# lukashermann/hulc

Hardware: AMD Instinct MI355X
Metric: trajectory-windows/sec (seq_len=32, bs=64/GPU) (higher is better)
Workload: dtype bf16; 1 GPU; HULC training step, vision goal only (use_clip_auxiliary_loss=false), B=64 windows/GPU, seq_len=32, 200x200 static + 84x84 gripper fp32 NCHW frames, fwd+loss+bwd+Adam, dropout 0.1; global_batch=64, seq_len=32, parallelism=dp1

## Files before the change

### hulc_amd/csrc/capi.hip

```cpp
#include <cstdarg>
#include <cstdio>
#include <cstring>
#include <cstdlib>
#include <cmath>
#include <algorithm>
#include <stdexcept>

#include "engine.h"
#include "sbert.h"
#include "store_gather.h"
#include "store_stage.h"

using namespace hulc_bf16;

static thread_local char g_err[1024] = "";
void hulc_set_error(const char* fmt, ...) {
    va_list ap;
    va_start(ap, fmt);
    vsnprintf(g_err, sizeof(g_err), fmt, ap);
    va_end(ap);
}

struct hulc_ctx {
    IEngine* e = nullptr;
// ... 316 lines not shown
int hulc_set_dropout(hulc_ctx* ctx, float p) {
    if (!(p >= 0.f && p < 1.f)) { hulc_set_error("hulc_set_dropout: p must be in [0,1)"); return 1; }
    ctx->e->set_dropout(p);
    return 0;
}
int hulc_set_option(hulc_ctx* ctx, const char* name, int64_t value) {
    if (!ctx) { hulc_set_error("hulc_set_option: null context"); return 1; }
    return ctx->e->set_option(name, (long long)value);
}
int hulc_get_option(hulc_ctx* ctx, const char* name, int64_t* value) {
    if (!ctx || !value) { hulc_set_error("hulc_get_option: null argument"); return 1; }
    if (name && !strcmp(name, "stage_tickets")) { *value = HULC_STAGE_TICKETS; return 0; }
    long long v = 0;
    const int rc = ctx->e->get_option(name, &v);
    *value = (int64_t)v;
    return rc;
}
int hulc_timers_enable(hulc_ctx* ctx, int32_t on, const char* only_class) { ctx->e->set_timing(on != 0, only_class); return 0; }
int hulc_timers_read(hulc_ctx* ctx, char* json_out, int64_t cap, int32_t reset) { return ctx->e->timers_read(json_out, cap, reset != 0); }
int hulc_get_tensor(hulc_ctx* ctx, const char* name, float* out, int64_t cap, int64_t* n) { return ctx->e->get_tensor(name, out, cap, n); }
int hulc_get_plan_idx(hulc_ctx* ctx, int32_t* out, int64_t cap) { return ctx->e->get_plan_idx(out, cap); }

int hulc_k_gemm_nt(int32_t dtype, const void* A, const void* B, float* C, int32_t M, int32_t N, int32_t K, int64_t lda, int64_t ldb, int64_t ldc,
                   const float* bias, int32_t relu, void* stream) {
    if (dtype == HULC_DTYPE_F16) return hulc_f16::k_gemm_nt(0, A, B, C, M, N, K, lda, ldb, ldc, bias, relu, stream);
    return hulc_bf16::k_gemm_nt(dtype == HULC_DTYPE_F32, A, B, C, M, N, K, lda, ldb, ldc, bias, relu, stream);
}
#define HULC_K_16BIT(name, call)                                                                                          \
    if (dtype == HULC_DTYPE_F16) return hulc_f16::call;                                                                    \
    if (dtype == HULC_DTYPE_BF16) return hulc_bf16::call;                                                                  \
    hulc_set_error(name ": dtype %d is not a 16-bit type", (int)dtype);                                                    \
    return 1
int hulc_k_spatial_softmax64(int32_t dtype, const void* f, int32_t H, int32_t W, int32_t Nf, void* out, float* stats, const float* dout, void* df, void* stream) {
    HULC_K_16BIT("hulc_k_spatial_softmax64", k_spatial_softmax64(f, H, W, Nf, out, stats, dout, df, stream));
}
int hulc_k_enc_tail_fwd(int32_t dtype, int32_t Nf, int32_t ldemb, const hulc_enc_tail_job* a, const hulc_enc_tail_job* b, void* emb, const float* pos, int32_t S,
                        float drop_p, uint64_t seed, float* xf, void* xt, float* z0, float* z1, void* stream) {
    HULC_K_16BIT("hulc_k_enc_tail_fwd", k_enc_tail_fwd(Nf, ldemb, a, b, emb, pos, S, drop_p, (unsigned long long)seed, xf, xt, z0, z1, stream));
}
int hulc_k_enc_tail_bwd(int32_t dtype, int32_t Nf, int32_t ldemb, const hulc_enc_tail_bwd_job* a, const hulc_enc_tail_bwd_job* b, const float* demb, void* stream) {
    HULC_K_16BIT("hulc_k_enc_tail_bwd", k_enc_tail_bwd(Nf, ldemb, a, b, demb, stream));
}
int hulc_k_tr_layer_fwd(int32_t dtype, const hulc_tr_layer_job* job, int32_t B, int32_t S, int32_t ln_in, float dp, void* stream) {
    HULC_K_16BIT("hulc_k_tr_layer_fwd", k_tr_layer_fwd(job, B, S, ln_in, dp, stream));
}
int hulc_k_tr_ffn_bwd(int32_t dtype, const hulc_tr_ffn_bwd_job* job, int32_t B, int32_t S, int32_t bcast, float bdiv, float dp, void* stream) {
    HULC_K_16BIT("hulc_k_tr_ffn_bwd", k_tr_ffn_bwd(job, B, S, bcast, bdiv, dp, stream));
}
int hulc_k_tr_attn_bwd(int32_t dtype, const hulc_tr_attn_bwd_job* job, int32_t B, int32_t S, int32_t nparts, int64_t part_stride, float dp, void* stream) {
    HULC_K_16BIT("hulc_k_tr_attn_bwd", k_tr_attn_bwd(job, B, S, nparts, (long long)part_stride, dp, stream));
}
int hulc_k_gemm_multi(int32_t dtype, int32_t form, const hulc_gemm_epi_job* jobs, int32_t n, int32_t sh, int32_t* ran, void* stream) {
    HULC_K_16BIT("hulc_k_gemm_multi", k_gemm_multi(form, jobs, n, sh, ran, stream));
}
#undef HULC_K_16BIT
int hulc_k_gemm_epi(int32_t dtype, const hulc_gemm_epi_job* job, int32_t kernel, int32_t* ran, void* stream) {
    if (dtype == HULC_DTYPE_F16) return hulc_f16::k_gemm_epi(1, job, kernel, ran, stream);
    if (dtype != HULC_DTYPE_F32 && dtype != HULC_DTYPE_BF16) { hulc_set_error("hulc_k_gemm_epi: unknown dtype %d", (int)dtype); return 1; }
    return hulc_bf16::k_gemm_epi(dtype == HULC_DTYPE_BF16 ? 1 : 0, job, kernel, ran, stream);
}
int hulc_k_gemm_pick(int32_t dtype, int32_t M, int32_t N, int32_t K, int64_t lda, int64_t ldb, int32_t* pick, int32_t* bk) {
    if (dtype != HULC_DTYPE_F32 && dtype != HULC_DTYPE_BF16 && dtype != HULC_DTYPE_F16) { hulc_set_error("hulc_k_gemm_pick: unknown dtype %d", (int)dtype); return 1; }
    return hulc_bf16::k_gemm_pick(dtype != HULC_DTYPE_F32, M, N, K, (long long)lda, (long long)ldb, pick, bk);
}
int hulc_k_gemm_wgrad_nsplit(int32_t dtype, int32_t M, int32_t N, int32_t K, int32_t* nsplit, int32_t* big) {
    if (dtype != HULC_DTYPE_F32 && dtype != HULC_DTYPE_BF16 && dtype != HULC_DTYPE_F16) { hulc_set_error("hulc_k_gemm_wgrad_nsplit: unknown dtype %d", (int)dtype); return 1; }
    return hulc_bf16::k_gemm_wgrad_nsplit(dtype != HULC_DTYPE_F32, M, N, K, nsplit, big);
}
int hulc_k_logistic_loss(int32_t dtype, int32_t wide, const float* heads, int32_t ldh, const float* actions, const float* robot_obs, int32_t B, int32_t S,
                         int32_t n_mix, int32_t n_dim, int32_t num_classes, float log_scale_min, float gripper_alpha, int32_t gripper_control,
                         int32_t discrete_gripper, float grad_scale, const float* lscale, float* row_loss, float* a_tcp_out, void* dheads, void* stream) {
    if (dtype == HULC_DTYPE_F16)
        return hulc_f16::k_logistic_loss(1, wide, heads, ldh, actions, robot_obs, B, S, n_mix, n_dim, num_classes, log_scale_min, gripper_alpha, gripper_control,
                                         discrete_gripper, grad_scale, lscale, row_loss, a_tcp_out, dheads, stream);
    if (dtype != HULC_DTYPE_F32 && dtype != HULC_DTYPE_BF16) { hulc_set_error("hulc_k_logistic_loss: unknown dtype %d", (int)dtype); return 1; }
    return hulc_bf16::k_logistic_loss(dtype == HULC_DTYPE_BF16, wide, heads, ldh, actions, robot_obs, B, S, n_mix, n_dim, num_classes, log_scale_min, gripper_alpha,
                                      gripper_control, discrete_gripper, grad_scale, lscale, row_loss, a_tcp_out, dheads, stream);
}
#define HULC_K_ANY(name, fn, ...)                                                                                                     \
    if (dtype == HULC_DTYPE_F16) return hulc_f16::fn(1, __VA_ARGS__);                                                                  \
    if (dtype != HULC_DTYPE_F32 && dtype != HULC_DTYPE_BF16) { hulc_set_error(name ": unknown dtype %d", (int)dtype); return 1; }      \
    return hulc_bf16::fn(dtype == HULC_DTYPE_BF16 ? 1 : 0, __VA_ARGS__)
int hulc_k_plan_kl_sample(const float* pr_logits, const float* pp_logits, int32_t B, int32_t NCAT, int32_t NCLS, const int32_t* idx_in, int32_t* idx_out, float* probs,
                          float* kl_cat, float* dpp, float* dpr, float w_pp, float w_pr, uint64_t seed, const float* lscale, void* stream) {
    return hulc_bf16::k_plan_kl_sample(pr_logits, pp_logits, B, NCAT, NCLS, idx_in, idx_out, probs, kl_cat, dpp, dpr, w_pp, w_pr, (unsigned long long)seed, lscale, stream);
}
int hulc_k_st_softmax_bwd(int32_t dtype, const float* probs, const float* dplan, const float* dpr_kl, const float* dpp_kl, int32_t rows, int32_t NCLS, float* out, void* out_t,
                          void* dpp_t, void* stream) {
    HULC_K_ANY("hulc_k_st_softmax_bwd", k_st_softmax_bwd, probs, dplan, dpr_kl, dpp_kl, rows, NCLS, out, out_t, dpp_t, stream);
}
int hulc_k_plan_gather(int32_t dtype, const void* w_t, const int32_t* idx, int32_t B, int32_t NCAT, int32_t NCLS, int32_t H, const float* b1, const float* b2, float* out,
                       const void* emb, void* embg, int32_t S, int32_t W, const void* goal, int32_t G, int32_t grow0, void* cb, void* stream) {
    HULC_K_ANY("hulc_k_plan_gather", k_plan_gather, w_t, idx, B, NCAT, NCLS, H, b1, b2, out, emb, embg, S, W, goal, G, grow0, cb, stream);
}
int hulc_k_plan_scatter_grad(int32_t dtype, int32_t form, const void* dC, const int32_t* idx, int32_t B, int32_t NCAT, int32_t NCLS, int32_t H, int32_t KIN, float* dw,
                             int32_t store, void* stream) {
    HULC_K_ANY("hulc_k_plan_scatter_grad", k_plan_scatter_grad, form, dC, idx, B, NCAT, NCLS, H, KIN, dw, store, stream);
}
int hulc_k_normal_kl_sample(int32_t dtype, const float* pr_state, const float* pp_state, int32_t B, int32_t n, const float* eps_in, float* eps_out, float* plan_f, void* plan_t,
                            float* kl_elem, float* dpp, float* dpr, float w_pp, float w_pr, uint64_t seed, const float* lscale, void* stream) {
    HULC_K_ANY("hulc_k_normal_kl_sample", k_normal_kl_sample, pr_state, pp_state, B, n, eps_in, eps_out, plan_f, plan_t, kl_elem, dpp, dpr, w_pp, w_pr, (unsigned long long)seed, lscale, stream);
}
int hulc_k_normal_rsample_bwd(int32_t dtype, const float* dplan, const float* eps, const float* pr_state, const float* dpr_kl, int32_t B, int32_t n, void* out, void* stream) {
    HULC_K_ANY("hulc_k_normal_rsample_bwd", k_normal_rsample_bwd, dplan, eps, pr_state, dpr_kl, B, n, out, stream);
}
int hulc_k_det_head_loss(int32_t dtype, const void* H1, const void* W, const float* bias, const float* actions, const float* robot_obs, int32_t B, int32_t S,
// ... 234 lines not shown
```

### hulc_amd/csrc/conv_wgrad.h

```cpp
#pragma once
#include "common.h"

namespace HULC_NS {

typedef short s16x4_t __attribute__((ext_vector_type(4)));
typedef unsigned int u32x4_t __attribute__((ext_vector_type(4)));
typedef __attribute__((address_space(3))) u32x4_t lds_u32x4;

typedef __attribute__((address_space(3))) char lds_char;
DEVI h16x8_t tr_read8(lds_char* p0, lds_char* p1) {
    const s16x4_t lo = __builtin_amdgcn_ds_read_tr16_b64_v4i16((__attribute__((address_space(3))) s16x4_t*)p0);
    const s16x4_t hi = __builtin_amdgcn_ds_read_tr16_b64_v4i16((__attribute__((address_space(3))) s16x4_t*)p1);
    typedef short s16x8_t __attribute__((ext_vector_type(8)));
    const s16x8_t v = __builtin_shufflevector(lo, hi, 0, 1, 2, 3, 4, 5, 6, 7);
    return __builtin_bit_cast(h16x8_t, v);
}

template <int CI, int CO, int KH, int KW, int S>
struct WgradCfg {
    static constexpr int XS = (S == 1) ? ((CI * 2 / 32) | 1) * 32 : CI * 2 + 16;
    static constexpr int DYS = ((CO * 2 / 32) | 1) * 32;
    static constexpr int CGN = CI / 16;
    static constexpr int NT = KH * KW * CGN;
    static constexpr int NTW = NT / 4;
// ... 1547 lines not shown
    }
    const int grid = std::min(form == 5 ? cap : std::min(cap, 512), max_blocks);
    long long total = 0;
    for (int k = 0; k < n; ++k) total += j[k].Nf;
    if (wg) { for (int k = 0; k < n; ++k) ns[k] = std::min(std::max(wg[k], 1), j[k].Nf); }
    else if (n == 1) ns[0] = grid;
    else if (total <= std::min(form == 5 ? (int)total : 512, max_blocks)) { for (int k = 0; k < n; ++k) ns[k] = j[k].Nf; }
    else {
        if (grid < n) return false;
        int left = grid; double wl = 0;
        for (int k = 0; k < n; ++k) wl += w[k];
        for (int k = n - 1; k > 0; --k) {
            int a, b;
            camera_split(left, wl - w[k], w[k], a, b);
            b = std::min(std::min(b, left - k), j[k].Nf);
            ns[k] = b; left -= b; wl -= w[k];
        }
        ns[0] = std::min(left, j[0].Nf);
    }
    Wgrad1Batch bt{}; bt.n = n;
    int blk = 0;
    for (int k = 0; k < n; ++k) {
        if (k) j[k].part = j[k - 1].part + (long long)ns[k - 1] * Wgrad1Cfg::CO * 192;
        j[k].blk0 = blk; blk += ns[k];
        bt.j[k] = j[k];
    }
    if (form == 1) {
        static bool attr2 = false;
        if (!attr2) { hipFuncSetAttribute((const void*)conv1_wgrad_tr2_kernel<6, 2>, hipFuncAttributeMaxDynamicSharedMemorySize, 80 * 1024); attr2 = true; }
        hipLaunchKernelGGL((conv1_wgrad_tr2_kernel<6, 2>), dim3(blk), dim3(512), lds, st, bt);
    } else if (form == 2) {
        static bool attr2s = false;
        if (!attr2s) { hipFuncSetAttribute((const void*)conv1_wgrad_tr2r_kernel<3, 2, true>, hipFuncAttributeMaxDynamicSharedMemorySize, 80 * 1024); attr2s = true; }
        hipLaunchKernelGGL((conv1_wgrad_tr2r_kernel<3, 2, true>), dim3(blk), dim3(512), lds, st, bt);
    } else if (form == 3) {
        static bool attr2r = false;
        if (!attr2r) { hipFuncSetAttribute((const void*)conv1_wgrad_tr2r_kernel<4, 2>, hipFuncAttributeMaxDynamicSharedMemorySize, 80 * 1024); attr2r = true; }
        hipLaunchKernelGGL((conv1_wgrad_tr2r_kernel<4, 2>), dim3(blk), dim3(512), lds, st, bt);
    } else {
        static bool attr_set = false;
        if (!attr_set) { hipFuncSetAttribute((const void*)conv1_wgrad_tr_kernel, hipFuncAttributeMaxDynamicSharedMemorySize, 160 * 1024 - 64); attr_set = true; }
        for (int k = 0; k < n; ++k) bt.j[k].S.fold = 0;
        hipLaunchKernelGGL(conv1_wgrad_tr_kernel, dim3(blk), dim3(256), lds, st, bt);
    }
    return true;
}
static inline int launch_conv1_wgrad_tr(hipStream_t st, const Conv1Src& X, const h16_t* dY, float* part, float* bias_part, int Nf, int IH, int IW, int OH,
                                        int OW, int max_blocks, int* work_ctr = nullptr) {
    Wgrad1Job q{}; q.S = X; q.work_ctr = work_ctr; q.dY = dY; q.part = part; q.bias_part = bias_part; q.Nf = Nf; q.IH = IH; q.IW = IW; q.OH = OH; q.OW = OW;
    int ns = 0;
    return launch_conv1_wgrad_jobs(st, &q, 1, max_blocks, nullptr, &ns) ? ns : 0;
}

DEVI void lin_bwd_smallm_body(const h16_t* __restrict__ dY, long long ldy, const h16_t* __restrict__ X, long long ldx,
                              int M, int N, int K, float* __restrict__ dW, long long lddw, float* __restrict__ db,
                              float* __restrict__ db2, int mchunk, int store, const int bx, const int by, const int bz, const int gz, char* smem,
                              const bool slabs = false) {
    constexpr int TN = 64, TK = 128, YS = TN * 2 + 16, XS = TK * 2 + 16;
    lds_char* yimg = (lds_char*)smem;
    lds_char* ximg = yimg + 64 * YS;
    const int tid = threadIdx.x, lane = tid & 63, wave = tid >> 6;
    const int n0 = bx * TN, k0 = by * TK;
    const int mbeg = bz * mchunk, mend = min(M, mbeg + mchunk);
    const int g = lane >> 4, a = lane & 15;
    const int prow = a >> 2, ccol = (a & 3) * 8;
    f32x4 acc[8];
#pragma unroll
    for (int j = 0; j < 8; ++j) acc[j] = f32x4{0.f, 0.f, 0.f, 0.f};
    float bsum = 0.f;
    const bool atomic_b = gz > 1;
    const bool atomic = atomic_b && !slabs;
    const int n = n0 + wave * 16 + a;
    const bool vec_ok = !atomic && (lddw & 3) == 0 && ((reinterpret_cast<uintptr_t>(dW) & 15) == 0) && k0 + TK <= K;
    const int orow = lane >> 4, ocol = (lane & 15) * 4;
    float4 oldw[8];
    if (vec_ok) {
#pragma unroll
        for (int j = 0; j < 8; ++j) {
            const int nr = n0 + wave * 16 + (j & 3) * 4 + orow;
            oldw[j] = (store || nr >= N) ? make_float4(0.f, 0.f, 0.f, 0.f) : *reinterpret_cast<const float4*>(dW + (long long)nr * lddw + k0 + (j >> 2) * 64 + ocol);
        }
    }
    u32x4_t ry[2], rx[4];
    auto fetch = [&](int m0) {
#pragma unroll
        for (int u = 0; u < 2; ++u) {
            const int i = tid + u * 256, m = i / (TN / 8), c = i % (TN / 8);
            h16_t v[8];
            if (m0 + m < mend && n0 + c * 8 < N) load8_guard<h16_t>(dY + (long long)(m0 + m) * ldy + n0 + c * 8, N - (n0 + c * 8), v);
            else zero8<h16_t>(v);
            ry[u] = *reinterpret_cast<const u32x4_t*>(v);
        }
#pragma unroll
        for (int u = 0; u < 4; ++u) {
            const int i = tid + u * 256, m = i / (TK / 8), c = i % (TK / 8);
            h16_t v[8];
            if (m0 + m < mend && k0 + c * 8 < K) load8_guard<h16_t>(X + (long long)(m0 + m) * ldx + k0 + c * 8, K - (k0 + c * 8), v);
            else zero8<h16_t>(v);
            rx[u] = *reinterpret_cast<const u32x4_t*>(v);
        }
    };
    fetch(mbeg);
    for (int m0 = mbeg; m0 < mend; m0 += 64) {
        if (m0 > mbeg) __syncthreads();
#pragma unroll
        for (int u = 0; u < 2; ++u) { const int i = tid + u * 256; *(lds_u32x4*)(yimg + (i / (TN / 8)) * YS + (i % (TN / 8)) * 16) = ry[u]; }
#pragma unroll
        for (int u = 0; u < 4; ++u) { const int i = tid + u * 256; *(lds_u32x4*)(ximg + (i / (TK / 8)) * XS + (i % (TK / 8)) * 16) = rx[u]; }
        __syncthreads();
        if (m0 + 64 < mend) fetch(m0 + 64);
#pragma unroll
        for (int ms = 0; ms < 2; ++ms) {
            const int mrow = ms * 32 + g * 8 + prow;
            lds_char* yb = yimg + mrow * YS + wave * 32 + ccol;
            const h16x8_t yf = tr_read8(yb, yb + 4 * YS);
#pragma unroll
            for (int j = 0; j < 8; ++j) {
                lds_char* xb = ximg + mrow * XS + j * 32 + ccol;
                const h16x8_t xf = tr_read8(xb, xb + 4 * XS);
                acc[j] = MFMA_16x16x32_H(xf, yf, acc[j], 0, 0, 0);
            }
        }
        if (db && by == 0) {
#pragma unroll 16
            for (int m = 0; m < 16; ++m) bsum += h2f(*(__attribute__((address_space(3))) h16_t*)(yimg + (wave * 16 + m) * YS + lane * 2));
        }
    }
    if (db && by == 0) {
        __syncthreads();
        *(__attribute__((address_space(3))) float*)(yimg + (wave * 64 + lane) * 4) = bsum;
        __syncthreads();
        if (tid < TN) {
            bsum = 0.f;
#pragma unroll
            for (int w = 0; w < 4; ++w) bsum += *(__attribute__((address_space(3))) float*)(yimg + (w * 64 + tid) * 4);
        }
    }
    if (vec_ok) {
        constexpr int OP = 64 * 4 + 16;
        __syncthreads();
        lds_char* const tb = (lds_char*)smem + wave * (16 * OP);
#pragma unroll
        for (int h = 0; h < 2; ++h) {
#pragma unroll
            for (int jj = 0; jj < 4; ++jj) *(__attribute__((address_space(3))) f32x4*)(tb + a * OP + jj * 64 + g * 16) = acc[h * 4 + jj];
#pragma unroll
            for (int it = 0; it < 4; ++it) {
                const f32x4 v = *(__attribute__((address_space(3))) f32x4*)(tb + (it * 4 + orow) * OP + ocol * 4);
                const int nr = n0 + wave * 16 + it * 4 + orow;
                float4 o = oldw[h * 4 + it];
                o.x += v[0]; o.y += v[1]; o.z += v[2]; o.w += v[3];
                if (nr < N) *reinterpret_cast<float4*>(dW + (long long)nr * lddw + k0 + h * 64 + ocol) = o;
            }
        }
    } else if (n < N) {
#pragma unroll
        for (int j = 0; j < 8; ++j) {
            const int k = k0 + j * 16 + g * 4;
            float* p = dW + (long long)n * lddw + k;
            if (atomic) {
#pragma unroll
                for (int r = 0; r < 4; ++r)
                    if (k + r < K) unsafeAtomicAdd(p + r, acc[j][r]);
            } else if (k + 3 < K && ((((uintptr_t)p) & 15) == 0)) {
                float4 o = store ? make_float4(0.f, 0.f, 0.f, 0.f) : *reinterpret_cast<float4*>(p);
                o.x += acc[j][0]; o.y += acc[j][1]; o.z += acc[j][2]; o.w += acc[j][3];
                *reinterpret_cast<float4*>(p) = o;
            } else {
#pragma unroll
                for (int r = 0; r < 4; ++r)
                    if (k + r < K) p[r] = store ? acc[j][r] : p[r] + acc[j][r];
            }
        }
    }
    if (db && by == 0 && tid < TN && n0 + tid < N) {
        if (atomic_b) { unsafeAtomicAdd(db + n0 + tid, bsum); if (db2) unsafeAtomicAdd(db2 + n0 + tid, bsum); }
        else { db[n0 + tid] += bsum; if (db2) db2[n0 + tid] += bsum; }
    }
}

constexpr int LBS_LDS = 64 * (64 * 2 + 16) + 64 * (128 * 2 + 16);
__global__ void __launch_bounds__(256) lin_bwd_smallm_kernel(const h16_t* __restrict__ dY, long long ldy, const h16_t* __restrict__ X, long long ldx,
                                                             int M, int N, int K, float* __restrict__ dW, long long lddw, float* __restrict__ db,
                                                             float* __restrict__ db2, int mchunk, int store = 0) {
    __shared__ __attribute__((aligned(16))) char smem[LBS_LDS];
    lin_bwd_smallm_body(dY, ldy, X, ldx, M, N, K, dW, lddw, db, db2, mchunk, store, blockIdx.x, blockIdx.y, blockIdx.z, gridDim.z, smem);
}
struct LinBwdJob { const h16_t* dY; const h16_t* X; float* dW; float* db; long long ldx, lddw; int N, K, nx, blk0; float* part; };
struct LinBwdBatch { LinBwdJob j[8]; int n, M, store, mchunk; };
__global__ void __launch_bounds__(256) lin_bwd_smallm_batched_kernel(LinBwdBatch bt) {
    __shared__ __attribute__((aligned(16))) char smem[LBS_LDS];
    int k = 0;
    while (k + 1 < bt.n && (int)blockIdx.x >= bt.j[k + 1].blk0) ++k;
    const LinBwdJob J = bt.j[k];
    const int b = blockIdx.x - J.blk0;
    const bool slabs = bt.mchunk > 0 && J.part;
    lin_bwd_smallm_body(J.dY, (long long)J.N, J.X, J.ldx, bt.M, J.N, J.K, slabs ? J.part + (long long)blockIdx.y * J.N * J.K : J.dW, slabs ? (long long)J.K : J.lddw, J.db, nullptr,
                        bt.mchunk > 0 ? bt.mchunk : 64, slabs ? 1 : bt.store, b % J.nx, b / J.nx, blockIdx.y, gridDim.y, smem, slabs);
}

}
```

### hulc_amd/csrc/engine.h

```cpp
#pragma once
#include <algorithm>
#include <map>
#include <string>
#include <vector>

#include "iengine.h"
#include "repro_sites.h"
#include "trainable_plan.h"
#include "gemm.h"
#include "kernels.h"
#include "plan_ln_launch.h"
#include "conv_wgrad.h"
#include "conv_tile.h"
#include "conv_reg.h"
#include "tr_fused.h"
#include "rnn_persist.h"
#include "enc_tail.h"
#include "rollout_step.h"
#include "aux_heads.h"
#include "aux_rows.h"
#include "det_head.h"

namespace HULC_NS {

// ... 661 lines not shown
                    const int i = gq.n++;
                    gq.a[i] = a; gq.b[i] = b; gq.om[i] = om; gq.ep[i] = ep; gq.M[i] = M; gq.N[i] = N; gq.K[i] = K;
                    gq_fl += 2.0 * M * N * K; gq_by += ((double)M * K + (double)N * K + (double)M * N) * sizeof(T);
                    return;
                }
                gemm_group_flush();
            }
        }
        const double fl = 2.0 * M * N * K, by = ((double)M * K + (double)N * K + (double)M * N) * sizeof(T);
        const GemmPick pick = gemm_pick<T>(a, b, ep, M, N, K, gemm_use_glds);
        if (pick == GEMM_PICK_SKINNY) {
            TimerScope ts(this, M <= 64 ? "skinny_gemm_m64" : "skinny_gemm_rows", "hbm", fl, by);
            gemm_launch_picked<T>(st, pick, a, b, om, ep, M, N, K);
        } else if (gemm_pick_tile(pick) == 128) {
            TimerScope ts(this, "gemm_128x128", "mfma", fl, by);
            gemm_launch_picked<T>(st, pick, a, b, om, ep, M, N, K);
        } else gemm_launch_picked<T>(st, pick, a, b, om, ep, M, N, K);
    }
    void gemm_wgrad(const DenseLoader<T>& a, const DenseLoader<T>& b, float* dW, long long lddw, int M, int N, int K) {
        EpiP ep = epi(dW, true); ep.accumulate = 1;
        if constexpr (std::is_same<T, h16_t>::value) {
            if (a.R1 == 0x7fffffff && b.R1 == 0x7fffffff && skinny_ok(M, N, K, a.s1, b.s1, a.p, b.p)) { gemm(a, b, dense_out(lddw), ep, M, N, K); return; }
        }
        bool big = false;
        const int nsplit = gemm_wgrad_nsplit<T>(M, N, K, &big);
        if (nsplit <= 1) { gemm(a, b, dense_out(lddw), ep, M, N, K); return; }
        if (repro) {
            const long long zs = ((long long)M * N + 3) / 4 * 4;
            if (part_cur + zs * nsplit > this->partcap) { gemm(a, b, dense_out(lddw), ep, M, N, K); return; }
            float* const slabs = this->part + part_cur;
            EpiP es = epi(slabs, true); es.z_stride = zs;
            TimerScope ts(this, big ? "gemm_128x128" : "gemm_64x64_splitk", "mfma", 2.0 * M * N * K, ((double)M * K + (double)N * K) * sizeof(T) + 4.0 * M * N * nsplit);
            if (big) launch_gemm<T, 128, 128>(st, a, b, dense_out(N), es, M, N, K, 1, nsplit);
            else launch_gemm<T, 64, 64>(st, a, b, dense_out(N), es, M, N, K, 1, nsplit);
            const int vec = (N & 3) == 0 && (lddw & 3) == 0 && ((uintptr_t)slabs & 15) == 0 && ((uintptr_t)dW & 15) == 0;
            hipLaunchKernelGGL(slab_sum_kernel, dim3(cdiv((long long)M * N, vec ? 1024 : 256)), dim3(256), 0, st, (const float*)slabs, nsplit, zs, M, N, dW, lddw, vec);
            return;
        }
        nd(ND_GEMM_SPLITK);
        ep.atomic = 1;
        TimerScope ts(this, big ? "gemm_128x128" : "gemm_64x64_splitk", "mfma", 2.0 * M * N * K, ((double)M * K + (double)N * K) * sizeof(T) + 4.0 * M * N);
        if (big) launch_gemm<T, 128, 128>(st, a, b, dense_out(lddw), ep, M, N, K, 1, nsplit);
        else launch_gemm<T, 64, 64>(st, a, b, dense_out(lddw), ep, M, N, K, 1, nsplit);
    }
    EpiP epi(void* out, bool f32) const { EpiP e; e.out = out; e.out_f32 = f32 ? 1 : 0; e.generic_only = epilogue_fast ? 0 : 1; return e; }

    void lin_fwd(const T* X, long long ldx, int M, const LinW& L, EpiP ep, long long ldo) {
        if (!ep.bias) ep.bias = L.b32;
        gemm(dense<T>(X, M, ldx), dense<T>(L.W, L.N, L.K), dense_out(ldo), ep, M, L.N, L.K);
    }
    void lin_wgrad(const T* dY, const T* X, long long ldx, int M, int N, int K, float* dW, long long lddw, float* db, float* db2 = nullptr) {
        if constexpr (std::is_same<T, h16_t>::value) {
            if (M <= 64) {
                hipLaunchKernelGGL(lin_bwd_smallm_kernel, dim3(cdiv(N, 64), cdiv(K, 128)), dim3(256), 0, st, dY, (long long)N, X, ldx, M, N, K, dW, lddw, db, db2, 64, grad_first(dW) ? 1 : 0);
                return;
            }
            grad_ensure_zero(dW);
        }
        const int mp = ldpad(M);
        const bool fuse_cs = std::is_same<T, h16_t>::value && !repro;
        transpose_pair(dY, N, tA, M, N, X, ldx, tB, M, K, mp, fuse_cs ? db : nullptr, fuse_cs ? db2 : nullptr);
        gemm_wgrad(dense<T>(tA, N, mp), dense<T>(tB, K, mp), dW, lddw, N, K, M);
        if (db && !fuse_cs) colsum(dY, N, M, N, db, db2);
    }
    void lin_dgrad(const T* dY, int M, const LinW& L, EpiP ep, const DenseOut& om) {
        gemm(dense<T>(dY, M, L.N), dense<T>(L.Wt, L.K, L.N), om, ep, M, L.K, L.N);
    }
    void ln_fwd(const float* x, long long ldx, int rows, int n, const float* g, const float* b, T* out, long long ldo, float* outf, long long ldf,
                float* stats) {
        launch_ln_fwd<T>(st, x, ldx, rows, n, g, b, out, ldo, outf, ldf, stats);
    }
    static constexpr bool ln_bwd_can_bcast = ln_bwd_fused<T>();
    void ln_bwd(const float* dy, long long lddy, const float* x, long long ldx, const float* stats, const float* g, int rows, int n, float* dxf,
                long long ldd, int acc, T* dxt, long long ldt, float* dg, float* db, float drop_p = 0.f, unsigned long long drop_seed = 0,
                int bcast_rows = 0, float bcast_div = 1.f, int dy_parts = 1, long long dy_part_stride = 0) {
        if (ln_bwd_fused<T>() && !repro && dg && cdiv(rows, ln_bwd_rows_per_block(rows)) > 1) nd(ND_LN_PARAM);
        launch_ln_bwd<T>(st, cspart, dy, lddy, x, ldx, stats, g, rows, n, dxf, ldd, acc, dxt, ldt, dg, db, drop_p, drop_seed, bcast_rows, bcast_div, dy_parts, dy_part_stride, repro);
    }

    int prepare_weights(bool shadow_fresh = false) override {
        if (!bound) { hulc_set_error("hulc_prepare_weights before hulc_bind_params"); return 1; }
        const bool masked = shadow_fresh && tm_active;
        if (masked && tm_ntrain == 0) return 0;
        c1_bias_fold_valid = false;
        if constexpr (!std::is_same<T, float>::value) {
            if (!shadow_fresh) hipLaunchKernelGGL((cast_kernel<float, T>), dim3(2048), dim3(256), 0, st, P, wshadow, (long long)numel);
        }
        {
            ConvPackBatch d;
            int k = 0, blk = 0;
            for (EncW* e : {&encS, &encG})
                for (ConvW* c : {&e->c1, &e->c2, &e->c3}) {
                    d.w[k] = c->W32; d.wf[k] = c->Wf; d.wd[k] = c->nhwc ? c->Wd : nullptr; d.O[k] = (masked && !tm_trainable_w(c->W32)) ? 0 : c->O; d.I[k] = c->I; d.K[k] = c->KH; d.S[k] = c->S; d.nhwc[k] = c->nhwc;
                    d.blk0[k] = blk; blk += cdiv(c->O * c->I * c->KH * c->KW, 256); ++k;
                }
            d.blk0[6] = blk;
            const int blkA = blk, blkB = blkA + cdiv(128 * 3136, 256);
            HeadPack hp = head_pack();
            const int rows = head_rows[0] + head_rows[1] + head_rows[2] + head_rows[3];
            const int r7 = (masked && !tm_trainable_w(encG.fc7.W32)) ? 0 : 128;
            if (masked && !heads_trainable()) for (int i = 0; i < 4; ++i) hp.rows[i] = 0;
            T* const f7t = rest_by_pack ? encG.fc7.Wt : (T*)nullptr;
            T* const wht = rest_by_pack ? wheadsT : (T*)nullptr;
            hipLaunchKernelGGL((weight_pack_kernel<T>), dim3(blkB + cdiv((long long)rows * HID, 256)), dim3(256), 0, st, d, blkA, encG.fc7.W32, encG.fc7.W, r7, 64, 49, blkB, hp,
                               wheads, bheads, HID, f7t, wht, NHEAD);
        }
        if (masked) {
            if (std::is_same<T, float>::value) { if (tm_tr_all.blocks) hipLaunchKernelGGL((batched_transpose_kernel<float, T>), dim3(tm_tr_all.blocks), dim3(256), 0, st, (const TrDesc*)tm_tr_all.desc, tm_tr_all.n); }
            else if (tr_fresh) { if (tm_tr_rest.blocks && !rest_by_pack) hipLaunchKernelGGL(batched_transpose64_kernel, dim3(tm_tr_rest.blocks), dim3(256), 0, st, (const TrDesc*)tm_tr_rest.desc, tm_tr_rest.n, (const unsigned short*)tm_tr_rest.b2d); }
            else if (tm_tr_all.blocks) hipLaunchKernelGGL(batched_transpose64_kernel, dim3(tm_tr_all.blocks), dim3(256), 0, st, (const TrDesc*)tm_tr_all.desc, tm_tr_all.n, (const unsigned short*)tm_tr_all.b2d);
        }
        else if (std::is_same<T, float>::value) hipLaunchKernelGGL((batched_transpose_kernel<float, T>), dim3(tr_blocks), dim3(256), 0, st, trdesc_dev, (int)trdesc.size());
        else if (tr_fresh && tr_adam.n) {
            if (tr_rest.blocks && !rest_by_pack) hipLaunchKernelGGL(batched_transpose64_kernel, dim3(tr_rest.blocks), dim3(256), 0, st, tr_rest.desc, tr_rest.n, (const unsigned short*)tr_rest.b2d);
        }
        else hipLaunchKernelGGL(batched_transpose64_kernel, dim3(tr_blocks), dim3(256), 0, st, trdesc_dev, (int)trdesc.size(), (const unsigned short*)blk2desc_dev);
        const bool was_fresh = tr_fresh && tr_adam.n;
        tr_fresh = false;
        if constexpr (std::is_same<T, h16_t>::value) {
            if (masked) { if (tm_frag.n && !(was_fresh && frag_by_adam)) hipLaunchKernelGGL(frag_pack_kernel, dim3(tm_frag_blocks), dim3(256), 0, st, tm_frag); }
            else if (fragbatch.n && !(was_fresh && frag_by_adam)) hipLaunchKernelGGL(frag_pack_kernel, dim3(frag_blocks), dim3(256), 0, st, fragbatch);
        }
        if (hipGetLastError() != hipSuccess) { hulc_set_error("kernel launch failed in prepare_weights"); return 1; }
        return 0;
    }
    T *trb_c[2] = {nullptr, nullptr}, *trb_a[2] = {nullptr, nullptr}, *trb_d[2] = {nullptr, nullptr}, *trb_b[2] = {nullptr, nullptr};
    LinBwdBatch tr_wjobs{};
    int tr_wblocks = 0;
    void tr_wgrad_add(const T* dY, const T* X, const LinW& L) {
        if constexpr (std::is_same<T, h16_t>::value) {
            LinBwdJob& J = tr_wjobs.j[tr_wjobs.n++];
            J.dY = dY; J.X = X; J.dW = L.dW; J.db = L.db; J.ldx = L.K; J.lddw = L.K; J.N = L.N; J.K = L.K; J.nx = cdiv(L.N, 64); J.blk0 = tr_wblocks; J.part = nullptr;
            tr_wblocks += J.nx * cdiv(L.K, 128);
        }
    }
    void tr_wgrads_flush(int M) {
        if constexpr (std::is_same<T, h16_t>::value) {
            if (tr_wjobs.n == 0) return;
            const int chunk = 256, nz = cdiv(M, chunk);
            tr_wjobs.M = M; tr_wjobs.store = 0; tr_wjobs.mchunk = chunk;
            UnpackBatch ub{};
            int64_t cur = 0; int ublocks = 0;
            for (int i = 0; i < tr_wjobs.n; ++i) {
                LinBwdJob& J = tr_wjobs.j[i];
                const int64_t need = (int64_t)nz * J.N * J.K;
                if (part_cur + cur + need > this->partcap) { J.part = nullptr; continue; }
                J.part = this->part + part_cur + cur; cur += need;
                UnpackJob& U = ub.j[ub.n++];
                U.part = J.part; U.grad = J.dW; U.slab = (long long)J.N * J.K; U.nsplit = nz; U.O = J.N; U.I = J.K; U.KH = U.KW = 1; U.nhwc = 0; U.blk0 = ublocks; U.ysplit = 1;
                ublocks += cdiv(J.N * J.K, 1024);
            }
            if (nz > 1) nd(ND_LIN_BWD_ROWS);
            hipLaunchKernelGGL(lin_bwd_smallm_batched_kernel, dim3(tr_wblocks, nz), dim3(256), 0, st, tr_wjobs);
            if (ub.n > 0) hipLaunchKernelGGL(unpack_conv_wgrad_batched_kernel, dim3(ublocks, 1), dim3(256), 0, st, ub);
            tr_wjobs.n = 0; tr_wblocks = 0;
        }
    }
    float* dparts = nullptr;
    h16_t* dump_page = nullptr;
    bool grads_fresh = false;
    int wacc() const { return grads_fresh ? 0 : 1; }
    struct LazyG { int64_t off, n; bool stale; };
    std::vector<LazyG> lazy;
    void lazy_register(const LinW& L) {
        if (!std::is_same<T, h16_t>::value || !L.dW || (int64_t)L.N * L.K < 65536) return;
        const int64_t off = L.dW - G, exact = (int64_t)L.N * L.K;
        int64_t n = (exact + 63) / 64 * 64;
        for (const auto& kv : tab_order) if (kv.second.off > off && kv.second.off < off + n) n = exact;
        if (off + n > numel) n = exact;
        if (n % 4 || off % 4) return;
        for (const LazyG& z : lazy) if (z.off == off) return;
        if (lazy.size() < 30 && off >= 0 && off + n <= numel) lazy.push_back(LazyG{off, n, false});
    }
    int lazy_find(const float* dW) const { const int64_t off = dW - G; for (size_t i = 0; i < lazy.size(); ++i) if (lazy[i].off == off) return (int)i; return -1; }
    bool grad_first(const float* dW) {
        const int i = lazy_find(dW);
        if (i < 0) return grads_fresh;
        const bool s = lazy[i].stale;
        lazy[i].stale = false;
        return s;
    }
    void grad_ensure_zero(const float* dW) {
        const int i = lazy_find(dW);
        if (i >= 0 && lazy[i].stale) { hipMemsetAsync(G + lazy[i].off, 0, sizeof(float) * lazy[i].n, st); lazy[i].stale = false; }
    }
    void lazy_sweep(int64_t lo, int64_t hi, hipStream_t s) {
        MultiZero mz{}; int k = 0; long long mx = 0;
        for (LazyG& z : lazy)
            if (z.stale && z.off >= lo && z.off + z.n <= hi) { mz.p[k] = G + z.off; mz.n[k] = z.n; mx = std::max<long long>(mx, z.n); ++k; z.stale = false; }
        if (k) hipLaunchKernelGGL(multi_zero_kernel, dim3((unsigned)std::min<long long>(256, cdiv(mx, 4 * 256 * 8)), k), dim3(256), 0, s, mz);
    }
    int flush_grads() override {
        if (!bound) { hulc_set_error("hulc_flush_grads before hulc_bind_params"); return 1; }
        lazy_sweep(0, numel, st);
        return 0;
    }
    int zero_grads() override {
        if (!bound) { hulc_set_error("hulc_zero_grads before hulc_bind_params"); return 1; }
        if (!have_fwd) repro_latch();
        if (lazy.empty() || !lazy_zero_mode) {
            HIP_CHECK(hipMemsetAsync(G, 0, numel * sizeof(float), st));
            for (LazyG& z : lazy) z.stale = false;
        } else {
            MultiZero mz{}; int k = 0; long long mx = 0; int64_t cur = 0;
            auto add = [&](int64_t lo, int64_t hi) { if (hi > lo) { mz.p[k] = G + lo; mz.n[k] = hi - lo; mx = std::max<long long>(mx, hi - lo); ++k; } };
            for (LazyG& z : lazy) { add(cur, z.off); cur = z.off + z.n; z.stale = true; }
            add(cur, numel / 4 * 4);
            if (numel % 4) HIP_CHECK(hipMemsetAsync(G + numel / 4 * 4, 0, sizeof(float) * (numel % 4), st));
// ... 267 lines not shown
```

### hulc_amd/csrc/engine_backward.inc

```
    struct Bucket { int64_t lo, hi; };
    Bucket group_range(const char* prefix) const {
        int64_t lo = numel, hi = 0;
        const std::string a(prefix);
        for (size_t i = 0; i < tab_order.size(); ++i) {
            const auto& kv = tab_order[i];
            if (kv.first.compare(0, a.size(), a) == 0) { lo = std::min(lo, kv.second.off); hi = std::max(hi, i + 1 < tab_order.size() ? tab_order[i + 1].second.off : numel); }
        }
        if (hi <= lo) return Bucket{0, 0};
        return Bucket{lo, std::min<int64_t>(hi, numel)};
    }
    std::vector<std::pair<std::string, Ref>> tab_order;
    std::vector<Bucket> bucket_plan() const {
        std::vector<Bucket> v;
        const Bucket dec = group_range("action_decoder.");
        v.push_back(Bucket{dec.lo, numel});
        v.push_back(group_range("plan_proposal."));
        v.push_back(group_range("plan_recognition."));
        const Bucket vg = group_range("visual_goal."), lg = group_range("language_goal.");
        v.push_back(Bucket{std::min(vg.lo, lg.lo), std::max(vg.hi, lg.hi)});
        v.push_back(group_range("perceptual_encoder."));
        return v;
    }
    int comm_buckets(int64_t* lo, int64_t* hi, int cap) override {
        if (!bound) { hulc_set_error("hulc_comm_buckets before hulc_bind_params"); return -1; }
// ... 21 lines not shown
    int reduce_range(int64_t lo, int64_t hi, int dtype, int span = -1) {
        if (hi <= lo) return 0;
        GradComm& c = *comm;
        const bool vote = vote_pad() >= 0 ? (skip_pad >= lo && skip_pad < hi) : lo == 0;
        if (vote) { skip_vote_put(st); ar_voted = true; }
        c.gate_from(st);
        const size_t n = (size_t)(hi - lo);
        if (span >= 0) c.span_begin(span, (dtype == HULC_DTYPE_F32 ? 4.0 : 2.0) * n);
        int rc;
        if (dtype == HULC_DTYPE_BF16 || dtype == HULC_DTYPE_F16) {
            if (c.stage_elems < numel) {
                if (c.stage) hipFree(c.stage);
                if (hipMalloc(&c.stage, (size_t)numel * 2 + 256) != hipSuccess) { hulc_set_error("hulc_allreduce_grads: staging buffer allocation failed"); return 1; }
                c.stage_elems = numel;
            }
            h16_t* sg = reinterpret_cast<h16_t*>(c.stage) + lo;
            hipLaunchKernelGGL((cast_kernel<float, h16_t>), dim3(std::min<long long>(2048, cdiv((long long)n, 1024))), dim3(256), 0, c.cs, G + lo, sg, (long long)n);
#ifdef HULC_HALF_F16
            const int wire = GradComm::F16;
#else
            const int wire = GradComm::BF16;
#endif
            rc = GradComm::api().allreduce(sg, sg, n, wire, GradComm::SUM, c.comm, c.cs);
            hipLaunchKernelGGL((cast_kernel<h16_t, float>), dim3(std::min<long long>(2048, cdiv((long long)n, 1024))), dim3(256), 0, c.cs, sg, G + lo, (long long)n);
            c.bytes_reduced += 2.0 * n;
        } else {
            rc = GradComm::api().allreduce(G + lo, G + lo, n, GradComm::F32, GradComm::SUM, c.comm, c.cs);
            c.bytes_reduced += 4.0 * n;
        }
        c.n_collectives++;
        if (vote && vote_pad() < 0 && rc == 0 && vote_ptr()) { rc = GradComm::api().allreduce(vote_word, vote_word, 1, GradComm::F32, GradComm::SUM, c.comm, c.cs); c.n_collectives++; c.bytes_reduced += 4.0; }
        if (vote) skip_vote_get(c.cs);
        if (span >= 0) c.span_end(span);
        if (rc != 0) { hulc_set_error("ncclAllReduce failed: %s", GradComm::err(rc)); return 1; }
        return 0;
    }
    bool ar_voted = false;
    int vote_only() {
        if (!rp_skip) rp_skip = alloc<unsigned>(64);
        if (!vote_word) vote_word = alloc<float>(64);
        if (!rp_skip || !vote_word) { hulc_set_error("skip vote: allocation failed"); return 1; }
        GradComm& c = *comm;
        hipLaunchKernelGGL(dp_skip_put_kernel, dim3(1), dim3(1), 0, st, (const unsigned*)rp_skip, opt_seq + 1, vote_word);
        c.gate_from(st);
        const int rc = GradComm::api().allreduce(vote_word, vote_word, 1, GradComm::F32, GradComm::SUM, c.comm, c.cs);
        c.n_collectives++; c.bytes_reduced += 4.0;
        hipLaunchKernelGGL(dp_skip_get_kernel, dim3(1), dim3(1), 0, c.cs, vote_word, rp_skip, opt_seq + 1);
        ar_voted = true;
        if (rc != 0) { hulc_set_error("ncclAllReduce failed: %s", GradComm::err(rc)); return 1; }
        return 0;
    }
    int bucket_ready(int i) {
        if (ar_dtype < 0 || (ar_sent >> i) & 1u) return 0;
        const std::vector<Bucket> v = bucket_plan();
        ar_sent |= 1u << i;
        if (range_all_frozen(v[i].lo, v[i].hi)) return (i == 4 && !ar_voted) ? vote_only() : 0;
        lazy_sweep(v[i].lo, v[i].hi, st);
        return reduce_range(v[i].lo, v[i].hi, ar_dtype, comm_timing ? i : -1);
    }
    int check_ar_dtype(int dtype, const char* who) {
        if (!comm) { hulc_set_error("%s: no communicator (hulc_comm_init first)", who); return 1; }
        if (dtype != HULC_DTYPE_F32 && dtype != HULC_DTYPE_BF16 && dtype != HULC_DTYPE_F16) { hulc_set_error("%s: bucket dtype must be HULC_DTYPE_F32 or a 16-bit type", who); return 1; }
        if (dtype != HULC_DTYPE_F32) {
            if (std::is_same<T, float>::value) { hulc_set_error("%s: 16-bit buckets need a bf16 / fp16 engine (the fp32 engine has no 16-bit kernels in its unit)", who); return 1; }
#ifdef HULC_HALF_F16
            if (dtype != HULC_DTYPE_F16) { hulc_set_error("%s: the fp16 engine offers fp16 buckets (loss-scaled gradients), not bf16", who); return 1; }
#else
            if (dtype != HULC_DTYPE_BF16) { hulc_set_error("%s: the bf16 engine offers bf16 buckets, not fp16", who); return 1; }
#endif
        }
        return 0;
    }
    int allreduce_grads(int dtype) override {
        if (check_ar_dtype(dtype, "hulc_allreduce_grads")) return 1;
        if (!bound) { hulc_set_error("hulc_allreduce_grads before hulc_bind_params"); return 1; }
        if (bwd_stage != 0) { hulc_set_error("hulc_allreduce_grads: encoder part of the backward still pending"); return 1; }
        lazy_sweep(0, numel, st);
        if (tm_active && bucket_plan_ok()) {
            std::vector<Bucket> v = bucket_plan();
            v.erase(std::remove_if(v.begin(), v.end(), [](const Bucket& b) { return b.hi <= b.lo; }), v.end());
            std::sort(v.begin(), v.end(), [](const Bucket& a, const Bucket& b) { return a.lo < b.lo; });
            ar_voted = false;
            for (size_t i = 0; i < v.size();) {
                if (range_all_frozen(v[i].lo, v[i].hi)) { ++i; continue; }
                size_t j = i;
                while (j + 1 < v.size() && !range_all_frozen(v[j + 1].lo, v[j + 1].hi)) ++j;
                if (reduce_range(v[i].lo, v[j].hi, dtype)) return 1;
                i = j + 1;
            }
            if (!ar_voted && vote_only()) return 1;
        } else if (reduce_range(0, numel, dtype)) return 1;
        comm->gate_to(st);
        return 0;
    }
    bool bucket_plan_ok() const {
        std::vector<Bucket> v = bucket_plan();
        v.erase(std::remove_if(v.begin(), v.end(), [](const Bucket& b) { return b.hi <= b.lo; }), v.end());
        std::sort(v.begin(), v.end(), [](const Bucket& a, const Bucket& b) { return a.lo < b.lo; });
        if (v.empty() || v.front().lo != 0 || v.back().hi != numel) return false;
        for (size_t i = 0; i + 1 < v.size(); ++i) if (v[i].hi != v[i + 1].lo) return false;
        return true;
    }
    int backward_allreduce(int dtype) override {
        if (ema_refuse("hulc_backward_allreduce")) return 1;
        if (check_ar_dtype(dtype, "hulc_backward_allreduce")) return 1;
        if (!bucket_plan_ok()) { hulc_set_error("hulc_backward_allreduce: the module-group buckets do not partition the gradient buffer (layout changed?)"); return 1; }
        ar_dtype = dtype; ar_sent = 0; ar_voted = false;
        if (comm_timing) comm->bwd_mark(true, st);
        int rc = backward(-1);
        if (!rc) for (int i = 0; i < 5 && !rc; ++i) rc = bucket_ready(i);
        ar_dtype = -1;
        if (rc) return rc;
        if (comm_timing) comm->bwd_mark(false, st);
        comm->gate_to(st);
        return 0;
    }

    int bwd_stage = 0;
    int backward(int part = -1) override {
        if (ema_refuse("hulc_backward")) return 1;
        if (!have_fwd) { hulc_set_error("hulc_backward without a preceding hulc_forward_loss"); return 1; }
        persist_check("hulc_backward", false);
        bwd_since_opt = true;
        if (part == 1 && bwd_stage != 1) { hulc_set_error("hulc_backward_part(1) must follow hulc_backward_part(0)"); return 1; }
        if (part != 1 && bwd_stage != 0) { hulc_set_error("hulc_backward: encoder part of the previous backward still pending"); return 1; }
        const hulc_batch* b = &cur;
        const int B = b->B, S = b->S, N = B * S, SB = S * B;
        const bool hulc = cfg.kind == HULC_KIND_HULC;
        const float dp = cfg.dropout_p;
        const long long BH = (long long)B * HID;
        const bool cs16 = std::is_same<T, h16_t>::value && !repro;
        if (part == 1) { if (bwd_skip_enc) goto finish; goto encoders; }
        bwd_skip_enc = tm_enc_frozen;
        if (!arena_clean) HIP_CHECK(hipMemsetAsync(zero_arena, 0, sizeof(float) * zero_n, st));
        arena_clean = false;
        work_ctr_next = 0;
        if (poison_partials) HIP_CHECK(hipMemsetAsync(this->part, 0xFF, sizeof(float) * (size_t)this->partcap, st));
        {
        bool have_dseq = false, dseq_cast_done = false;
        const int proj_n = clip_n > 0 ? clip_n : mia_n;
        if (proj_n > 0 || bcz_n > 0) {
            const int n = proj_n > 0 ? proj_n : bcz_n;
            if (proj_n > 0) {
                hipLaunchKernelGGL((cast_kernel<float, T>), dim3(1), dim3(256), 0, st, dimg, dimg_t, (long long)n * GOAL);
                hipLaunchKernelGGL((cast_kernel<float, T>), dim3(1), dim3(256), 0, st, dtxt, dtxt_t, (long long)n * GOAL);
                lin_wgrad(dimg_t, im1, 128, n, GOAL, 128, cl_im2.dW, 128, cl_im2.db);
                { EpiP ep = epi(dim1, false); ep.mask = im1; lin_dgrad(dimg_t, n, cl_im2, ep, dense_out(128)); }
                lin_wgrad(dim1, sf_m, FCH, n, 128, FCH, cl_im0.dW, FCH, cl_im0.db);
                { EpiP ep = epi(dsf_m, true); lin_dgrad(dim1, n, cl_im0, ep, dense_out(FCH)); }
            }
            if (bcz_n > 0) {
                hipLaunchKernelGGL((cast_kernel<float, T>), dim3(cdiv(n * LANG, 256)), dim3(256), 0, st, bz_dpred, bz_dpred_t, (long long)n * LANG);
                lin_wgrad(bz_dpred_t, bz1, 512, n, LANG, 512, bz2.dW, 512, bz2.db);
                { EpiP ep = epi(dbz1, false); ep.mask = bz1; lin_dgrad(bz_dpred_t, n, bz2, ep, dense_out(512)); }
                lin_wgrad(dbz1, sf_m, FCH, n, 512, FCH, bz0.dW, FCH, bz0.db);
                { EpiP ep = epi(dsf_m, true); if (proj_n > 0) ep.accumulate = 1; lin_dgrad(dbz1, n, bz0, ep, dense_out(FCH)); }
            }
            hipLaunchKernelGGL(scatter_rows_add_kernel, dim3(cdiv(n * FCH, 256)), dim3(256), 0, st, dsf_m, auxrows, n, FCH, dseqf, (long long)FCH);
            if (proj_n > 0) {
                lin_wgrad(dtxt_t, la1, 128, n, GOAL, 128, cl_la2.dW, 128, cl_la2.db);
                { EpiP ep = epi(dla1, false); ep.mask = la1; lin_dgrad(dtxt_t, n, cl_la2, ep, dense_out(128)); }
                lin_wgrad(dla1, g_m, GOAL, n, 128, GOAL, cl_la0.dW, GOAL, cl_la0.db);
                { EpiP ep = epi(dg_m, true); lin_dgrad(dla1, n, cl_la0, ep, dense_out(GOAL)); }
                hipLaunchKernelGGL(scatter_rows_add_kernel, dim3(cdiv(n * GOAL, 256)), dim3(256), 0, st, dg_m, auxrows, n, GOAL, dgoal, (long long)GOAL);
            }
            have_dseq = true;
        }
        {
            const long long lastBH = (long long)(S - 1) * BH;
            if (det) {
                if (part_cur + (int64_t)det_head_slabs(SB) * DET_SLAB > this->partcap) { hulc_set_error("hulc_backward: no room for the deterministic head's gradient slabs"); return 1; }
                launch_det_head_dgrad<T>(st, dpre, det_w, H1, B, S, dH1, dZ1 + lastBH);
                launch_det_head_wgrad<T>(st, dpre, H1, SB, this->part + part_cur, det_dw, det_db);
            } else {
            { EpiP ep = epi(dH1, false);
              if (!mlp) { ep.out2 = dZ1 + lastBH; ep.out2_lo = lastBH; ep.out2_hi = lastBH + BH; ep.out2_mask = H1 + lastBH; }
              gemm(dense<T>(dheads, SB, NHEAD), dense<T>(wheadsT, HID, NHEAD), dense_out(HID), ep, SB, HID, NHEAD); }
            {
                const HeadPack hp = head_pack();
                const int rows = head_rows[0] + head_rows[1] + head_rows[2] + head_rows[3];
                const T* const hx = mlp ? Zx1 : H1;
                bool slabs = false;
                if constexpr (std::is_same<T, h16_t>::value) {
                    const int nz = cdiv(SB, 256);
                    if (SB > 64 && part_cur + (int64_t)nz * NHEAD * HID <= this->partcap) {
                        LinBwdBatch bt{}; bt.M = SB; bt.store = 0; bt.mchunk = 256; bt.n = 1;
                        LinBwdJob& J = bt.j[0];
                        if (nz > 1 && !repro) nd(ND_LIN_BWD_ROWS);
                        J.dY = dheads; J.X = hx; J.dW = nullptr; J.db = (repro && nz > 1) ? nullptr : dbheads_tmp; J.ldx = HID; J.lddw = HID; J.N = NHEAD; J.K = HID; J.nx = cdiv(NHEAD, 64); J.blk0 = 0;
                        J.part = this->part + part_cur;
                        hipLaunchKernelGGL(lin_bwd_smallm_batched_kernel, dim3(J.nx * cdiv(HID, 128), nz), dim3(256), 0, st, bt);
                        if (!J.db) colsum(dheads, NHEAD, SB, NHEAD, dbheads_tmp);
                        hipLaunchKernelGGL(unpack_heads_grad_kernel, dim3(cdiv((long long)rows * HID, 256)), dim3(256), 0, st, hp, J.part, dbheads_tmp, HID, nz, (long long)NHEAD * HID);
                        slabs = true;
                    }
                }
                if (!slabs) {
                    lin_wgrad(dheads, hx, HID, SB, NHEAD, HID, dwheads_tmp, HID, dbheads_tmp);
                    hipLaunchKernelGGL(unpack_heads_grad_kernel, dim3(cdiv((long long)rows * HID, 256)), dim3(256), 0, st, hp, dwheads_tmp, dbheads_tmp, HID, 1, 0ll);
                }
            }
            }
            if (mlp) {
                lin_wgrad(dH1, H1, HID, SB, HID, HID, mlp2.dW, HID, mlp2.db);
                { EpiP ep = epi(dZ1, false); ep.mask = H1; lin_dgrad(dH1, SB, mlp2, ep, dense_out(HID)); }
                lin_wgrad(dZ1, H0, HID, SB, HID, HID, mlp1.dW, HID, mlp1.db);
                { EpiP ep = epi(dZ0, false); ep.mask = H0; lin_dgrad(dZ1, SB, mlp1, ep, dense_out(HID)); }
                const int mp = ldpad(SB);
                transpose_pair(dZ0, HID, tA, SB, HID, embg, DE, tB, SB, DE, mp, cs16 ? dbih0 : nullptr, nullptr);
                h0t_valid = false;
                { EpiP ep = epi(dwih0 + dec_plan, true); ep.accumulate = 1; gemm(dense<T>(tA, HID, mp), dense<T>(tB, DE, mp), dense_out(KIN), ep, HID, DE, SB); }
            } else {
            rnn_bwd(dH1, H1, dZ1, whh1, B, S, 1, false, false, true);
            {
                const int mp = ldpad(SB);
                const bool fuse_cs = cs16;
                bool h0t_kept = false;
                if constexpr (std::is_same<T, h16_t>::value) {
                    if (!tB2) tB2 = alloc<T>(tcap);
                    if (tB2) { transpose_triple(dZ1, HID, tA, SB, HID, H1, HID, tB, SB, HID, H0, HID, tB2, SB, HID, mp, fuse_cs ? dbih1 : nullptr, fuse_cs ? dbhh1 : nullptr); h0t_kept = true; }
                }
                if (!h0t_kept)
                transpose_pair(dZ1, HID, tA, SB, HID, H1, HID, tB, SB, HID, mp, fuse_cs ? dbih1 : nullptr, fuse_cs ? dbhh1 : nullptr);
                h0t_valid = h0t_kept;
                bool paired = false;
                if constexpr (std::is_same<T, h16_t>::value) {
                    const bool pair_sw = gemm_pair_mode;
                    EpiP e1 = epi(whh1.dW, true), e2 = epi(wih1.dW, true);
                    if (pair_sw && gemm_use_glds && S > 1 && gemm_glds_pair_ok(dense<T>(tA, HID, mp), dense<T>(tB, HID, mp), dense<T>(tB, HID, mp), e1, e2, HID, HID, SB, B)) {
                        if (!tB2) tB2 = alloc<T>(tcap);
                        if (tB2) {
                            if (!h0t_kept) cast_tr<T, T>(H0, HID, nullptr, 0, tB2, mp, SB, HID);
                            e1.accumulate = grad_first(whh1.dW) ? 0 : 1; e2.accumulate = grad_first(wih1.dW) ? 0 : 1;
                            TimerScope ts(this, "gemm_128x128", "mfma", 2.0 * HID * HID * ((double)SB + (double)(S - 1) * B), (3.0 * HID * SB) * sizeof(T) + 8.0 * HID * HID, 1);
                            launch_gemm_glds_pair(st, dense<T>(tA, HID, mp), dense<T>(tB, HID, mp), dense<T>(tB2, HID, mp), dense_out(HID), e1, e2, HID, HID, SB, B);
                            paired = true;
                        }
                    }
                }
                if (!paired && h0t_kept && std::is_same<T, h16_t>::value) gemm_group_begin();
                if (!paired) {
                if (S > 1) { EpiP ep = epi(whh1.dW, true); ep.accumulate = grad_first(whh1.dW) ? 0 : 1;
                  gemm(dense<T>(tA + B, HID, mp), dense<T>(tB, HID, mp), dense_out(HID), ep, HID, HID, (S - 1) * B); }
                if (!h0t_kept) cast_tr<T, T>(H0, HID, nullptr, 0, tB, mp, SB, HID);
                { EpiP ep = epi(wih1.dW, true); ep.accumulate = grad_first(wih1.dW) ? 0 : 1; gemm(dense<T>(tA, HID, mp), dense<T>(h0t_kept ? tB2 : tB, HID, mp), dense_out(HID), ep, HID, HID, SB); }
                }
                if (!fuse_cs) colsum(dZ1, HID, SB, HID, dbih1, dbhh1);
            }
            { EpiP ep = epi(dH0, false); ep.out2 = dZ0 + lastBH; ep.out2_lo = lastBH; ep.out2_hi = lastBH + BH; ep.out2_mask = H0 + lastBH;
              gemm(dense<T>(dZ1, SB, HID), dense<T>(wih1.Wt, HID, HID), dense_out(HID), ep, SB, HID, HID); }
            gemm_group_end();
            rnn_bwd(dH0, H0, dZ0, whh0, B, S, 1, false, false, true);
            {
                const int mp = ldpad(SB);
                if (h0t_valid) {
                    transpose_pair(dZ0, HID, tA, SB, HID, embg, DE, tB, SB, DE, mp, cs16 ? dbih0 : nullptr, cs16 ? dbhh0 : nullptr);
                    if (S > 1) { EpiP ep = epi(whh0.dW, true); ep.accumulate = grad_first(whh0.dW) ? 0 : 1;
                      gemm(dense<T>(tA + B, HID, mp), dense<T>(tB2, HID, mp), dense_out(HID), ep, HID, HID, (S - 1) * B); }
                } else {
                transpose_pair(dZ0, HID, tA, SB, HID, H0, HID, tB, SB, HID, mp, cs16 ? dbih0 : nullptr, cs16 ? dbhh0 : nullptr);
                if (S > 1) { EpiP ep = epi(whh0.dW, true); ep.accumulate = grad_first(whh0.dW) ? 0 : 1;
                  gemm(dense<T>(tA + B, HID, mp), dense<T>(tB, HID, mp), dense_out(HID), ep, HID, HID, (S - 1) * B); }
                cast_tr<T, T>(embg, DE, nullptr, 0, tB, mp, SB, DE);
                }
                { EpiP ep = epi(dwih0 + dec_plan, true); ep.accumulate = 1; gemm(dense<T>(tA, HID, mp), dense<T>(tB, DE, mp), dense_out(KIN), ep, HID, DE, SB); }
            }
            }
            if (!bwd_skip_enc) { EpiP ep = epi(demb + (EMB - DE), true); ep.accumulate = 1;
              gemm(dense<T>(dZ0, SB, HID), dense<T>(wih0T + (long long)dec_plan * HID, DE, HID), dense_out_map(B, EMB, (long long)S * EMB), ep, SB, DE, HID); }
            hipLaunchKernelGGL((sum_over_t_kernel<T>), dim3(cdiv(BH, 256)), dim3(256), 0, st, dZ0, S, BH, dC);
            if constexpr (!std::is_same<T, h16_t>::value) colsum(dC, HID, B, HID, dbih0, dbhh0);
            else if (!cs16) colsum(dZ0, HID, SB, HID, dbih0, dbhh0);
            { EpiP ep = epi(dgoal, true); ep.accumulate = 1;
              gemm(dense<T>(dC, B, HID), dense<T>(wih0T + (long long)(dec_plan + DE) * HID, GOAL, HID), dense_out(GOAL), ep, B, GOAL, HID); }
            {
                const int mp = ldpad(B);
                transpose_pair(dC, HID, tA, B, HID, goal_t, GOAL, tB, B, GOAL, mp);
                EpiP ep = epi(dwih0 + dec_plan + DE, true); ep.accumulate = 1;
                gemm(dense<T>(tA, HID, mp), dense<T>(tB, GOAL, mp), dense_out(KIN), ep, HID, GOAL, B);
            }
            if (hulc) {
                { EpiP ep = epi(dplan, true); gemm(dense<T>(dC, B, HID), dense<T>(wih0T, PLAN, HID), dense_out(PLAN), ep, B, PLAN, HID); }
                launch_plan_scatter_grad<T>(st, plan_scatter_w4<T>(NCLS), dC, pidx, B, NCAT, NCLS, HID, KIN, dwih0, grads_fresh ? 1 : 0);
            }
            if (mcil) {
                { EpiP ep = epi(dplan, true); gemm(dense<T>(dC, B, HID), dense<T>(wih0T, dec_plan, HID), dense_out(dec_plan), ep, B, dec_plan, HID); }
                lin_wgrad(dC, plan_t, dec_plan, B, HID, dec_plan, dwih0, KIN, nullptr);
            }
        }
        const bool hold_buckets = hold_buckets_mode && mcil && !gru && ar_dtype >= 0 && persist_mode && !persist_under_comm && !(rp_probed && !rp_ok);
        if (!hold_buckets && bucket_ready(0)) return 1;
        if (hulc) {
            launch_st_softmax_bwd<T>(st, probs, dplan, dpr_kl, dpp_kl, B * NCAT, NCLS, dprl, dprl_t, dppl_t);
            DenseOut om = dense_out(EMB + GOAL);
            mlp_bwd(dppl_t, ppx, EMB + GOAL, B, pp, 5, ppa, dt_a, dt_a + (long long)B * HID, dppx, &om, 0);
            hipLaunchKernelGGL(pp_input_bwd_kernel, dim3(cdiv(B * (EMB + GOAL), 256)), dim3(256), 0, st, dppx, B, EMB, GOAL, demb, (long long)S * EMB, dgoal);
            if (bucket_ready(1)) return 1;
            lin_wgrad(dprl_t, seqf_t, FCH, B, PLAN, FCH, pr_fs.dW, FCH, pr_fs.db);
            { EpiP ep = epi(dseqf, true);
              if (have_dseq) ep.accumulate = 1;
              else { ep.out2 = dseq_t; ep.out2_lo = 0; ep.out2_hi = (long long)B * FCH; dseq_cast_done = true; }
              lin_dgrad(dprl_t, B, pr_fs, ep, dense_out(FCH)); }
            have_dseq = true;
        }
        if (mcil) {
            const int n = PLAN / 2;
            launch_normal_rsample_bwd<T>(st, dplan, plan_eps, pr_logits, dpr_kl, B, n, dprl_t);
            hipLaunchKernelGGL((cast_kernel<float, T>), dim3(cdiv(B * PLAN, 256)), dim3(256), 0, st, dpp_kl, dppl_t, (long long)B * PLAN);
            DenseOut om = dense_out(EMB + GOAL);
            mlp_bwd(dppl_t, ppx, EMB + GOAL, B, pp, 5, ppa, dt_a, dt_a + (long long)B * HID, dppx, &om, 0);
            hipLaunchKernelGGL(pp_input_bwd_kernel, dim3(cdiv(B * (EMB + GOAL), 256)), dim3(256), 0, st, dppx, B, EMB, GOAL, demb, (long long)S * EMB, dgoal);
            if (!hold_buckets && bucket_ready(1)) return 1;
            if (gru) bigru_bwd(dprl_t, B, S); else birnn_bwd(dprl_t, B, S);
            if (hold_buckets && (bucket_ready(0) || bucket_ready(1))) return 1;
        }
        if (have_dseq) {
            if (!dseq_cast_done) hipLaunchKernelGGL((cast_kernel<float, T>), dim3(cdiv(B * FCH, 256)), dim3(256), 0, st, dseqf, dseq_t, (long long)B * FCH);
            lin_wgrad(dseq_t, xm, EMB, B, FCH, EMB, pr_fc.dW, EMB, pr_fc.db);
            { EpiP ep = epi(dxm, true); lin_dgrad(dseq_t, B, pr_fc, ep, dense_out(EMB)); }
            float* dx = dxa; float* dnext = dxb;
            if (!ln_bwd_can_bcast) hipLaunchKernelGGL(bcast_over_s_kernel, dim3(cdiv((long long)N * EMB, 256)), dim3(256), 0, st, dxm, B, S, EMB, dx);
            for (int l = 1; l >= 0; --l) {
                const bool bc = ln_bwd_can_bcast && l == 1;
                bool ffn_fused = false;
                if constexpr (std::is_same<T, h16_t>::value) ffn_fused = trf_on() && S <= 64;
                T *b_c = dt_c, *b_a = dt_a, *b_d = dt_c, *b_b = dt_b;
                bool defer_w = false;
                if constexpr (std::is_same<T, h16_t>::value) {
                    defer_w = ffn_fused;
                    if (defer_w) {
                        if (!trb_c[l]) { trb_c[l] = alloc<T>((int64_t)maxN * EMB); trb_a[l] = alloc<T>((int64_t)maxN * FF); trb_d[l] = alloc<T>((int64_t)maxN * EMB, l ? "tr_bd1" : "tr_bd0"); trb_b[l] = alloc<T>((int64_t)maxN * 3 * EMB, l ? "tr_bb1" : "tr_bb0"); }
                        b_c = trb_c[l]; b_a = trb_a[l]; b_d = trb_d[l]; b_b = trb_b[l];
                    }
                }
                if constexpr (std::is_same<T, h16_t>::value) {
                    if (ffn_fused) {
                        if (!dparts) dparts = alloc<float>(4ll * maxN * EMB);
                        TrFfnBwdP q{};
                        q.dx = bc ? dxm : dx; q.bcast = bc ? 1 : 0; q.bdiv = (float)S; q.y2 = y2[l]; q.st2 = st2[l]; q.n2g = tr_n2g[l]; q.dg2 = d_tr_n2g[l]; q.db2 = d_tr_n2b[l];
                        q.W2t = tr_l2[l].Wtfr; q.W1t = tr_l1[l].Wtfr; q.hff = hff[l]; q.dt_c = b_c; q.dt_a = b_a; q.part = dparts; q.B = B; q.S = S; q.N = N; q.dp = dp;
                        q.seed_y = site_seed(4 + 4 * l);
                        {
                            TimerScope ts(this, "transformer_fused", "mfma", 2.0 * N * (2.0 * EMB * FF), (double)N * (2 * EMB + FF) * sizeof(T));
                            if (B > 1) nd(ND_TR_LN_BWD);
                            launch_tr_ffn_bwd(st, q);
                        }
                        tr_wgrad_add(b_c, hff[l], tr_l2[l]); tr_wgrad_add(b_a, x1t[l], tr_l1[l]);
                    }
                }
                if (!ffn_fused) {
                ln_bwd(bc ? dxm : dx, EMB, y2[l], EMB, st2[l], tr_n2g[l], N, EMB, dy_f, EMB, 0, dt_c, EMB, d_tr_n2g[l], d_tr_n2b[l], dp, site_seed(4 + 4 * l),
                       bc ? S : 0, (float)S);
                lin_wgrad(dt_c, hff[l], FF, N, EMB, FF, tr_l2[l].dW, FF, tr_l2[l].db);
                { EpiP ep = epi(dt_a, false); ep.mask = hff[l]; ep.alpha = dp > 0.f ? 1.f / (1.f - dp) : 1.f; lin_dgrad(dt_c, N, tr_l2[l], ep, dense_out(FF)); }
                lin_wgrad(dt_a, x1t[l], EMB, N, FF, EMB, tr_l1[l].dW, EMB, tr_l1[l].db);
                { EpiP ep = epi(dnext, true); ep.res = dy_f; ep.res_f32 = 1; ep.res_ld = EMB; lin_dgrad(dt_a, N, tr_l1[l], ep, dense_out(EMB)); }
                }
                bool attn_fused = false;
                if constexpr (std::is_same<T, h16_t>::value) {
                    attn_fused = ffn_fused && EMB == 128 && NH == 8 && S <= 32;
                    if (attn_fused) {
                        TrAttnBwdP q{};
                        q.parts = dparts; q.part_stride = (long long)N * EMB; q.nparts = 4; q.y1 = y1[l]; q.st1 = st1[l]; q.n1g = tr_n1g[l]; q.dg1 = d_tr_n1g[l]; q.db1 = d_tr_n1b[l];
                        q.Wot = tr_out[l].Wtfr; q.Wint = tr_in[l].Wtfr; q.qkv = qkv[l]; q.Pat = Pat[l]; q.b_d = b_d; q.b_b = b_b; q.dy_f = dy_f; q.dx = dx;
                        q.B = B; q.S = S; q.dp = dp; q.seed_o = site_seed(2 + 4 * l); q.seed_att = site_seed(1 + 4 * l);
                        launch_tr_attn_bwd(st, q);
                        tr_wgrad_add(b_d, ao[l], tr_out[l]);
                        tr_wgrad_add(b_b, xt[l], tr_in[l]);
                        continue;
                    }
                }
                ln_bwd(ffn_fused ? dparts : dnext, EMB, y1[l], EMB, st1[l], tr_n1g[l], N, EMB, dy_f, EMB, 0, b_d, EMB, d_tr_n1g[l], d_tr_n1b[l], dp, site_seed(2 + 4 * l), 0, 1.f,
                       ffn_fused ? 4 : 1, (long long)N * EMB);
                if (defer_w) tr_wgrad_add(b_d, ao[l], tr_out[l]);
                else lin_wgrad(b_d, ao[l], EMB, N, EMB, EMB, tr_out[l].dW, EMB, tr_out[l].db);
                { EpiP ep = epi(dt_a, false); lin_dgrad(b_d, N, tr_out[l], ep, dense_out(EMB)); }
                launch_attention_bwd<T>(st, attention_s64(S), qkv[l], Pat[l], dt_a, B, S, EMB, NH, b_b, dp, site_seed(1 + 4 * l));
                if (defer_w) tr_wgrad_add(b_b, xt[l], tr_in[l]);
                else lin_wgrad(b_b, xt[l], EMB, N, 3 * EMB, EMB, tr_in[l].dW, EMB, tr_in[l].db);
                { EpiP ep = epi(dx, true); ep.res = dy_f; ep.res_f32 = 1; ep.res_ld = EMB; lin_dgrad(b_b, N, tr_in[l], ep, dense_out(EMB)); }
            }
            tr_wgrads_flush(N);
            {
                const int bchunk = (std::is_same<T, float>::value || repro) ? B : 8;
                if (cdiv(B, bchunk) > 1) nd(ND_POS_EMB);
                hipLaunchKernelGGL(pr_input_bwd_kernel, dim3(cdiv(S * EMB, 256), cdiv(B, bchunk)), dim3(256), 0, st, dx, B, S, EMB, dp, site_seed(0), demb, dpos, bchunk);
            }
        }
        if (bucket_ready(1) || bucket_ready(2)) return 1;
        if (pair) {
            const int Bv = pairBv, Bl = B - pairBv;
            T* av[2] = {gl1, gl2};
            T* al[2] = {gl1 + (long long)Bv * HID, gl2 + (long long)Bv * HID};
            ln_bwd(dgoal, GOAL, gl3, GOAL, goal_st, ln_vg_g, Bv, GOAL, nullptr, 0, 0, dgl3_t, GOAL, d_ln_vg_g, d_ln_vg_b);
            DenseOut om = dense_out((long long)S * EMB);
            mlp_bwd(dgl3_t, emb + (long long)(S - 1) * EMB, (long long)S * EMB, Bv, vg, 3, av, dt_a, dt_a + (long long)B * HID, bwd_skip_enc ? nullptr : demb + (long long)(S - 1) * EMB, bwd_skip_enc ? nullptr : &om, bwd_skip_enc ? 0 : 1);
            ln_bwd(dgoal + Bv * GOAL, GOAL, gl3 + Bv * GOAL, GOAL, goal_st + 2 * Bv, ln_lg_g, Bl, GOAL, nullptr, 0, 0, dgl3_t + Bv * GOAL, GOAL, d_ln_lg_g, d_ln_lg_b);
            mlp_bwd(dgl3_t + Bv * GOAL, lang_t, LANG, Bl, lg, 3, al, dt_a, dt_a + (long long)B * HID, nullptr, nullptr, 0);
        } else {
            T* acts[2] = {gl1, gl2};
            if (b->is_lang) {
                ln_bwd(dgoal, GOAL, gl3, GOAL, goal_st, ln_lg_g, B, GOAL, nullptr, 0, 0, dgl3_t, GOAL, d_ln_lg_g, d_ln_lg_b);
                mlp_bwd(dgl3_t, lang_t, LANG, B, lg, 3, acts, dt_a, dt_a + (long long)B * HID, nullptr, nullptr, 0);
            } else {
                ln_bwd(dgoal, GOAL, gl3, GOAL, goal_st, ln_vg_g, B, GOAL, nullptr, 0, 0, dgl3_t, GOAL, d_ln_vg_g, d_ln_vg_b);
                DenseOut om = dense_out((long long)S * EMB);
                mlp_bwd(dgl3_t, emb + (long long)(S - 1) * EMB, (long long)S * EMB, B, vg, 3, acts, dt_a, dt_a + (long long)B * HID,
                        bwd_skip_enc ? nullptr : demb + (long long)(S - 1) * EMB, bwd_skip_enc ? nullptr : &om, bwd_skip_enc ? 0 : 1);
            }
        }
        }
        if (bucket_ready(3)) return 1;
        if (part == 0) {
            lazy_sweep(0, numel, st);
            if (hipGetLastError() != hipSuccess) { hulc_set_error("kernel launch failed in backward"); return 1; }
            bwd_stage = 1;
            return 0;
        }
        if (bwd_skip_enc) goto finish;
    encoders:
        {
            const Conv1Src src[2] = {conv1_src(*b, false), conv1_src(*b, true)}, src2[2] = {conv1_src(cur2, false), conv1_src(cur2, true)};
            const int Nenc = enc_frames(N);
            const bool tail_fused = enc_tail_fusable() && (!repro || enc_tail_bwd_room(Nenc));
            if (ragged()) launch_rows_reduce(st, demb, rg_lens(), rg_off(), B, S, EMB, demb_c);
            if (tail_fused) enc_tail_bwd_both(Nenc);
            enc_bwd_both(src, pair ? src2 : nullptr, Nenc, tail_fused);
            flush_unpacks();
        }
    finish:
        if (bucket_ready(4)) return 1;
        lazy_sweep(0, numel, st);
        if (hipGetLastError() != hipSuccess) { hulc_set_error("kernel launch failed in backward"); return 1; }
        have_fwd = false;
        bwd_stage = 0;
        grads_fresh = false;
        return 0;
    }
```

### hulc_amd/csrc/engine_encoders.inc

```
    ConvGeom geom(int Nf, int IH, int C, int K, int S) const {
        ConvGeom g; g.Nf = Nf; g.IH = g.IW = IH; g.C = C; g.KH = g.KW = K; g.S = S; g.OH = g.OW = (IH - K) / S + 1; return g;
    }
    Conv1Src conv1_src(const hulc_batch& b, bool gripper) const {
        Conv1Src s;
        s.X = gripper ? b.rgb_gripper : b.rgb_static;
        s.u8 = b.frames_u8 != 0;
        s.shift = s.u8 ? (gripper ? b.shift_gripper : b.shift_static) : nullptr;
        s.pad = gripper ? b.pad_gripper : b.pad_static;
        s.fold = (s.u8 && std::is_same<T, h16_t>::value && u8_fold_mode) ? 1 : 0;
        if (s.u8 && b.window_start) { s.wstart = reinterpret_cast<const long long*>(b.window_start); s.S = b.S; s.nstore = b.store_frames; }
        if (s.wstart && (b.window_len || b.window_len_host)) {
            const int set = &b == &cur2 ? 1 : 0;
            s.wstart = wl_frame[set]; s.S = 1;
            if (s.shift) s.shift = wl_shift[set][gripper ? 1 : 0];
        }
        return s;
    }
    static Conv1Src conv1_src_f32(const void* x) { return Conv1Src{x, nullptr, 0, 0}; }
    long long* wl_frame[2] = {nullptr, nullptr};
    int* wl_shift[2][2] = {{nullptr, nullptr}, {nullptr, nullptr}};
    int wl_alloc(int set) {
        if (!wl_frame[set]) {
            wl_frame[set] = alloc<long long>((int64_t)maxN); wl_shift[set][0] = alloc<int>((int64_t)maxN * 2); wl_shift[set][1] = alloc<int>((int64_t)maxN * 2);
            if (alloc_failed) { hulc_set_error("window_len: workspace allocation failed"); return 1; }
// ... 181 lines not shown
        return ok(encS) && ok(encG) && EMB == 128;
    }
    bool x0_done = false;
    void enc_tail_fwd_both(int Nf, bool with_x0 = false, int S = 1, float dp = 0.f) {
        if constexpr (std::is_same<T, h16_t>::value) {
            EncTailP q{};
            if (with_x0) { q.pos = pos32; q.xf = xf[0]; q.xt = xt[0]; q.z0 = y2[0]; q.z1 = y2[1]; q.S = S; q.drop_p = dp; q.seed = site_seed(0); x0_done = true; }
            for (int k = 0; k < 2; ++k) {
                const EncW& e = encw(k); EncA& a = enca(k);
                EncTailCam& c = q.cam[k];
                c.x = e.gripper ? a.g0 : a.ss; c.W1 = e.fc1.W; c.W2 = e.fc2.W; c.b1 = e.fc1.b32; c.b2 = e.fc2.b32;
                c.lng = e.lng; c.lnb = e.lnb; c.f1 = a.f1; c.f2 = a.f2; c.lnst = a.lnst; c.col0 = k * 64;
            }
            q.emb = enc_emb(); q.Nf = Nf; q.ldemb = EMB;
            launch_enc_tail_fwd(st, q);
        }
    }
    UnpackBatch unpack_jobs{};
    int64_t part_cur = 0;
    int unpack_blocks = 0;
    bool unpack_room(int jobs, int64_t floats) const { return unpack_jobs.n + jobs <= UNPACK_MAX_JOBS && part_cur + floats <= this->partcap; }
    float* queue_unpack(float* grad, int O, int I, int KH, int KW, int nhwc, int nsplit, int ysplit) {
        const long long slab = (long long)O * I * KH * KW;
        if (!unpack_room(1, nsplit * slab)) return nullptr;
        float* const slabs = this->part + part_cur;
        UnpackJob& U = unpack_jobs.j[unpack_jobs.n++];
        U.part = slabs; U.grad = grad; U.slab = slab; U.nsplit = nsplit; U.O = O; U.I = I; U.KH = KH; U.KW = KW; U.nhwc = nhwc; U.blk0 = unpack_blocks; U.ysplit = ysplit;
        unpack_blocks += cdiv((int)slab, 1024); part_cur += nsplit * slab;
        return slabs;
    }
    void flush_unpacks() {
        constexpr int yparts = 8;
        if (repro) for (int i = 0; i < unpack_jobs.n; ++i) unpack_jobs.j[i].ysplit = 1;
        else for (int i = 0; i < unpack_jobs.n; ++i) if (unpack_jobs.j[i].ysplit == 0 && unpack_jobs.j[i].nsplit > 1) nd(ND_CONV_UNPACK_SPLIT);
        if (unpack_jobs.n > 0) hipLaunchKernelGGL(unpack_conv_wgrad_batched_kernel, dim3(unpack_blocks, repro ? 1 : yparts), dim3(256), 0, st, unpack_jobs);
        unpack_jobs.n = 0; part_cur = 0; unpack_blocks = 0;
    }
    bool tail_fc7_done = false;
    void enc_tail_bwd_both(int Nf) {
        if constexpr (std::is_same<T, h16_t>::value) {
            EncTailBwdP q{};
            for (int k = 0; k < 2; ++k) {
                const EncW& e = encw(k); EncA& a = enca(k);
                EncTailBwdCam& c = q.cam[k];
                c.f2 = a.f2; c.lnst = a.lnst; c.lng = e.lng; c.f1 = a.f1; c.W2t = e.fc2.Wt; c.W1t = e.fc1.Wt;
                c.xmask = a.g0; c.dlng = e.dlng; c.dlnb = e.dlnb;
                c.d_f2 = a.d_f2t; c.d_f1 = a.d_f1; c.dx_f32 = a.d_ss; c.dx_t = a.d_g0; c.col0 = k * 64;
            }
            q.demb = enc_demb(); q.Nf = Nf; q.ldemb = EMB;
            const int nblk = cdiv(Nf, 16);
            const bool slab_pg = repro && nblk > 1;
            if (slab_pg) for (int k = 0; k < 2; ++k) q.cam[k].pg_slab = cspart + (long long)k * 2 * nblk * 64;
            if (!repro && Nf > 16) nd(ND_ENC_TAIL_LN);
            if (!repro && Nf > 256) nd(ND_LIN_BWD_ROWS);
            launch_enc_tail_bwd(st, q);
            if (slab_pg)
                for (int k = 0; k < 2; ++k) {
                    hipLaunchKernelGGL(colsum_final_kernel, dim3(1), dim3(256), 0, st, (const float*)q.cam[k].pg_slab, nblk, 64, encw(k).dlng, (float*)nullptr, 1.f);
                    hipLaunchKernelGGL(colsum_final_kernel, dim3(1), dim3(256), 0, st, (const float*)q.cam[k].pg_slab + (long long)nblk * 64, nblk, 64, encw(k).dlnb, (float*)nullptr, 1.f);
                }
            constexpr int chunk = 256;
            LinBwdBatch bt{}; bt.M = Nf; bt.store = 0; bt.mchunk = chunk;
            int blk = 0;
            const int nz = cdiv(Nf, chunk);
            const bool cs_bias = repro && nz > 1;
            auto add = [&](const T* dY, const T* X, const LinW& L, float* dW, float* slabs) {
                LinBwdJob& J = bt.j[bt.n++];
                J.dY = dY; J.X = X; J.dW = dW; J.db = cs_bias ? nullptr : L.db; J.ldx = L.K; J.lddw = L.K; J.N = L.N; J.K = L.K; J.nx = cdiv(L.N, 64); J.blk0 = blk; J.part = slabs;
                blk += J.nx * cdiv(L.K, 128);
            };
            for (int k = 0; k < 2; ++k) {
                const EncW& e = encw(k); EncA& a = enca(k);
                add(a.d_f2t, a.f1, e.fc2, e.fc2.dW, queue_unpack(e.fc2.dW, e.fc2.N, e.fc2.K, 1, 1, 0, nz, 1));
                add(a.d_f1, e.gripper ? a.g0 : a.ss, e.fc1, e.fc1.dW, queue_unpack(e.fc1.dW, e.fc1.N, e.fc1.K, 1, 1, 0, nz, 1));
            }
            const LinW& L = encG.fc7;
            float* const slabs7 = L.N == 128 && L.K == 3136 ? queue_unpack(L.dW, 128, 64, 7, 7, 1, nz, 1) : nullptr;
            tail_fc7_done = slabs7 != nullptr;
            if (slabs7) add(aG.d_g0, aG.a3, L, nullptr, slabs7);
            hipLaunchKernelGGL(lin_bwd_smallm_batched_kernel, dim3(blk, nz), dim3(256), 0, st, bt);
            if (cs_bias) {
                for (int k = 0; k < 2; ++k) {
                    const EncW& e = encw(k); EncA& a = enca(k);
                    colsum(a.d_f2t, e.fc2.N, Nf, e.fc2.N, e.fc2.db);
                    colsum(a.d_f1, e.fc1.N, Nf, e.fc1.N, e.fc1.db);
                }
                if (slabs7) colsum(aG.d_g0, L.N, Nf, L.N, L.db);
            }
        }
    }
    bool enc_tail_bwd_room(int Nf) const {
        const int64_t nz = cdiv(Nf, 256);
        return unpack_room(5, nz * (2 * (64ll * 512 + 512ll * 128) + 128ll * 3136));
    }
    h16_t* zero_page = nullptr;
    const h16_t* wgrad_zero_page() {
        if constexpr (std::is_same<T, h16_t>::value) { if (!zero_page) zero_page = alloc<h16_t>(128); }
        return zero_page;
    }
    template <int TM, typename LB> int wgrad_gemm(const ConvW& c, const T* dy, const LB& lb, long long npix) {
        const int Kc = c.I * c.KH * c.KW;
        int nsplit = (int)std::min<long long>(std::max<long long>(1, npix / 2048), (this->partcap - part_cur) / ((long long)c.O * Kc));
        nsplit = std::min(nsplit, 256);
        EpiP ep = epi(this->part + part_cur, true); ep.z_stride = (long long)c.O * Kc;
        PixMajorLoaderT<T> la{}; la.p = dy; la.rows = c.O; la.ld = c.O;
        launch_gemm<T, TM, 64>(st, la, lb, dense_out(Kc), ep, c.O, Kc, (int)npix, 1, nsplit);
        return nsplit;
    }
    void wgrad_unpack(const ConvW& c, const T* dy, long long npix, int nsplit, bool bias_done) {
        const bool many = std::is_same<T, h16_t>::value && nsplit >= 64;
        const int yparts = many && !repro ? 16 : 1;
        if (!(many && queue_unpack(c.dW, c.O, c.I, c.KH, c.KW, c.nhwc, nsplit, 0))) {
            if (yparts > 1) nd(ND_CONV_UNPACK_SPLIT);
            hipLaunchKernelGGL(unpack_conv_wgrad_kernel, dim3(cdiv(c.O * c.I * c.KH * c.KW, 1024), yparts), dim3(256), 0, st, this->part + part_cur, nsplit,
                               (long long)c.O * c.I * c.KH * c.KW, c.dW, c.O, c.I, c.KH, c.KW, c.nhwc);
        }
        if (!bias_done) colsum(dy, c.O, (int)npix, c.O, c.db);
    }
    void conv_wgrad(int k, int sn, int Nf) {
        const Stage s = stage(k, sn, Nf);
        const ConvW& c = s.c; const ConvGeom& g = s.g;
        const long long npix = (long long)g.Nf * g.OH * g.OW;
        int nsplit = 0;
        if constexpr (std::is_same<T, h16_t>::value) {
            TimerScope ts(this, "conv_wgrad_tr", "mfma", conv_wgrad_flops(c, g), conv_wgrad_bytes(c, g, 2));
            float* const kb = repro ? nullptr : c.db;
            if (c.I == 64 && c.KH == 3) nsplit = launch_conv_wgrad_tr<64, 64, 3, 3, 1>(st, s.x, s.dy, this->part + part_cur, kb, g.Nf, g.IH, g.IW, g.OH, g.OW, 512, claim_ctr(g.Nf > 1), wgrad_zero_page());
            else if (c.I == 32 && c.KH == 4) nsplit = launch_conv_wgrad_tr<32, 64, 4, 4, 2>(st, s.x, s.dy, this->part + part_cur, kb, g.Nf, g.IH, g.IW, g.OH, g.OW, 512, claim_ctr(g.Nf > 1), wgrad_zero_page());
            if (nsplit > 1 && !repro) nd(ND_CONV_BIAS);
        }
        const bool tr = nsplit > 0;
        if (!tr) nsplit = wgrad_gemm<64>(c, s.dy, ConvNHWCLoaderT<T>{s.x, g}, npix);
        wgrad_unpack(c, s.dy, npix, nsplit, tr && !repro);
    }
    void conv1_wgrad(int k, const Conv1Src& src, int Nf, const Conv1Src* src2) {
        const EncW& e = encw(k); EncA& a = enca(k);
        const ConvW& c = e.c1;
        for (int h = 0; h < (src2 ? 2 : 1); ++h) {
            const int nf = src2 ? src_frames(Nf, h) : Nf;
            const ConvGeom g = geom(nf, e.IH, 3, 8, 4);
            const long long npix = (long long)nf * g.OH * g.OW;
            const Conv1Src& sh = h ? *src2 : src;
            const long long foff = h ? src_frames(Nf, 0) : 0;
            const T* dy = a.dact1 + foff * g.OH * g.OW * 32;
            const float* x = nullptr;
// ... 191 lines not shown
```

### hulc_amd/csrc/engine_forward.inc

```
    void mlp_fwd(const T* x, long long ldx, int M, LinW* L, int n, T** acts, float* outf, T* outt) {
        const T* in = x; long long ld = ldx;
        for (int i = 0; i < n; ++i) {
            if (i < n - 1) { EpiP ep = epi(acts[i], false); ep.relu = 1; lin_fwd(in, ld, M, L[i], ep, L[i].N); in = acts[i]; ld = L[i].N; }
            else {
                if (outf) { EpiP ep = epi(outf, true); lin_fwd(in, ld, M, L[i], ep, L[i].N); }
                if (outt) { EpiP ep = epi(outt, false); lin_fwd(in, ld, M, L[i], ep, L[i].N); }
            }
        }
    }
    T* mlp_dy[8] = {nullptr, nullptr, nullptr, nullptr, nullptr, nullptr, nullptr, nullptr};
    void mlp_bwd(const T* dy, const T* x, long long ldx, int M, LinW* L, int n, T** acts, T* s0, T* s1, float* dxf, const DenseOut* om, int dx_acc) {
        const T* d = dy;
        if constexpr (std::is_same<T, h16_t>::value) {
            if (M <= 64 && n <= 8) {
                bool all_first = true;
                for (int i = 0; i < n; ++i) { const int z = lazy_find(L[i].dW); all_first = all_first && (z >= 0 ? lazy[z].stale : grads_fresh); }
                for (int i = 0; i < n; ++i) { if (all_first) grad_first(L[i].dW); else grad_ensure_zero(L[i].dW); }
                LinBwdBatch bt{}; bt.M = M; bt.store = all_first ? 1 : 0;
                int blk = 0;
                for (int i = n - 1; i >= 0; --i) {
                    const T* in = i > 0 ? acts[i - 1] : x;
                    const long long ld = i > 0 ? L[i - 1].N : ldx;
                    LinBwdJob& J = bt.j[bt.n++];
                    J.dY = d; J.X = in; J.dW = L[i].dW; J.db = L[i].db; J.ldx = ld; J.lddw = L[i].K; J.N = L[i].N; J.K = L[i].K; J.nx = cdiv(L[i].N, 64); J.blk0 = blk;
                    blk += J.nx * cdiv(L[i].K, 128);
                    if (i > 0) {
                        if (!mlp_dy[i]) mlp_dy[i] = alloc<T>((int64_t)64 * 2048);
                        T* o = L[i].K <= 2048 ? mlp_dy[i] : (T*)nullptr;
                        if (!o) { hulc_set_error("mlp_bwd: hidden width %d exceeds the per-layer gradient buffers", L[i].K); return; }
                        EpiP ep = epi(o, false); ep.mask = acts[i - 1];
                        lin_dgrad(d, M, L[i], ep, dense_out(L[i].K));
                        d = o;
                    } else if (dxf) {
                        EpiP ep = epi(dxf, true); ep.accumulate = dx_acc;
                        lin_dgrad(d, M, L[i], ep, *om);
                    }
                }
                hipLaunchKernelGGL(lin_bwd_smallm_batched_kernel, dim3(blk), dim3(256), 0, st, bt);
                return;
            }
        }
        T* scratch[2] = {s0, s1};
        for (int i = n - 1; i >= 0; --i) {
            const T* in = i > 0 ? acts[i - 1] : x;
            const long long ld = i > 0 ? L[i - 1].N : ldx;
            lin_wgrad(d, in, ld, M, L[i].N, L[i].K, L[i].dW, L[i].K, L[i].db);
            if (i > 0) {
                T* o = scratch[i & 1];
                EpiP ep = epi(o, false); ep.mask = acts[i - 1];
                lin_dgrad(d, M, L[i], ep, dense_out(L[i].K));
                d = o;
            } else if (dxf) {
                EpiP ep = epi(dxf, true); ep.accumulate = dx_acc;
                lin_dgrad(d, M, L[i], ep, *om);
            }
        }
    }

    void trunk_fwd(const hulc_batch* b, float dp) {
        const int B = b->B, S = b->S, N = B * S;
        const bool hulc = cfg.kind == HULC_KIND_HULC;
        bool ppx_packed = false;
        {
            const Conv1Src src[2] = {conv1_src(*b, false), conv1_src(*b, true)}, src2[2] = {conv1_src(cur2, false), conv1_src(cur2, true)};
            const bool tail_fused = enc_tail_fusable();
            const int Nenc = enc_frames(N);
            enc_fwd_both(src, pair ? src2 : nullptr, Nenc, tail_fused);
            x0_done = false;
            if (tail_fused) enc_tail_fwd_both(Nenc, !ragged() && !mcil && trf_on() && S <= 64 && EMB == 128, S, dp);
            if (ragged()) launch_rows_expand<T>(st, emb_c, rg_lens(), rg_off(), B, S, EMB, emb);
            enc_frames_last = Nenc;
        }
        if (pair) {
            const int Bv = pairBv, Bl = B - pairBv;
            T* av[2] = {gl1, gl2};
            T* al[2] = {gl1 + (long long)Bv * HID, gl2 + (long long)Bv * HID};
            mlp_fwd(emb + (long long)(S - 1) * EMB, (long long)S * EMB, Bv, vg, 3, av, gl3, nullptr);
            ln_fwd(gl3, GOAL, Bv, GOAL, ln_vg_g, ln_vg_b, goal_t, GOAL, nullptr, 0, goal_st);
            hipLaunchKernelGGL((cast_kernel<float, T>), dim3(cdiv(Bl * LANG, 256)), dim3(256), 0, st, b->lang, lang_t, (long long)Bl * LANG);
            mlp_fwd(lang_t, LANG, Bl, lg, 3, al, gl3 + Bv * GOAL, nullptr);
            ln_fwd(gl3 + Bv * GOAL, GOAL, Bl, GOAL, ln_lg_g, ln_lg_b, goal_t + Bv * GOAL, GOAL, nullptr, 0, goal_st + 2 * Bv);
        } else {
            T* acts[2] = {gl1, gl2};
            auto goal_ln = [&](const float* g_, const float* b_) {
                if (hulc || mcil) {
                    hipLaunchKernelGGL((goal_ln_concat_kernel<T>), dim3(cdiv(B, 4) + cdiv(B * EMB, 256)), dim3(256), 0, st, gl3, B, GOAL, g_, b_, goal_t, goal_st, emb, (long long)S * EMB, EMB, ppx);
                    ppx_packed = true;
                } else ln_fwd(gl3, GOAL, B, GOAL, g_, b_, goal_t, GOAL, nullptr, 0, goal_st);
            };
            if (b->is_lang) {
                hipLaunchKernelGGL((cast_kernel<float, T>), dim3(cdiv(B * LANG, 256)), dim3(256), 0, st, b->lang, lang_t, (long long)B * LANG);
// ... 260 lines not shown
```

### hulc_amd/csrc/iengine.h

```cpp
#pragma once
#include <hip/hip_runtime.h>
#include <cstring>
#include <map>
#include <string>
#include <vector>

#include "../../include/hulc_hip.h"
#include "comm.h"

void hulc_set_error(const char* fmt, ...);

struct IEngine {
    virtual ~IEngine() { delete comm; delete comm_pending; }
    virtual int bind(float* p, float* g, float* m, float* v, int64_t numel, int n, const char* const* names, const int64_t* offs,
                     const int64_t* numels) = 0;
    virtual int prepare_weights(bool shadow_fresh = false) = 0;
    virtual int zero_grads() = 0;
    virtual int flush_grads() = 0;
    virtual int forward(const hulc_batch* b, float lw, float cw, float* out, int on_host) = 0;
    virtual int forward_pair(const hulc_batch* vis, const hulc_batch* lang, float lw, float cw, float* out8, int on_host) = 0;
    virtual int backward(int part = -1) = 0;
    virtual int validate(const hulc_batch* b, const hulc_val_noise* nz, float* out17, int32_t* plan_pp_out, int32_t* plan_pr_out, float* pred_pp_out,
                         float* pred_pr_out) = 0;
    virtual int clip_gt_encode(const float* lang_emb, int m, int slot) = 0;
// ... 125 lines not shown
            js += buf; first = false;
            if (reset) { t.used = 0; t.flops = t.bytes = 0; t.launches = 0; }
        }
        js += "}";
        if ((int64_t)js.size() + 1 > cap) { hulc_set_error("hulc_timers_read: buffer too small"); return 1; }
        memcpy(out, js.c_str(), js.size() + 1);
        return 0;
    }
};

#define HULC_TU_DECLS                                                                                                                         \
    IEngine* make_engine(const hulc_config& cfg, int* rc);                                                                                   \
    int k_gemm_nt(int is_f32, const void* A, const void* B, float* C, int M, int N, int K, long long lda, long long ldb, long long ldc, \
                  const float* bias, int relu, void* stream);                                                                                \
    int k_spatial_softmax64(const void* f, int H, int W, int Nf, void* out, float* stats, const float* dout, void* df, void* stream);          \
    int k_enc_tail_fwd(int Nf, int ldemb, const hulc_enc_tail_job* a, const hulc_enc_tail_job* b, void* emb, const float* pos, int S,           \
                       float drop_p, unsigned long long seed, float* xf, void* xt, float* z0, float* z1, void* stream);                         \
    int k_enc_tail_bwd(int Nf, int ldemb, const hulc_enc_tail_bwd_job* a, const hulc_enc_tail_bwd_job* b, const float* demb, void* stream);     \
    int k_logistic_loss(int t16, int wide, const float* heads, int ldh, const float* actions, const float* robot_obs, int B, int S, int nmix,   \
                        int ndim, int num_classes, float log_scale_min, float gripper_alpha, int gripper_control, int discrete_gripper,         \
                        float grad_scale, const float* lscale, float* row_loss, float* a_tcp_out, void* dheads, void* stream);                  \
    int k_det_head_loss(int t16, const void* H1, const void* W, const float* bias, const float* actions, const float* robot_obs, int B, int S, int criterion,     \
                        int frame, float grad_scale, const float* lscale, float* row_loss, float* pred, float* dpre, void* stream);                              \
    int k_det_head_bwd(int t16, const float* dpre, const void* W, const void* H1, int B, int S, void* dH1, void* dZ1, float* dW, float* db, void* stream);        \
    int k_det_head_act(int t16, const void* h1, const void* W, const float* bias, const float* robot_obs, int n, float* out, void* stream);                       \
    int k_plan_kl_sample(const float* pr_logits, const float* pp_logits, int B, int NCAT, int NCLS, const int* idx_in, int* idx_out, float* probs,  \
                         float* kl_cat, float* dpp, float* dpr, float w_pp, float w_pr, unsigned long long seed, const float* lscale, void* stream); \
    int k_st_softmax_bwd(int t16, const float* probs, const float* dplan, const float* dpr_kl, const float* dpp_kl, int rows, int NCLS, float* out,  \
                         void* out_t, void* dpp_t, void* stream);                                                                               \
    int k_plan_gather(int t16, const void* w_t, const int* idx, int B, int NCAT, int NCLS, int H, const float* b1, const float* b2, float* out,   \
                      const void* emb, void* embg, int S, int W, const void* goal, int G, int grow0, void* cb, void* stream);                     \
    int k_plan_scatter_grad(int t16, int form, const void* dC, const int* idx, int B, int NCAT, int NCLS, int H, int KIN, float* dw, int store,   \
                            void* stream);                                                                                                      \
    int k_normal_kl_sample(int t16, const float* pr_state, const float* pp_state, int B, int n, const float* eps_in, float* eps_out, float* plan_f, \
                           void* plan_t, float* kl_elem, float* dpp, float* dpr, float w_pp, float w_pr, unsigned long long seed,                 \
                           const float* lscale, void* stream);                                                                                  \
    int k_normal_rsample_bwd(int t16, const float* dplan, const float* eps, const float* pr_state, const float* dpr_kl, int B, int n, void* out,  \
                             void* stream);                                                                                                     \
    int k_layernorm_fwd(int t16, const float* x, long long ldx, int rows, int n, const float* g, const float* b, void* out, long long ldo,        \
                        float* out_f32, long long ldf, float* stats, void* stream);                                                             \
    int k_layernorm_bwd(int t16, const float* dy, long long lddy, const float* x, long long ldx, const float* stats, const float* g, int rows,    \
                        int n, float* dx_f32, long long ldd, int accumulate, void* dx_t, long long ldt, float* dg, float* db, float drop_p,       \
                        unsigned long long seed, int bcast_rows, float bcast_div, int dy_parts, long long dy_part_stride, float* scratch,        \
                        void* stream);                                                                                                          \
    int k_layernorm_mean(int t16, const float* x, int B, int S, int n, const float* g, const float* b, float* stats, void* out, float* yout,      \
                         void* stream);                                                                                                         \
    int k_tr_layer_fwd(const hulc_tr_layer_job* j, int B, int S, int ln_in, float dp, void* stream);                                            \
    int k_tr_ffn_bwd(const hulc_tr_ffn_bwd_job* j, int B, int S, int bcast, float bdiv, float dp, void* stream);                                \
    int k_tr_attn_bwd(const hulc_tr_attn_bwd_job* j, int B, int S, int nparts, long long part_stride, float dp, void* stream);                  \
    int k_gemm_epi(int t16, const hulc_gemm_epi_job* j, int kernel, int* ran, void* stream);                                                    \
    int k_gemm_multi(int form, const hulc_gemm_epi_job* jobs, int n, int sh, int* ran, void* stream);                                           \
    int k_gemm_pick(int t16, int M, int N, int K, long long lda, long long ldb, int* pick, int* bk);                                            \
    int k_gemm_wgrad_nsplit(int t16, int M, int N, int K, int* nsplit, int* big);                                                               \
    int k_conv_wgrad(const char* who, int typed, int which, const void* X, const void* dY, float* out, float* db_out, int Nf, int IH, int* slabs, \
                     void* stream);                                                                                                             \
    int k_conv1_wgrad_u8(const char* who, int typed, const void* X, const int* shifts, int pad, const void* dY, float* dw_out, float* db_out,   \
                         int Nf, int IH, int form, int fold, int* slabs, void* stream);                                                         \
    int k_conv_tile(const char* who, int typed, int mode, const void* img, const void* w, const float* bias, const void* mask, void* out,       \
                    unsigned* bits1_out, int Nf, int IMH, int OUTH, int relu, int wgs, void* stream);                                           \
    int k_conv_pair(const char* who, int typed, int stage, const hulc_conv_job* a, const hulc_conv_job* b, int wg_a, int wg_b, int* slabs,      \
                    void* stream);                                                                                                              \
    int k_conv_plan(int form, int frames, int in_side, int out_side, int wgs, int* nbands, int* rows_per_band, int* frames_per_band, int* items);
namespace hulc_bf16 { HULC_TU_DECLS }
namespace hulc_f16 { HULC_TU_DECLS }
```

### hulc_amd/csrc/k_entries.h

```cpp
#pragma once
#include "iengine.h"
#include "kernels.h"
#include "enc_tail.h"
#include "plan_ln_launch.h"
#include "gemm.h"
#include "tr_fused.h"
#include "det_head.h"
#include <vector>

namespace HULC_NS {

static inline bool k_misaligned16(const void* p) { return (reinterpret_cast<uintptr_t>(p) & 15) != 0; }
static inline int k_launched(const char* who) {
    const hipError_t e = hipGetLastError();
    if (e != hipSuccess) { hulc_set_error("%s: launch failed: %s", who, hipGetErrorString(e)); return 1; }
    return 0;
}

int k_spatial_softmax64(const void* f, int H, int W, int Nf, void* out, float* stats, const float* dout, void* df, void* stream) {
    hipStream_t st = (hipStream_t)stream;
    if (Nf < 1 || H < 2 || W < 2 || (long long)H * W > (1 << 20)) { hulc_set_error("hulc_k_spatial_softmax64: Nf=%d H=%d W=%d (need Nf >= 1, H, W >= 2)", Nf, H, W); return 1; }
    if (!f || !stats || (dout ? !df : !out)) { hulc_set_error("hulc_k_spatial_softmax64: null argument"); return 1; }
    if (k_misaligned16(f) || k_misaligned16(stats) || k_misaligned16(dout) || k_misaligned16(df)) { hulc_set_error("hulc_k_spatial_softmax64: f, stats, dout, df must be 16-byte aligned"); return 1; }
    if (!dout) launch_spatial_softmax64_fwd(st, (const h16_t*)f, Nf, H, W, (h16_t*)out, stats);
// ... 506 lines not shown
        const hulc_gemm_epi_job& j = jobs[i];
        if (k_gemm_job_bad(who, i, &j, 2)) return 1;
        if (j.nsplit != 1 || j.z_stride != 0 || j.atomic || j.wfrag) { hulc_set_error("%s: job %d: nsplit = 1, z_stride = 0, no atomic, no wfrag", who, i); return 1; }
        a[i] = dense<h16_t>((const h16_t*)j.A, j.M, j.lda); b[i] = dense<h16_t>((const h16_t*)j.B, j.N, j.ldb); om[i] = k_gemm_job_om(j); ep[i] = k_gemm_job_epi(j);
    }
    const hulc_gemm_epi_job &j0 = jobs[0], &j1 = jobs[1];
    if (form == 0) {
        GemmGroupP g{};
        g.n = n;
        for (int i = 0; i < n; ++i) {
            if (!gemm_glds_ok(a[i], b[i], ep[i], jobs[i].M, jobs[i].N, jobs[i].K)) { hulc_set_error("%s: job %d: gemm_glds_ok refuses (K >= 64, K %% 32 == 0, rows 16-byte aligned)", who, i); return 1; }
            g.a[i] = a[i]; g.b[i] = b[i]; g.om[i] = om[i]; g.ep[i] = ep[i]; g.M[i] = jobs[i].M; g.N[i] = jobs[i].N; g.K[i] = jobs[i].K;
        }
        launch_gemm_glds_group(st, g);
        *ran = HULC_GEMM_RAN_GROUP;
        return k_launched(who);
    }
    if (j0.M != j1.M || j0.N != j1.N || j0.K != j1.K || j0.lda != j1.lda || j0.ldb != j1.ldb || j0.ldc != j1.ldc || j0.out_R1 != j1.out_R1 || j0.out_s0 != j1.out_s0) {
        hulc_set_error("%s: forms 1 and 2: the two jobs share M, N, K, the leading dimensions and the output map", who); return 1;
    }
    if (form == 1) {
        if (j0.A != j1.A) { hulc_set_error("%s: form 1: the two jobs share A", who); return 1; }
        if (!gemm_glds_pair_ok(a[0], b[0], b[1], ep[0], ep[1], j0.M, j0.N, j0.K, sh)) {
            hulc_set_error("%s: form 1: gemm_glds_pair_ok refuses (K >= 192, K, sh multiples of 64, 0 < sh < K, M, N multiples of 128, plain fp32 epilogues, 16-byte aligned)", who); return 1;
        }
        launch_gemm_glds_pair(st, a[0], b[0], b[1], om[0], ep[0], ep[1], j0.M, j0.N, j0.K, sh);
        *ran = HULC_GEMM_RAN_PAIR;
        return k_launched(who);
    }
    if (!skinny_use_lds || !skinny_lds_dual_ok(a[0].p, b[0].p, a[1].p, b[1].p, j0.lda, j0.ldb, j0.M, j0.N, j0.K)) {
        hulc_set_error("%s: form 2: shape not covered by the dual launch (32 < M <= 64, K = 2048, N %% 16 == 0, lda %% 64 == 0, A 128-byte aligned, W 16-byte aligned)", who); return 1;
    }
    if (!launch_skinny_lds_dual(st, a[0].p, b[0].p, ep[0], a[1].p, b[1].p, ep[1], j0.lda, j0.ldb, j0.M, j0.N, j0.K, om[0])) { hulc_set_error("%s: form 2: the launcher refused", who); return 1; }
    *ran = HULC_GEMM_RAN_DUAL;
    return k_launched(who);
}
int k_gemm_pick(int t16, int M, int N, int K, long long lda, long long ldb, int* pick, int* bk) {
    if (!pick || !bk || M < 1 || N < 1 || K < 1 || lda < K || ldb < K) { hulc_set_error("hulc_k_gemm_pick: null argument or bad shape"); return 1; }
    EpiP ep;
    GemmPick p;
    const void* al = (const void*)(uintptr_t)0x10000;
    if (t16) p = gemm_pick<h16_t>(dense<h16_t>((const h16_t*)al, M, lda), dense<h16_t>((const h16_t*)al, N, ldb), ep, M, N, K, gemm_use_glds);
    else p = gemm_pick<float>(dense<float>((const float*)al, M, lda), dense<float>((const float*)al, N, ldb), ep, M, N, K, gemm_use_glds);
    *pick = p == GEMM_PICK_SKINNY ? HULC_GEMM_RAN_SKINNY_ROUTER : p == GEMM_PICK_GLDS ? HULC_GEMM_RAN_GLDS : gemm_pick_tile(p) == 128 ? HULC_GEMM_RAN_128 : gemm_pick_tile(p) == 64 ? HULC_GEMM_RAN_64 : HULC_GEMM_RAN_32;
    *bk = (p == GEMM_PICK_SKINNY || p == GEMM_PICK_GLDS) ? 0 : (p == GEMM_PICK_64_BK128 || p == GEMM_PICK_32_BK128) ? 128 : p == GEMM_PICK_128_BK64 ? 64 : 32;
    return 0;
}
int k_gemm_wgrad_nsplit(int t16, int M, int N, int K, int* nsplit, int* big) {
    if (!nsplit || !big || M < 1 || N < 1 || K < 1) { hulc_set_error("hulc_k_gemm_wgrad_nsplit: null argument or bad shape"); return 1; }
    bool b = false;
    *nsplit = t16 ? gemm_wgrad_nsplit<h16_t>(M, N, K, &b) : gemm_wgrad_nsplit<float>(M, N, K, &b);
    *big = b ? 1 : 0;
    return 0;
}

static inline int k_conv_fwd_side(int in_side, int K, int S) { return in_side < K ? -1 : (in_side - K) / S + 1; }
static inline bool k_conv_mode_bench_only(int mode) { return mode == 12 || mode == 13 || mode == 18 || mode == 19; }
int k_conv_wgrad(const char* who, int typed, int which, const void* X, const void* dY, float* out, float* db_out, int Nf, int IH, int* slabs, void* stream) {
    hipStream_t st = (hipStream_t)stream;
    if (slabs) *slabs = 0;
    if (typed) {
        if (which < 1 || which > 3) { hulc_set_error("%s: which must be 1, 2 or 3", who); return 1; }
        const int KH = which == 3 ? 3 : (which == 2 ? 4 : 8);
        if (!X || !dY || !out || Nf < 1 || IH < KH || IH > 4096 || (long long)Nf * IH * IH * 64 >= (1ll << 31)) { hulc_set_error("%s: null argument, or Nf=%d, IH=%d out of range", who, Nf, IH); return 1; }
    }
    float* part = nullptr;
    static float* bias_tmp = nullptr;
    if (!bias_tmp && hipMalloc(&bias_tmp, sizeof(float) * 512 * 64) != hipSuccess) { hulc_set_error("%s: hipMalloc failed", who); return 1; }
    const int KC = which == 3 ? 576 : (which == 2 ? 512 : 192);
    const int CO = which == 1 ? 32 : 64;
    if (hipMalloc(&part, sizeof(float) * 512ll * 64 * KC) != hipSuccess) { hulc_set_error("%s: hipMalloc failed", who); return 1; }
    int ns;
    static h16_t* zp = nullptr;
    if (!zp) { if (hipMalloc(&zp, 256) != hipSuccess) { hulc_set_error("%s: hipMalloc failed", who); return 1; } hipMemset(zp, 0, 256); }
    if (db_out) hipMemsetAsync(bias_tmp, 0, sizeof(float) * 64, st);
    if (which == 3) { const int OH = IH - 2; ns = launch_conv_wgrad_tr<64, 64, 3, 3, 1>(st, (const h16_t*)X, (const h16_t*)dY, part, bias_tmp, Nf, IH, IH, OH, OH, 512, nullptr, zp); }
    else if (which == 2) { const int OH = (IH - 4) / 2 + 1; ns = launch_conv_wgrad_tr<32, 64, 4, 4, 2>(st, (const h16_t*)X, (const h16_t*)dY, part, bias_tmp, Nf, IH, IH, OH, OH, 512, nullptr, zp); }
    else if (which == 1) { const int OH = (IH - 8) / 4 + 1; ns = launch_conv1_wgrad_tr(st, Conv1Src{X, nullptr, 0, 0}, (const h16_t*)dY, part, bias_tmp, Nf, IH, IH, OH, OH, 512); }
    else { hipFree(part); hulc_set_error("%s: which must be 1, 2 or 3", who); return 1; }
    hipMemsetAsync(out, 0, sizeof(float) * CO * KC, st);
    hipLaunchKernelGGL(unpack_conv_wgrad_kernel, dim3((CO * KC + 1023) / 1024), dim3(256), 0, st, part, ns, (long long)CO * KC, out, CO, KC, 1, 1, 0);
    if (db_out) hipMemcpyAsync(db_out, bias_tmp, sizeof(float) * CO, hipMemcpyDeviceToDevice, st);
    hipError_t e = hipStreamSynchronize(st);
    hipFree(part);
    if (e != hipSuccess) { hulc_set_error("%s: %s", who, hipGetErrorString(e)); return 1; }
    if (slabs) *slabs = ns;
    return 0;
}

int k_conv1_wgrad_u8(const char* who, int typed, const void* X, const int* shifts, int pad, const void* dY, float* dw_out, float* db_out, int Nf, int IH, int form, int fold, int* slabs,
                     void* stream) {
    hipStream_t st = (hipStream_t)stream;
    if (slabs) *slabs = 0;
    if (form != 1 && form != 2) { hulc_set_error("%s: form must be 1 or 2 (got %d)", who, form); return 1; }
    if (typed) {
        if (form != 2) { hulc_set_error("%s: form %d is a bench-only form (the engine runs form 2)", who, form); return 1; }
        if (!X || !dY || !dw_out || !db_out || Nf < 1 || IH < 8 || IH > 4096 || pad < 0 || pad > CONV1_RAW_MARGIN) { hulc_set_error("%s: null argument, or Nf=%d, IH=%d, pad=%d out of range", who, Nf, IH, pad); return 1; }
    }
    float *part = nullptr, *bias = nullptr;
    if (hipMalloc(&part, sizeof(float) * 512ll * 32 * 192) != hipSuccess || hipMalloc(&bias, sizeof(float) * 64) != hipSuccess) { hulc_set_error("%s: hipMalloc failed", who); return 1; }
    hipMemsetAsync(bias, 0, sizeof(float) * 64, st);
    Conv1Src src{}; src.X = X; src.shift = shifts; src.u8 = 1; src.pad = pad; src.fold = fold != 0;
    const int OH = (IH - 8) / 4 + 1;
    const int keep = g_conv1_wgrad_u8reg;
    g_conv1_wgrad_u8reg = form;
    const int ns = launch_conv1_wgrad_tr(st, src, (const h16_t*)dY, part, bias, Nf, IH, IH, OH, OH, 512);
// ... 218 lines not shown
```

### hulc_amd/lib.py

```python
from __future__ import annotations

import ctypes as C
import os

_HERE = os.path.dirname(os.path.abspath(__file__))
LIB_PATH = os.path.join(_HERE, "csrc", "libhulc_hip.so")

KIND = {"hulc": 0, "gcbc": 1, "mcil": 2, "mcil_gru": 3}
DTYPE = {"fp32": 0, "bf16": 1, "fp16": 2}


class HulcConfig(C.Structure):
    _fields_ = [("kind", C.c_int32), ("dtype", C.c_int32), ("max_batch", C.c_int32), ("max_seq", C.c_int32),
                ("max_window", C.c_int32), ("use_clip", C.c_int32), ("kl_beta", C.c_float),
                ("kl_balancing_mix", C.c_float), ("dropout_p", C.c_float), ("num_classes", C.c_int32),
                ("gripper_alpha", C.c_float), ("log_scale_min", C.c_float), ("seed", C.c_uint64)]


class HulcBatch(C.Structure):
    _fields_ = [("B", C.c_int32), ("S", C.c_int32), ("is_lang", C.c_int32), ("rgb_static", C.c_void_p),
                ("rgb_gripper", C.c_void_p), ("actions", C.c_void_p), ("robot_obs", C.c_void_p), ("lang", C.c_void_p),
                ("plan_idx", C.c_void_p), ("aux_rows", C.c_void_p), ("n_aux", C.c_int32), ("step", C.c_uint64),
                ("frames_u8", C.c_int32), ("pad_static", C.c_int32), ("pad_gripper", C.c_int32), ("shift_static", C.c_void_p),
                ("shift_gripper", C.c_void_p), ("plan_eps", C.c_void_p), ("actions_absolute", C.c_int32), ("max_rel_pos", C.c_float),
# ... 41 lines not shown

class HulcConvJob(C.Structure):
    _fields_ = [("input", C.c_void_p), ("w", C.c_void_p), ("bias", C.c_void_p), ("out", C.c_void_p), ("bits", C.c_void_p),
                ("frames", C.c_int32), ("in_side", C.c_int32), ("out_side", C.c_int32)]


class HulcEncTailJob(C.Structure):
    _fields_ = [("x", C.c_void_p), ("W1", C.c_void_p), ("W2", C.c_void_p), ("b1", C.c_void_p), ("b2", C.c_void_p), ("lng", C.c_void_p), ("lnb", C.c_void_p),
                ("f1", C.c_void_p), ("f2", C.c_void_p), ("lnst", C.c_void_p), ("col0", C.c_int32)]


class HulcEncTailBwdJob(C.Structure):
    _fields_ = [("f2", C.c_void_p), ("lnst", C.c_void_p), ("lng", C.c_void_p), ("f1", C.c_void_p), ("W2t", C.c_void_p), ("W1t", C.c_void_p), ("xmask", C.c_void_p),
                ("dlng", C.c_void_p), ("dlnb", C.c_void_p), ("d_f2", C.c_void_p), ("d_f1", C.c_void_p), ("dx_f32", C.c_void_p), ("dx_t", C.c_void_p), ("col0", C.c_int32)]


class HulcTrLayerJob(C.Structure):
    _fields_ = [(n, C.c_void_p) for n in ("xin", "ln_g", "ln_b", "xf_out", "xt_out", "st_out", "Wqkv", "Wo", "W1", "W2", "bqkv", "bo", "b1", "b2", "n1g", "n1b",
                                          "qkv", "Pat", "ao", "y1", "st1", "x1t", "x1f", "hff", "y2")] + \
               [(n, C.c_uint64) for n in ("seed_att", "seed_o", "seed_h", "seed_y")]


class HulcTrFfnBwdJob(C.Structure):
    _fields_ = [(n, C.c_void_p) for n in ("dx", "y2", "st2", "n2g", "dg2", "db2", "W2t", "W1t", "hff", "dt_c", "dt_a", "part")] + [("seed_y", C.c_uint64)]


class HulcTrAttnBwdJob(C.Structure):
    _fields_ = [(n, C.c_void_p) for n in ("parts", "y1", "st1", "n1g", "dg1", "db1", "Wot", "Wint", "qkv", "Pat", "b_d", "b_b", "dy_f", "dx")] + \
               [("seed_o", C.c_uint64), ("seed_att", C.c_uint64)]


class HulcGemmEpiJob(C.Structure):
    _fields_ = [("A", C.c_void_p), ("B", C.c_void_p), ("M", C.c_int32), ("N", C.c_int32), ("K", C.c_int32), ("lda", C.c_int64), ("ldb", C.c_int64),
                ("ldc", C.c_int64), ("out_R1", C.c_int32), ("out_s0", C.c_int64), ("nsplit", C.c_int32), ("wfrag", C.c_int32),
                ("out", C.c_void_p), ("out_f32", C.c_int32), ("accumulate", C.c_int32), ("atomic", C.c_int32), ("z_stride", C.c_int64),
                ("bias", C.c_void_p), ("bias2", C.c_void_p), ("res", C.c_void_p), ("res_f32", C.c_int32), ("res_ld", C.c_int64), ("res_rowmod", C.c_int32),
                ("res_late", C.c_int32), ("mask", C.c_void_p), ("mask_tanh", C.c_int32), ("relu", C.c_int32), ("alpha", C.c_float), ("drop_p", C.c_float),
                ("drop_seed", C.c_uint64), ("out2", C.c_void_p), ("out2_lo", C.c_int64), ("out2_hi", C.c_int64), ("out2_mask", C.c_void_p),
                ("out2_relu", C.c_int32), ("generic_only", C.c_int32)]


GEMM_RAN = {"none": 0, "32": 1, "64": 2, "128": 3, "glds": 4, "skinny_router": 5, "skinny_reg": 6, "kchunk": 7, "splitk_64": 8, "splitk_128": 9, "group": 10, "pair": 11,
            "dual": 12}

EXPORTS = ["hulc_last_error", "hulc_ctx_create", "hulc_ctx_destroy", "hulc_set_stream", "hulc_workspace_bytes",
           "hulc_bind_params", "hulc_prepare_weights", "hulc_zero_grads", "hulc_flush_grads", "hulc_forward_loss", "hulc_forward_loss_pair", "hulc_backward", "hulc_backward_part",
           "hulc_adam_step", "hulc_optimizer_step", "hulc_comm_unique_id", "hulc_comm_prepare", "hulc_comm_init", "hulc_comm_destroy", "hulc_comm_buckets", "hulc_comm_stats", "hulc_comm_size", "hulc_comm_timeline", "hulc_allreduce_grads", "hulc_backward_allreduce", "hulc_scaler_enable", "hulc_scaler_get", "hulc_scaler_set", "hulc_grad_clip_set", "hulc_grad_norm_get", "hulc_validate", "hulc_store_gather", "hulc_store_stage", "hulc_store_stage_join", "hulc_store_stage_stats", "hulc_clip_gt_encode", "hulc_clip_gt_scores", "hulc_aux_heads_enable", "hulc_decoder_select", "hulc_aux_weights_set", "hulc_aux_losses_get", "hulc_rollout_reset", "hulc_rollout_plan", "hulc_rollout_act", "hulc_rollout_get_goal", "hulc_rollout_set_state", "hulc_rollout_envs_init", "hulc_rollout_envs_reset", "hulc_rollout_envs_plan", "hulc_rollout_envs_act", "hulc_rollout_envs_get_state", "hulc_rollout_envs_set_state", "hulc_sbert_create", "hulc_sbert_destroy", "hulc_sbert_set_stream", "hulc_sbert_bind", "hulc_sbert_encode", "hulc_set_kl_beta", "hulc_set_dropout", "hulc_set_option", "hulc_get_option", "hulc_timers_enable", "hulc_timers_read", "hulc_get_tensor", "hulc_get_plan_idx", "hulc_k_gemm_nt", "hulc_k_cast", "hulc_k_trread_probe", "hulc_k_conv_wgrad", "hulc_k_conv1_wgrad_u8", "hulc_k_conv1_interior_groups", "hulc_k_conv_tile", "hulc_k_camera_split", "hulc_k_conv_pair", "hulc_k_skinny", "hulc_k_attention", "hulc_k_rnn_persist", "hulc_k_rnn_persist_flag_words", "hulc_k_clip_loss", "hulc_k_clip_loss_fp32", "hulc_k_mia_head", "hulc_k_cosine_dist", "hulc_k_spatial_softmax64", "hulc_k_enc_tail_fwd", "hulc_k_enc_tail_bwd", "hulc_k_logistic_loss",
           "hulc_k_plan_kl_sample", "hulc_k_st_softmax_bwd", "hulc_k_plan_gather", "hulc_k_plan_scatter_grad", "hulc_k_normal_kl_sample", "hulc_k_normal_rsample_bwd",
           "hulc_k_layernorm_fwd", "hulc_k_layernorm_bwd", "hulc_k_layernorm_mean", "hulc_k_tr_layer_fwd", "hulc_k_tr_ffn_bwd", "hulc_k_tr_attn_bwd",
           "hulc_k_window_compact", "hulc_k_rows_expand", "hulc_k_rows_reduce", "hulc_k_gemm_epi", "hulc_k_gemm_multi", "hulc_k_gemm_pick", "hulc_k_gemm_wgrad_nsplit",
           "hulc_k_det_head_loss", "hulc_k_det_head_bwd", "hulc_k_det_head_act",
           "hulc_k_conv_wgrad_t", "hulc_k_conv1_wgrad_u8_t", "hulc_k_conv_tile_t", "hulc_k_conv_pair_t", "hulc_k_conv_plan",
           "hulc_decoder_body_select", "hulc_trainable_set", "hulc_trainable_get", "hulc_trainable_steps_set",
           "hulc_ema_enable", "hulc_ema_state_get", "hulc_ema_state_set", "hulc_ema_swap", "hulc_ema_swapped", "hulc_k_ema_update"]

_lib = None


def load():
    global _lib
    if _lib is not None:
        return _lib
    path = os.environ.get("HULC_LIB_PATH") or LIB_PATH
    if not os.path.exists(path):
        raise RuntimeError(f"hulc_amd: {path} not built — run `python -c 'import __graft_entry__ as g; g.build()'`; "
                           "there is no CPU fallback for the product path")
    import torch
    lib = C.CDLL(path)
    lib.hulc_last_error.restype = C.c_char_p
    lib.hulc_workspace_bytes.restype = C.c_int64
    lib.hulc_ctx_create.argtypes = [C.POINTER(HulcConfig), C.POINTER(C.c_void_p)]
    lib.hulc_ctx_destroy.argtypes = [C.c_void_p]
    lib.hulc_set_stream.argtypes = [C.c_void_p, C.c_void_p]
    lib.hulc_workspace_bytes.argtypes = [C.c_void_p]
    lib.hulc_bind_params.argtypes = [C.c_void_p, C.c_void_p, C.c_void_p, C.c_void_p, C.c_void_p, C.c_int64, C.c_int32,
                                     C.POINTER(C.c_char_p), C.POINTER(C.c_int64), C.POINTER(C.c_int64)]
    lib.hulc_prepare_weights.argtypes = [C.c_void_p]
    lib.hulc_zero_grads.argtypes = [C.c_void_p]
    if os.environ.get("HULC_LIB_PATH") and not hasattr(lib, "hulc_flush_grads"):
        lib.hulc_zero_grads.argtypes = [C.c_void_p]
    else:
        lib.hulc_flush_grads.argtypes = [C.c_void_p]
    lib.hulc_forward_loss.argtypes = [C.c_void_p, C.POINTER(HulcBatch), C.c_float, C.c_float, C.c_void_p, C.c_int32]
    lib.hulc_forward_loss_pair.argtypes = [C.c_void_p, C.POINTER(HulcBatch), C.POINTER(HulcBatch), C.c_float, C.c_float, C.c_void_p, C.c_int32]
    lib.hulc_backward.argtypes = [C.c_void_p]
    lib.hulc_backward_part.argtypes = [C.c_void_p, C.c_int32]
    lib.hulc_adam_step.argtypes = [C.c_void_p, C.c_float, C.c_float, C.c_float, C.c_float, C.c_int64, C.c_float]
    lib.hulc_optimizer_step.argtypes = [C.c_void_p, C.POINTER(HulcOptim)]
    lib.hulc_comm_unique_id.argtypes = [C.c_void_p, C.c_int64]
    lib.hulc_comm_prepare.argtypes = [C.c_void_p]
    lib.hulc_comm_init.argtypes = [C.c_void_p, C.c_void_p, C.c_int32, C.c_int32]
    lib.hulc_comm_destroy.argtypes = [C.c_void_p]
    lib.hulc_comm_buckets.argtypes = [C.c_void_p, C.POINTER(C.c_int64), C.POINTER(C.c_int64), C.c_int32]
    lib.hulc_comm_stats.argtypes = [C.c_void_p, C.POINTER(C.c_int64), C.POINTER(C.c_double)]
    if hasattr(lib, "hulc_comm_size") or not os.environ.get("HULC_LIB_PATH"):
        lib.hulc_comm_size.argtypes = [C.c_void_p, C.POINTER(C.c_int32), C.POINTER(C.c_int32)]
    lib.hulc_comm_timeline.argtypes = [C.c_void_p, C.POINTER(C.c_double), C.c_int32, C.POINTER(C.c_double)]
    lib.hulc_allreduce_grads.argtypes = [C.c_void_p, C.c_int32]
    lib.hulc_backward_allreduce.argtypes = [C.c_void_p, C.c_int32]
    lib.hulc_scaler_enable.argtypes = [C.c_void_p, C.c_float, C.c_float, C.c_float, C.c_int32]
    lib.hulc_scaler_get.argtypes = [C.c_void_p, C.POINTER(C.c_float), C.POINTER(C.c_int32), C.POINTER(C.c_int64), C.POINTER(C.c_int32), C.POINTER(C.c_int64)]
    lib.hulc_scaler_set.argtypes = [C.c_void_p, C.c_float, C.c_int32, C.c_int64]
    if hasattr(lib, "hulc_grad_clip_set") or not os.environ.get("HULC_LIB_PATH"):
        lib.hulc_grad_clip_set.argtypes = [C.c_void_p, C.c_int32, C.c_float, C.c_int32]
        lib.hulc_grad_norm_get.argtypes = [C.c_void_p, C.POINTER(C.c_float), C.POINTER(C.c_float), C.c_void_p, C.c_int64]
    lib.hulc_clip_gt_encode.argtypes = [C.c_void_p, C.c_void_p, C.c_int32, C.c_int32]
    lib.hulc_clip_gt_scores.argtypes = [C.c_void_p, C.c_int32, C.c_void_p, C.c_int64, C.POINTER(C.c_int32), C.POINTER(C.c_int32)]
# ... 40 lines not shown
                                   C.c_int64, C.c_int64, C.c_void_p, C.c_int32, C.c_void_p]
    lib.hulc_k_conv_wgrad.argtypes = [C.c_int32, C.c_void_p, C.c_void_p, C.c_void_p, C.c_int32, C.c_int32, C.c_void_p]
    if hasattr(lib, "hulc_k_conv1_wgrad_u8") or not os.environ.get("HULC_LIB_PATH"):
        lib.hulc_k_conv1_interior_groups.argtypes = [C.c_int32, C.c_int32, C.c_int32, C.POINTER(C.c_int32), C.POINTER(C.c_int32)]
        lib.hulc_k_conv1_wgrad_u8.argtypes = [C.c_void_p, C.c_void_p, C.c_int32, C.c_void_p, C.c_void_p, C.c_void_p, C.c_int32, C.c_int32, C.c_int32, C.c_int32, C.c_void_p]
    lib.hulc_k_conv_tile.argtypes = [C.c_int32, C.c_void_p, C.c_void_p, C.c_void_p, C.c_void_p, C.c_void_p, C.c_int32, C.c_int32, C.c_int32,
                                     C.c_int32, C.c_void_p]
    if hasattr(lib, "hulc_k_conv_pair") or not os.environ.get("HULC_LIB_PATH"):
        lib.hulc_k_camera_split.argtypes = [C.c_int32, C.c_double, C.c_double, C.POINTER(C.c_int32), C.POINTER(C.c_int32)]
        lib.hulc_k_conv_pair.argtypes = [C.c_int32, C.POINTER(HulcConvJob), C.POINTER(HulcConvJob), C.c_int32, C.c_int32, C.c_void_p]
    lib.hulc_k_skinny.argtypes = [C.c_void_p, C.c_void_p, C.c_void_p, C.c_int32, C.c_int32, C.c_int32, C.c_int32, C.c_void_p]
    lib.hulc_k_trread_probe.argtypes = [C.c_void_p, C.c_void_p, C.c_void_p]
    lib.hulc_k_cast.argtypes = [C.c_int32, C.c_void_p, C.c_void_p, C.c_int64, C.c_void_p]
    if hasattr(lib, "hulc_k_clip_loss") or not os.environ.get("HULC_LIB_PATH"):
        for f in (lib.hulc_k_clip_loss, lib.hulc_k_clip_loss_fp32):
            f.argtypes = [C.c_void_p, C.c_void_p, C.c_int32, C.c_void_p, C.c_float, C.c_void_p, C.c_void_p, C.c_void_p, C.c_void_p, C.c_void_p]
        lib.hulc_k_mia_head.argtypes = [C.c_void_p, C.c_void_p, C.c_int32, C.c_void_p, C.c_void_p, C.c_void_p, C.c_void_p, C.c_float, C.c_void_p, C.c_void_p, C.c_void_p,
                                        C.c_int32, C.c_void_p, C.c_void_p, C.c_void_p, C.c_void_p, C.c_void_p]
        lib.hulc_k_cosine_dist.argtypes = [C.c_void_p, C.c_void_p, C.c_int32, C.c_int32, C.c_float, C.c_void_p, C.c_void_p, C.c_void_p]
    lib.hulc_k_attention.argtypes = [C.c_int32, C.c_void_p, C.c_void_p, C.c_void_p, C.c_void_p, C.c_void_p, C.c_int32, C.c_int32, C.c_float, C.c_uint64, C.c_void_p]
    if hasattr(lib, "hulc_k_enc_tail_fwd") or not os.environ.get("HULC_LIB_PATH"):
        lib.hulc_k_spatial_softmax64.argtypes = [C.c_int32, C.c_void_p, C.c_int32, C.c_int32, C.c_int32, C.c_void_p, C.c_void_p, C.c_void_p, C.c_void_p, C.c_void_p]
        lib.hulc_k_enc_tail_fwd.argtypes = [C.c_int32, C.c_int32, C.c_int32, C.POINTER(HulcEncTailJob), C.POINTER(HulcEncTailJob), C.c_void_p, C.c_void_p, C.c_int32,
                                            C.c_float, C.c_uint64, C.c_void_p, C.c_void_p, C.c_void_p, C.c_void_p, C.c_void_p]
        lib.hulc_k_enc_tail_bwd.argtypes = [C.c_int32, C.c_int32, C.c_int32, C.POINTER(HulcEncTailBwdJob), C.POINTER(HulcEncTailBwdJob), C.c_void_p, C.c_void_p]
        lib.hulc_k_logistic_loss.argtypes = [C.c_int32, C.c_int32, C.c_void_p, C.c_int32, C.c_void_p, C.c_void_p, C.c_int32, C.c_int32, C.c_int32, C.c_int32, C.c_int32,
                                             C.c_float, C.c_float, C.c_int32, C.c_int32, C.c_float, C.c_void_p, C.c_void_p, C.c_void_p, C.c_void_p, C.c_void_p]
    if hasattr(lib, "hulc_k_layernorm_bwd") or not os.environ.get("HULC_LIB_PATH"):
        P, I, F, U, Q = C.c_void_p, C.c_int32, C.c_float, C.c_uint64, C.c_int64
        lib.hulc_k_plan_kl_sample.argtypes = [P, P, I, I, I, P, P, P, P, P, P, F, F, U, P, P]
        lib.hulc_k_st_softmax_bwd.argtypes = [I, P, P, P, P, I, I, P, P, P, P]
        lib.hulc_k_plan_gather.argtypes = [I, P, P, I, I, I, I, P, P, P, P, P, I, I, P, I, I, P, P]
        lib.hulc_k_plan_scatter_grad.argtypes = [I, I, P, P, I, I, I, I, I, P, I, P]
        lib.hulc_k_normal_kl_sample.argtypes = [I, P, P, I, I, P, P, P, P, P, P, P, F, F, U, P, P]
        lib.hulc_k_normal_rsample_bwd.argtypes = [I, P, P, P, P, I, I, P, P]
        lib.hulc_k_layernorm_fwd.argtypes = [I, P, Q, I, I, P, P, P, Q, P, Q, P, P]
        lib.hulc_k_layernorm_bwd.argtypes = [I, P, Q, P, Q, P, P, I, I, P, Q, I, P, Q, P, P, F, U, I, F, I, Q, P, P]
        lib.hulc_k_layernorm_mean.argtypes = [I, P, I, I, I, P, P, P, P, P, P]
    if hasattr(lib, "hulc_k_tr_layer_fwd") or not os.environ.get("HULC_LIB_PATH"):
        lib.hulc_k_tr_layer_fwd.argtypes = [C.c_int32, C.POINTER(HulcTrLayerJob), C.c_int32, C.c_int32, C.c_int32, C.c_float, C.c_void_p]
        lib.hulc_k_tr_ffn_bwd.argtypes = [C.c_int32, C.POINTER(HulcTrFfnBwdJob), C.c_int32, C.c_int32, C.c_int32, C.c_float, C.c_float, C.c_void_p]
        lib.hulc_k_tr_attn_bwd.argtypes = [C.c_int32, C.POINTER(HulcTrAttnBwdJob), C.c_int32, C.c_int32, C.c_int32, C.c_int64, C.c_float, C.c_void_p]
    if hasattr(lib, "hulc_k_rows_reduce") or not os.environ.get("HULC_LIB_PATH"):
        P, I, Q = C.c_void_p, C.c_int32, C.c_int64
        lib.hulc_k_window_compact.argtypes = [P, P, P, I, I, I, Q, P, P, P, P, P, P]
        lib.hulc_k_rows_expand.argtypes = [I, P, P, P, I, I, I, P, P]
        lib.hulc_k_rows_reduce.argtypes = [P, P, P, I, I, I, P, P]
    if hasattr(lib, "hulc_k_gemm_epi") or not os.environ.get("HULC_LIB_PATH"):
        I, Q, PI = C.c_int32, C.c_int64, C.POINTER(C.c_int32)
        lib.hulc_k_gemm_epi.argtypes = [I, C.POINTER(HulcGemmEpiJob), I, PI, C.c_void_p]
        lib.hulc_k_gemm_multi.argtypes = [I, I, C.POINTER(HulcGemmEpiJob), I, I, PI, C.c_void_p]
        lib.hulc_k_gemm_pick.argtypes = [I, I, I, I, Q, Q, PI, PI]
        lib.hulc_k_gemm_wgrad_nsplit.argtypes = [I, I, I, I, PI, PI]
    if hasattr(lib, "hulc_decoder_select") or not os.environ.get("HULC_LIB_PATH"):
        P, I, F = C.c_void_p, C.c_int32, C.c_float
        lib.hulc_decoder_select.argtypes = [P, I, I]
        lib.hulc_k_det_head_loss.argtypes = [I, P, P, P, P, P, I, I, I, I, F, P, P, P, P, P]
        lib.hulc_k_det_head_bwd.argtypes = [I, P, P, P, I, I, P, P, P, P, P]
        lib.hulc_k_det_head_act.argtypes = [I, P, P, P, P, I, P, P]
    if hasattr(lib, "hulc_decoder_body_select") or not os.environ.get("HULC_LIB_PATH"):
        lib.hulc_decoder_body_select.argtypes = [C.c_void_p, C.c_int32]
    if hasattr(lib, "hulc_trainable_set") or not os.environ.get("HULC_LIB_PATH"):
        lib.hulc_trainable_set.argtypes = [C.c_void_p, C.c_int32, C.c_void_p]
        lib.hulc_trainable_get.argtypes = [C.c_void_p, C.c_int64, C.c_void_p, C.c_void_p]
        lib.hulc_trainable_steps_set.argtypes = [C.c_void_p, C.c_int32, C.c_void_p, C.c_int64]
    if hasattr(lib, "hulc_ema_enable") or not os.environ.get("HULC_LIB_PATH"):
        lib.hulc_ema_enable.argtypes = [C.c_void_p, C.c_void_p, C.c_float, C.c_int64, C.c_int32]
        lib.hulc_ema_state_get.argtypes = [C.c_void_p, C.POINTER(C.c_int64), C.POINTER(C.c_float)]
        lib.hulc_ema_state_set.argtypes = [C.c_void_p, C.c_int64]
        lib.hulc_ema_swap.argtypes = [C.c_void_p]
        lib.hulc_ema_swapped.argtypes = [C.c_void_p, C.POINTER(C.c_int32)]
        lib.hulc_k_ema_update.argtypes = [C.c_void_p, C.c_void_p, C.c_int64, C.c_float, C.c_void_p, C.c_void_p, C.c_int32, C.c_void_p]
    if hasattr(lib, "hulc_k_conv_plan") or not os.environ.get("HULC_LIB_PATH"):
        P, I, PI = C.c_void_p, C.c_int32, C.POINTER(C.c_int32)
        lib.hulc_k_conv_wgrad_t.argtypes = [I, I, P, P, P, P, I, I, PI, P]
        lib.hulc_k_conv1_wgrad_u8_t.argtypes = [I, P, P, I, P, P, P, I, I, I, I, PI, P]
        lib.hulc_k_conv_tile_t.argtypes = [I, I, P, P, P, P, P, P, I, I, I, I, I, P]
        lib.hulc_k_conv_pair_t.argtypes = [I, I, C.POINTER(HulcConvJob), C.POINTER(HulcConvJob), I, I, PI, P]
        lib.hulc_k_conv_plan.argtypes = [I, I, I, I, I, PI, PI, PI, PI]
    _lib = lib
    return lib


def check(rc: int):
    if rc != 0:
        raise RuntimeError("libhulc_hip: " + load().hulc_last_error().decode("utf-8", "replace"))
```

### include/hulc_hip.h

```cpp
#ifndef HULC_HIP_H
#define HULC_HIP_H
#include <stdint.h>

#ifdef __cplusplus
extern "C" {
#endif

typedef struct hulc_ctx hulc_ctx;

enum { HULC_KIND_HULC = 0, HULC_KIND_GCBC = 1, HULC_KIND_MCIL = 2, HULC_KIND_MCIL_GRU = 3 };
enum { HULC_DTYPE_F32 = 0, HULC_DTYPE_BF16 = 1, HULC_DTYPE_F16 = 2 };

typedef struct hulc_config {
    int32_t kind;
    int32_t dtype;
    int32_t max_batch;
    int32_t max_seq;
    int32_t max_window;
    int32_t use_clip;
    float kl_beta;
    float kl_balancing_mix;
    float dropout_p;
    int32_t num_classes;
    float gripper_alpha;
// ... 267 lines not shown
int hulc_k_normal_rsample_bwd(int32_t dtype, const float* dplan, const float* eps, const float* pr_state, const float* dpr_kl, int32_t B, int32_t n, void* out,
                              void* hip_stream);
int hulc_k_layernorm_fwd(int32_t dtype, const float* x, int64_t ldx, int32_t rows, int32_t n, const float* g, const float* b, void* out, int64_t ldo, float* out_f32,
                         int64_t ldf, float* stats, void* hip_stream);
int hulc_k_layernorm_bwd(int32_t dtype, const float* dy, int64_t lddy, const float* x, int64_t ldx, const float* stats, const float* g, int32_t rows, int32_t n, float* dx_f32,
                         int64_t ldd, int32_t accumulate, void* dx_t, int64_t ldt, float* dg, float* db, float drop_p, uint64_t seed, int32_t bcast_rows, float bcast_div,
                         int32_t dy_parts, int64_t dy_part_stride, float* scratch, void* hip_stream);
int hulc_k_layernorm_mean(int32_t dtype, const float* x, int32_t B, int32_t S, int32_t n, const float* g, const float* b, float* stats, void* out, float* yout,
                          void* hip_stream);
int hulc_k_window_compact(const int64_t* window_start, const int32_t* lens, const int32_t* off, int32_t off_base, int32_t B, int32_t S, int64_t store_frames,
                          const int32_t* shift_static, const int32_t* shift_gripper, int64_t* frame_out, int32_t* shift_static_out, int32_t* shift_gripper_out,
                          void* hip_stream);
int hulc_k_rows_expand(int32_t elem_bytes, const void* src, const int32_t* lens, const int32_t* off, int32_t B, int32_t S, int32_t n, void* dst, void* hip_stream);
int hulc_k_rows_reduce(const float* src, const int32_t* lens, const int32_t* off, int32_t B, int32_t S, int32_t n, float* dst, void* hip_stream);
int hulc_k_ema_update(float* ema, const float* p, int64_t n, float w, const int64_t* chunk_start, const int32_t* chunk_n, int32_t chunks, void* hip_stream);

typedef struct hulc_tr_layer_job {
    const float* xin; const float* ln_g; const float* ln_b; float* xf_out; void* xt_out; float* st_out;
    const void* Wqkv; const void* Wo; const void* W1; const void* W2;
    const float* bqkv; const float* bo; const float* b1; const float* b2; const float* n1g; const float* n1b;
    void* qkv; float* Pat; void* ao; float* y1; float* st1; void* x1t; float* x1f; void* hff; float* y2;
    uint64_t seed_att, seed_o, seed_h, seed_y;
} hulc_tr_layer_job;
int hulc_k_tr_layer_fwd(int32_t dtype, const hulc_tr_layer_job* job, int32_t B, int32_t S, int32_t ln_in, float dp, void* hip_stream);
typedef struct hulc_tr_ffn_bwd_job {
    const float* dx; const float* y2; const float* st2; const float* n2g; float* dg2; float* db2;
    const void* W2t; const void* W1t; const void* hff; void* dt_c; void* dt_a; float* part;
    uint64_t seed_y;
} hulc_tr_ffn_bwd_job;
int hulc_k_tr_ffn_bwd(int32_t dtype, const hulc_tr_ffn_bwd_job* job, int32_t B, int32_t S, int32_t bcast, float bdiv, float dp, void* hip_stream);
typedef struct hulc_tr_attn_bwd_job {
    const float* parts; const float* y1; const float* st1; const float* n1g; float* dg1; float* db1;
    const void* Wot; const void* Wint; const void* qkv; const float* Pat; void* b_d; void* b_b; float* dy_f; float* dx;
    uint64_t seed_o, seed_att;
} hulc_tr_attn_bwd_job;
int hulc_k_tr_attn_bwd(int32_t dtype, const hulc_tr_attn_bwd_job* job, int32_t B, int32_t S, int32_t nparts, int64_t part_stride, float dp, void* hip_stream);

typedef struct hulc_gemm_epi_job {
    const void* A; const void* B; int32_t M, N, K; int64_t lda, ldb;
    int64_t ldc; int32_t out_R1; int64_t out_s0;
    int32_t nsplit, wfrag;
    void* out; int32_t out_f32, accumulate, atomic; int64_t z_stride;
    const float* bias; const float* bias2;
    const void* res; int32_t res_f32; int64_t res_ld; int32_t res_rowmod, res_late;
    const void* mask; int32_t mask_tanh, relu; float alpha, drop_p; uint64_t drop_seed;
    void* out2; int64_t out2_lo, out2_hi; const void* out2_mask; int32_t out2_relu, generic_only;
} hulc_gemm_epi_job;
enum { HULC_GEMM_RAN_NONE = 0, HULC_GEMM_RAN_32 = 1, HULC_GEMM_RAN_64 = 2, HULC_GEMM_RAN_128 = 3, HULC_GEMM_RAN_GLDS = 4, HULC_GEMM_RAN_SKINNY_ROUTER = 5, HULC_GEMM_RAN_SKINNY_REG = 6,
       HULC_GEMM_RAN_KCHUNK = 7, HULC_GEMM_RAN_SPLITK_64 = 8, HULC_GEMM_RAN_SPLITK_128 = 9, HULC_GEMM_RAN_GROUP = 10, HULC_GEMM_RAN_PAIR = 11, HULC_GEMM_RAN_DUAL = 12 };
int hulc_k_gemm_epi(int32_t dtype, const hulc_gemm_epi_job* job, int32_t kernel, int32_t* ran, void* hip_stream);
int hulc_k_gemm_multi(int32_t dtype, int32_t form, const hulc_gemm_epi_job* jobs, int32_t n, int32_t sh, int32_t* ran, void* hip_stream);
int hulc_k_gemm_pick(int32_t dtype, int32_t M, int32_t N, int32_t K, int64_t lda, int64_t ldb, int32_t* pick, int32_t* bk);
int hulc_k_gemm_wgrad_nsplit(int32_t dtype, int32_t M, int32_t N, int32_t K, int32_t* nsplit, int32_t* big);

#ifdef __cplusplus
}
#endif
#endif
```

Measured before the change: 21410 windows/s.

## Add streamed DMA-pipelined linear weight-grad kernel and queue small-M MLP wgrads

Adds a new linear weight-gradient kernel that streams dY and X tiles into a three-stage LDS ring via direct-to-LDS DMA with swizzled layouts, split-K across M with slab reduction. Small-M MLP backward no longer launches its own batched wgrad kernel; jobs are queued (wq_add) into a larger batch of up to 32 jobs so more wgrads share one launch, with multiple gradient buffer sets. The encoder tail split count now comes from a new heuristic. The aim is to hide global-load latency and cut launch count, at the cost of added complexity and possible alignment constraints.

```diff
diff --git a/hulc_amd/csrc/capi.hip b/hulc_amd/csrc/capi.hip
--- a/hulc_amd/csrc/capi.hip
+++ b/hulc_amd/csrc/capi.hip
@@ -392,6 +392,10 @@
 }
 int hulc_k_gemm_multi(int32_t dtype, int32_t form, const hulc_gemm_epi_job* jobs, int32_t n, int32_t sh, int32_t* ran, void* stream) {
     HULC_K_16BIT("hulc_k_gemm_multi", k_gemm_multi(form, jobs, n, sh, ran, stream));
+}
+int hulc_k_lin_bwd_stream(int32_t dtype, const void* dY, const void* X, int64_t ldx, int32_t M, int32_t N, int32_t K, int32_t nsplit, int32_t store, float* dW, int64_t lddw,
+                          float* db, float* slabs, void* stream) {
+    HULC_K_16BIT("hulc_k_lin_bwd_stream", k_lin_bwd_stream(dY, X, (long long)ldx, M, N, K, nsplit, store, dW, (long long)lddw, db, slabs, stream));
 }
 #undef HULC_K_16BIT
 int hulc_k_gemm_epi(int32_t dtype, const hulc_gemm_epi_job* job, int32_t kernel, int32_t* ran, void* stream) {
diff --git a/hulc_amd/csrc/conv_wgrad.h b/hulc_amd/csrc/conv_wgrad.h
--- a/hulc_amd/csrc/conv_wgrad.h
+++ b/hulc_amd/csrc/conv_wgrad.h
@@ -1623,90 +1623,11 @@
     return launch_conv1_wgrad_jobs(st, &q, 1, max_blocks, nullptr, &ns) ? ns : 0;
 }
 
-DEVI void lin_bwd_smallm_body(const h16_t* __restrict__ dY, long long ldy, const h16_t* __restrict__ X, long long ldx,
-                              int M, int N, int K, float* __restrict__ dW, long long lddw, float* __restrict__ db,
-                              float* __restrict__ db2, int mchunk, int store, const int bx, const int by, const int bz, const int gz, char* smem,
-                              const bool slabs = false) {
-    constexpr int TN = 64, TK = 128, YS = TN * 2 + 16, XS = TK * 2 + 16;
-    lds_char* yimg = (lds_char*)smem;
-    lds_char* ximg = yimg + 64 * YS;
+DEVI void lin_bwd_tile_out(const f32x4 (&acc)[8], const float4 (&oldw)[8], const bool vec_ok, const bool atomic, const int store, float* __restrict__ dW, const long long lddw,
+                           const int N, const int K, const int (&r0)[2], const int (&c0)[2], char* smem) {
     const int tid = threadIdx.x, lane = tid & 63, wave = tid >> 6;
-    const int n0 = bx * TN, k0 = by * TK;
-    const int mbeg = bz * mchunk, mend = min(M, mbeg + mchunk);
     const int g = lane >> 4, a = lane & 15;
-    const int prow = a >> 2, ccol = (a & 3) * 8;
-    f32x4 acc[8];
-#pragma unroll
-    for (int j = 0; j < 8; ++j) acc[j] = f32x4{0.f, 0.f, 0.f, 0.f};
-    float bsum = 0.f;
-    const bool atomic_b = gz > 1;
-    const bool atomic = atomic_b && !slabs;
-    const int n = n0 + wave * 16 + a;
-    const bool vec_ok = !atomic && (lddw & 3) == 0 && ((reinterpret_cast<uintptr_t>(dW) & 15) == 0) && k0 + TK <= K;
     const int orow = lane >> 4, ocol = (lane & 15) * 4;
-    float4 oldw[8];
-    if (vec_ok) {
-#pragma unroll
-        for (int j = 0; j < 8; ++j) {
-            const int nr = n0 + wave * 16 + (j & 3) * 4 + orow;
-            oldw[j] = (store || nr >= N) ? make_float4(0.f, 0.f, 0.f, 0.f) : *reinterpret_cast<const float4*>(dW + (long long)nr * lddw + k0 + (j >> 2) * 64 + ocol);
-        }
-    }
-    u32x4_t ry[2], rx[4];
-    auto fetch = [&](int m0) {
-#pragma unroll
-        for (int u = 0; u < 2; ++u) {
-            const int i = tid + u * 256, m = i / (TN / 8), c = i % (TN / 8);
-            h16_t v[8];
-            if (m0 + m < mend && n0 + c * 8 < N) load8_guard<h16_t>(dY + (long long)(m0 + m) * ldy + n0 + c * 8, N - (n0 + c * 8), v);
-            else zero8<h16_t>(v);
-            ry[u] = *reinterpret_cast<const u32x4_t*>(v);
-        }
-#pragma unroll
-        for (int u = 0; u < 4; ++u) {
-            const int i = tid + u * 256, m = i / (TK / 8), c = i % (TK / 8);
-            h16_t v[8];
-            if (m0 + m < mend && k0 + c * 8 < K) load8_guard<h16_t>(X + (long long)(m0 + m) * ldx + k0 + c * 8, K - (k0 + c * 8), v);
-            else zero8<h16_t>(v);
-            rx[u] = *reinterpret_cast<const u32x4_t*>(v);
-        }
-    };
-    fetch(mbeg);
-    for (int m0 = mbeg; m0 < mend; m0 += 64) {
-        if (m0 > mbeg) __syncthreads();
-#pragma unroll
-        for (int u = 0; u < 2; ++u) { const int i = tid + u * 256; *(lds_u32x4*)(yimg + (i / (TN / 8)) * YS + (i % (TN / 8)) * 16) = ry[u]; }
-#pragma unroll
-        for (int u = 0; u < 4; ++u) { const int i = tid + u * 256; *(lds_u32x4*)(ximg + (i / (TK / 8)) * XS + (i % (TK / 8)) * 16) = rx[u]; }
-        __syncthreads();
-        if (m0 + 64 < mend) fetch(m0 + 64);
-#pragma unroll
-        for (int ms = 0; ms < 2; ++ms) {
-            const int mrow = ms * 32 + g * 8 + prow;
-            lds_char* yb = yimg + mrow * YS + wave * 32 + ccol;
-            const h16x8_t yf = tr_read8(yb, yb + 4 * YS);
-#pragma unroll
-            for (int j = 0; j < 8; ++j) {
-                lds_char* xb = ximg + mrow * XS + j * 32 + ccol;
-                const h16x8_t xf = tr_read8(xb, xb + 4 * XS);
-                acc[j] = MFMA_16x16x32_H(xf, yf, acc[j], 0, 0, 0);
-            }
-        }
-        if (db && by == 0) {
-#pragma unroll 16
-            for (int m = 0; m < 16; ++m) bsum += h2f(*(__attribute__((address_space(3))) h16_t*)(yimg + (wave * 16 + m) * YS + lane * 2));
-        }
-    }
-    if (db && by == 0) {
-        __syncthreads();
-        *(__attribute__((address_space(3))) float*)(yimg + (wave * 64 + lane) * 4) = bsum;
-        __syncthreads();
-        if (tid < TN) {
-            bsum = 0.f;
-#pragma unroll
-            for (int w = 0; w < 4; ++w) bsum += *(__attribute__((address_space(3))) float*)(yimg + (w * 64 + tid) * 4);
-        }
-    }
     if (vec_ok) {
         constexpr int OP = 64 * 4 + 16;
         __syncthreads();
@@ -1718,16 +1639,17 @@
 #pragma unroll
             for (int it = 0; it < 4; ++it) {
                 const f32x4 v = *(__attribute__((address_space(3))) f32x4*)(tb + (it * 4 + orow) * OP + ocol * 4);
-                const int nr = n0 + wave * 16 + it * 4 + orow;
+                const int nr = r0[h] + it * 4 + orow;
                 float4 o = oldw[h * 4 + it];
                 o.x += v[0]; o.y += v[1]; o.z += v[2]; o.w += v[3];
-                if (nr < N) *reinterpret_cast<float4*>(dW + (long long)nr * lddw + k0 + h * 64 + ocol) = o;
-            }
-        }
-    } else if (n < N) {
+                if (nr < N) *reinterpret_cast<float4*>(dW + (long long)nr * lddw + c0[h] + ocol) = o;
+            }
+        }
+    } else {
 #pragma unroll
         for (int j = 0; j < 8; ++j) {
-            const int k = k0 + j * 16 + g * 4;
+            const int n = r0[j >> 2] + a, k = c0[j >> 2] + (j & 3) * 16 + g * 4;
+            if (n >= N) continue;
             float* p = dW + (long long)n * lddw + k;
             if (atomic) {
 #pragma unroll
@@ -1744,30 +1666,267 @@
             }
         }
     }
-    if (db && by == 0 && tid < TN && n0 + tid < N) {
-        if (atomic_b) { unsafeAtomicAdd(db + n0 + tid, bsum); if (db2) unsafeAtomicAdd(db2 + n0 + tid, bsum); }
-        else { db[n0 + tid] += bsum; if (db2) db2[n0 + tid] += bsum; }
-    }
+}
+
+DEVI void lin_bwd_smallm_body(const h16_t* __restrict__ dY, long long ldy, const h16_t* __restrict__ X, long long ldx,
+                              int M, int N, int K, float* __restrict__ dW, long long lddw, float* __restrict__ db,
+                              float* __restrict__ db2, int store, const int bx, const int by, char* smem) {
+    constexpr int TN = 64, TK = 128, YS = TN * 2 + 16, XS = TK * 2 + 16;
+    lds_char* yimg = (lds_char*)smem;
+    lds_char* ximg = yimg + 64 * YS;
+    const int tid = threadIdx.x, lane = tid & 63, wave = tid >> 6;
+    const int n0 = bx * TN, k0 = by * TK;
+    const int g = lane >> 4, a = lane & 15;
+    const int prow = a >> 2, ccol = (a & 3) * 8;
+    f32x4 acc[8];
+#pragma unroll
+    for (int j = 0; j < 8; ++j) acc[j] = f32x4{0.f, 0.f, 0.f, 0.f};
+    float bsum = 0.f;
+    const bool vec_ok = (lddw & 3) == 0 && ((reinterpret_cast<uintptr_t>(dW) & 15) == 0) && k0 + TK <= K;
+    const int orow = lane >> 4, ocol = (lane & 15) * 4;
+    float4 oldw[8];
+    if (vec_ok) {
+#pragma unroll
+        for (int j = 0; j < 8; ++j) {
+            const int nr = n0 + wave * 16 + (j & 3) * 4 + orow;
+            oldw[j] = (store || nr >= N) ? make_float4(0.f, 0.f, 0.f, 0.f) : *reinterpret_cast<const float4*>(dW + (long long)nr * lddw + k0 + (j >> 2) * 64 + ocol);
+        }
+    }
+    u32x4_t ry[2], rx[4];
+    auto fetch = [&](int m0) {
+#pragma unroll
+        for (int u = 0; u < 2; ++u) {
+            const int i = tid + u * 256, m = i / (TN / 8), c = i % (TN / 8);
+            h16_t v[8];
+            if (m0 + m < M && n0 + c * 8 < N) load8_guard<h16_t>(dY + (long long)(m0 + m) * ldy + n0 + c * 8, N - (n0 + c * 8), v);
+            else zero8<h16_t>(v);
+            ry[u] = *reinterpret_cast<const u32x4_t*>(v);
+        }
+#pragma unroll
+        for (int u = 0; u < 4; ++u) {
+            const int i = tid + u * 256, m = i / (TK / 8), c = i % (TK / 8);
+            h16_t v[8];
+            if (m0 + m < M && k0 + c * 8 < K) load8_guard<h16_t>(X + (long long)(m0 + m) * ldx + k0 + c * 8, K - (k0 + c * 8), v);
+            else zero8<h16_t>(v);
+            rx[u] = *reinterpret_cast<const u32x4_t*>(v);
+        }
+    };
+    fetch(0);
+    for (int m0 = 0; m0 < M; m0 += 64) {
+        if (m0 > 0) __syncthreads();
+#pragma unroll
+        for (int u = 0; u < 2; ++u) { const int i = tid + u * 256; *(lds_u32x4*)(yimg + (i / (TN / 8)) * YS + (i % (TN / 8)) * 16) = ry[u]; }
+#pragma unroll
+        for (int u = 0; u < 4; ++u) { const int i = tid + u * 256; *(lds_u32x4*)(ximg + (i / (TK / 8)) * XS + (i % (TK / 8)) * 16) = rx[u]; }
+        __syncthreads();
+        if (m0 + 64 < M) fetch(m0 + 64);
+#pragma unroll
+        for (int ms = 0; ms < 2; ++ms) {
+            const int mrow = ms * 32 + g * 8 + prow;
+            lds_char* yb = yimg + mrow * YS + wave * 32 + ccol;
+            const h16x8_t yf = tr_read8(yb, yb + 4 * YS);
+#pragma unroll
+            for (int j = 0; j < 8; ++j) {
+                lds_char* xb = ximg + mrow * XS + j * 32 + ccol;
+                const h16x8_t xf = tr_read8(xb, xb + 4 * XS);
+                acc[j] = MFMA_16x16x32_H(xf, yf, acc[j], 0, 0, 0);
+            }
+        }
+        if (db && by == 0) {
+#pragma unroll 16
+            for (int m = 0; m < 16; ++m) bsum += h2f(*(__attribute__((address_space(3))) h16_t*)(yimg + (wave * 16 + m) * YS + lane * 2));
+        }
+    }
+    if (db && by == 0) {
+        __syncthreads();
+        *(__attribute__((address_space(3))) float*)(yimg + (wave * 64 + lane) * 4) = bsum;
+        __syncthreads();
+        if (tid < TN) {
+            bsum = 0.f;
+#pragma unroll
+            for (int w = 0; w < 4; ++w) bsum += *(__attribute__((address_space(3))) float*)(yimg + (w * 64 + tid) * 4);
+        }
+    }
+    const int r0[2] = {n0 + wave * 16, n0 + wave * 16}, c0[2] = {k0, k0 + 64};
+    lin_bwd_tile_out(acc, oldw, vec_ok, false, store, dW, lddw, N, K, r0, c0, smem);
+    if (db && by == 0 && tid < TN && n0 + tid < N) { db[n0 + tid] += bsum; if (db2) db2[n0 + tid] += bsum; }
 }
 
 constexpr int LBS_LDS = 64 * (64 * 2 + 16) + 64 * (128 * 2 + 16);
 __global__ void __launch_bounds__(256) lin_bwd_smallm_kernel(const h16_t* __restrict__ dY, long long ldy, const h16_t* __restrict__ X, long long ldx,
                                                              int M, int N, int K, float* __restrict__ dW, long long lddw, float* __restrict__ db,
-                                                             float* __restrict__ db2, int mchunk, int store = 0) {
+                                                             float* __restrict__ db2, int store = 0) {
     __shared__ __attribute__((aligned(16))) char smem[LBS_LDS];
-    lin_bwd_smallm_body(dY, ldy, X, ldx, M, N, K, dW, lddw, db, db2, mchunk, store, blockIdx.x, blockIdx.y, blockIdx.z, gridDim.z, smem);
-}
-struct LinBwdJob { const h16_t* dY; const h16_t* X; float* dW; float* db; long long ldx, lddw; int N, K, nx, blk0; float* part; };
-struct LinBwdBatch { LinBwdJob j[8]; int n, M, store, mchunk; };
+    lin_bwd_smallm_body(dY, ldy, X, ldx, M, N, K, dW, lddw, db, db2, store, blockIdx.x, blockIdx.y, smem);
+}
+struct LinBwdJob { const h16_t* dY; const h16_t* X; float* dW; float* db; long long ldx, lddw; int M, N, K, nx, blk0, store; };
+constexpr int LBS_MAX_JOBS = 32;
+struct LinBwdBatch { LinBwdJob j[LBS_MAX_JOBS]; int n; };
 __global__ void __launch_bounds__(256) lin_bwd_smallm_batched_kernel(LinBwdBatch bt) {
     __shared__ __attribute__((aligned(16))) char smem[LBS_LDS];
     int k = 0;
     while (k + 1 < bt.n && (int)blockIdx.x >= bt.j[k + 1].blk0) ++k;
     const LinBwdJob J = bt.j[k];
     const int b = blockIdx.x - J.blk0;
-    const bool slabs = bt.mchunk > 0 && J.part;
-    lin_bwd_smallm_body(J.dY, (long long)J.N, J.X, J.ldx, bt.M, J.N, J.K, slabs ? J.part + (long long)blockIdx.y * J.N * J.K : J.dW, slabs ? (long long)J.K : J.lddw, J.db, nullptr,
-                        bt.mchunk > 0 ? bt.mchunk : 64, slabs ? 1 : bt.store, b % J.nx, b / J.nx, blockIdx.y, gridDim.y, smem, slabs);
-}
-
-}
+    lin_bwd_smallm_body(J.dY, (long long)J.N, J.X, J.ldx, J.M, J.N, J.K, J.dW, J.lddw, J.db, nullptr, J.store, b % J.nx, b / J.nx, smem);
+}
+
+constexpr int LBT_NST = 3, LBT_YB = 64 * 128, LBT_STAGE = LBT_YB + 64 * 256, LBT_LDS = LBT_NST * LBT_STAGE;
+__device__ __attribute__((aligned(16))) unsigned int lbt_zero16[4] = {0u, 0u, 0u, 0u};
+DEVI int lbt_swy(int row) { return (((row >> 1) & 1) | (((row >> 3) & 1) << 1)) << 1; }
+DEVI int lbt_swx(int row) { return ((row & 7) << 1) ^ (row & 8); }
+DEVI void lin_bwd_stream_body(const h16_t* __restrict__ dY, long long ldy, const h16_t* __restrict__ X, long long ldx, const int mbeg, const int mend, const int N, const int K,
+                              float* __restrict__ dW, long long lddw, float* __restrict__ db, const int store, const bool atomic, const bool atomic_b, const int bx, const int by,
+                              char* smem) {
+    lds_char* const ring = (lds_char*)smem;
+    const int tid = threadIdx.x, lane = tid & 63, wave = tid >> 6;
+    const int n0 = bx * 64, k0 = by * 128;
+    const int g = lane >> 4, a = lane & 15;
+    const int prow = a >> 2, ccol = (a & 3) * 8;
+    f32x4 acc[8];
+#pragma unroll
+    for (int j = 0; j < 8; ++j) acc[j] = f32x4{0.f, 0.f, 0.f, 0.f};
+    float bsum = 0.f;
+    const bool vec_ok = !atomic && (lddw & 3) == 0 && ((reinterpret_cast<uintptr_t>(dW) & 15) == 0) && k0 + 128 <= K;
+    const int orow = lane >> 4, ocol = (lane & 15) * 4;
+    const int wn = wave & 1, wk = wave >> 1;
+    const int r0[2] = {n0 + wn * 32, n0 + wn * 32 + 16}, c0[2] = {k0 + wk * 64, k0 + wk * 64};
+    float4 oldw[8];
+    if (vec_ok) {
+#pragma unroll
+        for (int j = 0; j < 8; ++j) {
+            const int nr = r0[j >> 2] + (j & 3) * 4 + orow;
+            oldw[j] = (store || nr >= N) ? make_float4(0.f, 0.f, 0.f, 0.f) : *reinterpret_cast<const float4*>(dW + (long long)nr * lddw + c0[j >> 2] + ocol);
+        }
+    }
+    const h16_t* src[6];
+    int srow[6], scol[6];
+    unsigned full = 0, part = 0;
+#pragma unroll
+    for (int u = 0; u < 6; ++u) {
+        const bool y = u < 2;
+        const int row = y ? (wave * 2 + u) * 8 + (lane >> 3) : (wave * 4 + u - 2) * 4 + (lane >> 4);
+        const int slot = y ? (lane & 7) : (lane & 15);
+        const int c = slot ^ (y ? lbt_swy(row) : lbt_swx(row));
+        const int col = (y ? n0 : k0) + c * 8, lim = y ? N : K;
+        srow[u] = row; scol[u] = col;
+        src[u] = (y ? dY : X) + (long long)row * (y ? ldy : ldx) + col;
+        if (col + 8 <= lim) full |= 1u << u;
+        else if (col < lim) part |= 1u << u;
+    }
+    const bool any_part = __any((int)part) != 0;
+    const int nk = mend > mbeg ? (mend - mbeg + 63) >> 6 : 0;
+    auto issue = [&](int kt, int buf) {
+        const int m0 = mbeg + kt * 64;
+        lds_char* const st = ring + buf * LBT_STAGE;
+#pragma unroll
+        for (int u = 0; u < 6; ++u) {
+            const bool ok = ((full >> u) & 1u) && m0 + srow[u] < mend;
+            const void* s = ok ? (const void*)(src[u] + (long long)m0 * (u < 2 ? ldy : ldx)) : (const void*)lbt_zero16;
+            lds_dma16(s, (unsigned)(size_t)(st + (u < 2 ? (wave * 2 + u) * 1024 : LBT_YB + (wave * 4 + u - 2) * 1024)));
+        }
+    };
+    auto patch = [&](int kt, int buf) {
+        const int m0 = mbeg + kt * 64;
+        lds_char* const st = ring + buf * LBT_STAGE;
+#pragma unroll
+        for (int u = 0; u < 6; ++u) {
+            if (!((part >> u) & 1u) || m0 + srow[u] >= mend) continue;
+            const h16_t* s = src[u] + (long long)m0 * (u < 2 ? ldy : ldx);
+            lds_char* d = st + (u < 2 ? (wave * 2 + u) * 1024 : LBT_YB + (wave * 4 + u - 2) * 1024) + lane * 16;
+            const int nv = (u < 2 ? N : K) - scol[u];
+#pragma unroll
+            for (int e = 0; e < 7; ++e)
+                if (e < nv) *(__attribute__((address_space(3))) h16_t*)(d + e * 2) = s[e];
+        }
+    };
+#pragma unroll
+    for (int j = 0; j < LBT_NST - 1; ++j)
+        if (j < nk) issue(j, j);
+    int buf = 0;
+#pragma unroll 1
+    for (int kt = 0; kt < nk; ++kt) {
+        static_assert(LBT_NST == 3, "one counted wait per number of younger stages in flight: 0 or 1");
+        if (nk - 1 - kt >= 1) asm volatile("s_waitcnt vmcnt(6)" ::: "memory");
+        else asm volatile("s_waitcnt vmcnt(0)" ::: "memory");
+        if (any_part) patch(kt, buf);
+        asm volatile("s_waitcnt lgkmcnt(0)\n\ts_barrier" ::: "memory");
+        if (kt + LBT_NST - 1 < nk) issue(kt + LBT_NST - 1, buf == 0 ? LBT_NST - 1 : buf - 1);
+        lds_char* const yimg = ring + buf * LBT_STAGE;
+        lds_char* const ximg = yimg + LBT_YB;
+#pragma unroll
+        for (int ms = 0; ms < 2; ++ms) {
+            const int mrow = ms * 32 + g * 8 + prow;
+            const int sy = lbt_swy(mrow), sx = lbt_swx(mrow);
+            h16x8_t yf[2], xf[4];
+#pragma unroll
+            for (int i = 0; i < 2; ++i) {
+                lds_char* yb = yimg + mrow * 128 + (((wn * 4 + i * 2 + (ccol >> 4)) ^ sy) << 4) + (ccol & 15);
+                yf[i] = tr_read8(yb, yb + 4 * 128);
+            }
+#pragma unroll
+            for (int jj = 0; jj < 4; ++jj) {
+                const int c = wk * 8 + jj * 2 + (ccol >> 4);
+                xf[jj] = tr_read8(ximg + mrow * 256 + ((c ^ sx) << 4) + (ccol & 15), ximg + (mrow + 4) * 256 + ((c ^ sx ^ 8) << 4) + (ccol & 15));
+            }
+#pragma unroll
+            for (int i = 0; i < 2; ++i)
+#pragma unroll
+                for (int jj = 0; jj < 4; ++jj) acc[i * 4 + jj] = MFMA_16x16x32_H(xf[jj], yf[i], acc[i * 4 + jj], 0, 0, 0);
+        }
+        if (db && by == 0) {
+#pragma unroll 16
+            for (int m = 0; m < 16; ++m) {
+                const int r = wave * 16 + m;
+                bsum += h2f(*(__attribute__((address_space(3))) h16_t*)(yimg + r * 128 + (((lane >> 3) ^ lbt_swy(r)) << 4) + (lane & 7) * 2));
+            }
+        }
+        buf = buf == LBT_NST - 1 ? 0 : buf + 1;
+    }
+    if (db && by == 0) {
+        __syncthreads();
+        *(__attribute__((address_space(3))) float*)(ring + (wave * 64 + lane) * 4) = bsum;
+        __syncthreads();
+        if (tid < 64) {
+            bsum = 0.f;
+#pragma unroll
+            for (int w = 0; w < 4; ++w) bsum += *(__attribute__((address_space(3))) float*)(ring + (w * 64 + tid) * 4);
+        }
+    }
+    lin_bwd_tile_out(acc, oldw, vec_ok, atomic, store, dW, lddw, N, K, r0, c0, smem);
+    if (db && by == 0 && tid < 64 && n0 + tid < N) {
+        if (atomic_b) unsafeAtomicAdd(db + n0 + tid, bsum);
+        else db[n0 + tid] += bsum;
+    }
+}
+struct LinStreamJob { const h16_t* dY; const h16_t* X; float* dW; float* db; float* part; long long ldx, lddw; int M, N, K, nx, blk0, nsplit, mchunk, store; };
+constexpr int LBT_MAX_JOBS = 32;
+struct LinStreamBatch { LinStreamJob j[LBT_MAX_JOBS]; int n; };
+__global__ void __launch_bounds__(256) lin_bwd_stream_kernel(LinStreamBatch bt) {
+    extern __shared__ __attribute__((aligned(16))) char lbt_smem[];
+    int k = 0;
+    while (k + 1 < bt.n && (int)blockIdx.x >= bt.j[k + 1].blk0) ++k;
+    const LinStreamJob J = bt.j[k];
+    const int tiles = J.nx * ((J.K + 127) >> 7);
+    const int b = blockIdx.x - J.blk0, z = b / tiles, t = b % tiles;
+    const int mbeg = z * J.mchunk, mend = min(J.M, mbeg + J.mchunk);
+    lin_bwd_stream_body(J.dY, (long long)J.N, J.X, J.ldx, mbeg, mend, J.N, J.K, J.part ? J.part + (long long)z * J.N * J.K : J.dW, J.part ? (long long)J.K : J.lddw, J.db,
+                        J.part ? 1 : J.store, !J.part && J.nsplit > 1, J.nsplit > 1, t % J.nx, t / J.nx, lbt_smem);
+}
+static inline bool lin_stream_ok(const void* dY, const void* X, long long ldx, int N) { return (N & 3) == 0 && (ldx & 3) == 0 && (((uintptr_t)dY | (uintptr_t)X) & 7) == 0; }
+static inline int lin_stream_add(LinStreamBatch& bt, int& blocks, const h16_t* dY, const h16_t* X, long long ldx, int M, int N, int K, float* dW, long long lddw, float* db,
+                                 float* part, int nsplit, int store) {
+    LinStreamJob& J = bt.j[bt.n++];
+    J.dY = dY; J.X = X; J.dW = dW; J.db = db; J.part = part; J.ldx = ldx; J.lddw = lddw; J.M = M; J.N = N; J.K = K; J.nx = (N + 63) / 64; J.blk0 = blocks;
+    J.nsplit = nsplit; J.mchunk = ((M + nsplit - 1) / nsplit + 63) / 64 * 64; J.store = store;
+    const int wg = J.nx * ((K + 127) / 128) * nsplit;
+    blocks += wg;
+    return wg;
+}
+static inline void launch_lin_stream(hipStream_t st, const LinStreamBatch& bt, int blocks) {
+    static bool attr = false;
+    if (!attr) { hipFuncSetAttribute((const void*)lin_bwd_stream_kernel, hipFuncAttributeMaxDynamicSharedMemorySize, LBT_LDS); attr = true; }
+    if (bt.n > 0 && blocks > 0) hipLaunchKernelGGL(lin_bwd_stream_kernel, dim3(blocks), dim3(256), LBT_LDS, st, bt);
+}
+
+}
diff --git a/hulc_amd/csrc/engine.h b/hulc_amd/csrc/engine.h
--- a/hulc_amd/csrc/engine.h
+++ b/hulc_amd/csrc/engine.h
@@ -737,7 +737,7 @@
     void lin_wgrad(const T* dY, const T* X, long long ldx, int M, int N, int K, float* dW, long long lddw, float* db, float* db2 = nullptr) {
         if constexpr (std::is_same<T, h16_t>::value) {
             if (M <= 64) {
-                hipLaunchKernelGGL(lin_bwd_smallm_kernel, dim3(cdiv(N, 64), cdiv(K, 128)), dim3(256), 0, st, dY, (long long)N, X, ldx, M, N, K, dW, lddw, db, db2, 64, grad_first(dW) ? 1 : 0);
+                hipLaunchKernelGGL(lin_bwd_smallm_kernel, dim3(cdiv(N, 64), cdiv(K, 128)), dim3(256), 0, st, dY, (long long)N, X, ldx, M, N, K, dW, lddw, db, db2, grad_first(dW) ? 1 : 0);
                 return;
             }
             grad_ensure_zero(dW);
@@ -810,35 +810,55 @@
         return 0;
     }
     T *trb_c[2] = {nullptr, nullptr}, *trb_a[2] = {nullptr, nullptr}, *trb_d[2] = {nullptr, nullptr}, *trb_b[2] = {nullptr, nullptr};
-    LinBwdBatch tr_wjobs{};
-    int tr_wblocks = 0;
-    void tr_wgrad_add(const T* dY, const T* X, const LinW& L) {
+    struct WqJob { const T* dY; const T* X; long long ldx, lddw; int M, N, K; float* dW; float* db; bool heads; };
+    std::vector<WqJob> wq;
+    static int lin_stream_nsplit(int tiles, int M) { return (M > 256 && tiles < 128) ? 2 : 1; }
+    bool wq_small(int M) const { return std::is_same<T, h16_t>::value && M <= 64; }
+    void wq_add(const T* dY, const T* X, long long ldx, int M, int N, int K, float* dW, long long lddw, float* db, bool heads = false) {
+        wq.push_back(WqJob{dY, X, ldx, lddw, M, N, K, dW, db, heads});
+    }
+    void wq_add(const T* dY, const T* X, int M, const LinW& L) {
         if constexpr (std::is_same<T, h16_t>::value) {
-            LinBwdJob& J = tr_wjobs.j[tr_wjobs.n++];
-            J.dY = dY; J.X = X; J.dW = L.dW; J.db = L.db; J.ldx = L.K; J.lddw = L.K; J.N = L.N; J.K = L.K; J.nx = cdiv(L.N, 64); J.blk0 = tr_wblocks; J.part = nullptr;
-            tr_wblocks += J.nx * cdiv(L.K, 128);
-        }
-    }
-    void tr_wgrads_flush(int M) {
+            if (M <= 64 || lin_stream_ok(dY, X, L.K, L.N)) { wq_add(dY, X, L.K, M, L.N, L.K, L.dW, L.K, L.db); return; }
+        }
+        lin_wgrad(dY, X, L.K, M, L.N, L.K, L.dW, L.K, L.db);
+    }
+    void wq_flush() {
         if constexpr (std::is_same<T, h16_t>::value) {
-            if (tr_wjobs.n == 0) return;
-            const int chunk = 256, nz = cdiv(M, chunk);
-            tr_wjobs.M = M; tr_wjobs.store = 0; tr_wjobs.mchunk = chunk;
-            UnpackBatch ub{};
-            int64_t cur = 0; int ublocks = 0;
-            for (int i = 0; i < tr_wjobs.n; ++i) {
-                LinBwdJob& J = tr_wjobs.j[i];
-                const int64_t need = (int64_t)nz * J.N * J.K;
-                if (part_cur + cur + need > this->partcap) { J.part = nullptr; continue; }
-                J.part = this->part + part_cur + cur; cur += need;
-                UnpackJob& U = ub.j[ub.n++];
-                U.part = J.part; U.grad = J.dW; U.slab = (long long)J.N * J.K; U.nsplit = nz; U.O = J.N; U.I = J.K; U.KH = U.KW = 1; U.nhwc = 0; U.blk0 = ublocks; U.ysplit = 1;
-                ublocks += cdiv(J.N * J.K, 1024);
-            }
-            if (nz > 1) nd(ND_LIN_BWD_ROWS);
-            hipLaunchKernelGGL(lin_bwd_smallm_batched_kernel, dim3(tr_wblocks, nz), dim3(256), 0, st, tr_wjobs);
-            if (ub.n > 0) hipLaunchKernelGGL(unpack_conv_wgrad_batched_kernel, dim3(ublocks, 1), dim3(256), 0, st, ub);
-            tr_wjobs.n = 0; tr_wblocks = 0;
+            if (wq.empty()) return;
+            int tiles = 0;
+            for (const WqJob& q : wq) if (q.M > 64) tiles += cdiv(q.N, 64) * cdiv(q.K, 128);
+            LinBwdBatch ob{}; int oblk = 0;
+            LinStreamBatch sb{}; int sblk = 0;
+            auto run_one = [&]() { if (ob.n) hipLaunchKernelGGL(lin_bwd_smallm_batched_kernel, dim3(oblk), dim3(256), 0, st, ob); ob.n = 0; oblk = 0; };
+            auto run_str = [&]() { launch_lin_stream(st, sb, sblk); sb.n = 0; sblk = 0; };
+            const WqJob* hj = nullptr; int hsplit = 1; bool hcolsum = false;
+            for (const WqJob& q : wq) {
+                if (q.M <= 64) {
+                    if (ob.n == LBS_MAX_JOBS) run_one();
+                    LinBwdJob& J = ob.j[ob.n++];
+                    J.dY = q.dY; J.X = q.X; J.dW = q.dW; J.db = q.db; J.ldx = q.ldx; J.lddw = q.lddw; J.M = q.M; J.N = q.N; J.K = q.K; J.nx = cdiv(q.N, 64); J.blk0 = oblk;
+                    J.store = grad_first(q.dW) ? 1 : 0;
+                    oblk += J.nx * cdiv(q.K, 128);
+                    continue;
+                }
+                if (sb.n == LBT_MAX_JOBS) run_str();
+                if (q.heads) {
+                    hj = &q; hsplit = lin_stream_nsplit(tiles, q.M);
+                    if (part_cur + (int64_t)hsplit * q.N * q.K > this->partcap) hsplit = 1;
+                    hcolsum = repro && hsplit > 1;
+                    if (hsplit > 1 && !repro) nd(ND_LIN_BWD_ROWS);
+                    lin_stream_add(sb, sblk, (const h16_t*)q.dY, (const h16_t*)q.X, q.ldx, q.M, q.N, q.K, nullptr, q.lddw, hcolsum ? nullptr : q.db, this->part + part_cur, hsplit, 1);
+                } else lin_stream_add(sb, sblk, (const h16_t*)q.dY, (const h16_t*)q.X, q.ldx, q.M, q.N, q.K, q.dW, q.lddw, q.db, nullptr, 1, grad_first(q.dW) ? 1 : 0);
+            }
+            run_one(); run_str();
+            if (hj) {
+                if (hcolsum) colsum(hj->dY, hj->N, hj->M, hj->N, hj->db);
+                const HeadPack hp = head_pack();
+                const int rows = head_rows[0] + head_rows[1] + head_rows[2] + head_rows[3];
+                hipLaunchKernelGGL(unpack_heads_grad_kernel, dim3(cdiv((long long)rows * HID, 256)), dim3(256), 0, st, hp, (const float*)(this->part + part_cur), (const float*)hj->db, HID, hsplit, (long long)hj->N * hj->K);
+            }
+            wq.clear();
         }
     }
     float* dparts = nullptr;
diff --git a/hulc_amd/csrc/engine_backward.inc b/hulc_amd/csrc/engine_backward.inc
--- a/hulc_amd/csrc/engine_backward.inc
+++ b/hulc_amd/csrc/engine_backward.inc
@@ -97,6 +97,7 @@
     }
     int bucket_ready(int i) {
         if (ar_dtype < 0 || (ar_sent >> i) & 1u) return 0;
+        wq_flush();
         const std::vector<Bucket> v = bucket_plan();
         ar_sent |= 1u << i;
         if (range_all_frozen(v[i].lo, v[i].hi)) return (i == 4 && !ar_voted) ? vote_only() : 0;
@@ -180,6 +181,7 @@
         if (!arena_clean) HIP_CHECK(hipMemsetAsync(zero_arena, 0, sizeof(float) * zero_n, st));
         arena_clean = false;
         work_ctr_next = 0;
+        wq.clear(); mlp_dy_next = 0;
         if (poison_partials) HIP_CHECK(hipMemsetAsync(this->part, 0xFF, sizeof(float) * (size_t)this->partcap, st));
         {
         bool have_dseq = false, dseq_cast_done = false;
@@ -227,16 +229,8 @@
                 const T* const hx = mlp ? Zx1 : H1;
                 bool slabs = false;
                 if constexpr (std::is_same<T, h16_t>::value) {
-                    const int nz = cdiv(SB, 256);
-                    if (SB > 64 && part_cur + (int64_t)nz * NHEAD * HID <= this->partcap) {
-                        LinBwdBatch bt{}; bt.M = SB; bt.store = 0; bt.mchunk = 256; bt.n = 1;
-                        LinBwdJob& J = bt.j[0];
-                        if (nz > 1 && !repro) nd(ND_LIN_BWD_ROWS);
-                        J.dY = dheads; J.X = hx; J.dW = nullptr; J.db = (repro && nz > 1) ? nullptr : dbheads_tmp; J.ldx = HID; J.lddw = HID; J.N = NHEAD; J.K = HID; J.nx = cdiv(NHEAD, 64); J.blk0 = 0;
-                        J.part = this->part + part_cur;
-                        hipLaunchKernelGGL(lin_bwd_smallm_batched_kernel, dim3(J.nx * cdiv(HID, 128), nz), dim3(256), 0, st, bt);
-                        if (!J.db) colsum(dheads, NHEAD, SB, NHEAD, dbheads_tmp);
-                        hipLaunchKernelGGL(unpack_heads_grad_kernel, dim3(cdiv((long long)rows * HID, 256)), dim3(256), 0, st, hp, J.part, dbheads_tmp, HID, nz, (long long)NHEAD * HID);
+                    if (SB > 64 && lin_stream_ok(dheads, hx, HID, NHEAD) && part_cur + (int64_t)NHEAD * HID <= this->partcap) {
+                        wq_add(dheads, hx, HID, SB, NHEAD, HID, nullptr, HID, dbheads_tmp, true);
                         slabs = true;
                     }
                 }
@@ -341,7 +335,8 @@
             mlp_bwd(dppl_t, ppx, EMB + GOAL, B, pp, 5, ppa, dt_a, dt_a + (long long)B * HID, dppx, &om, 0);
             hipLaunchKernelGGL(pp_input_bwd_kernel, dim3(cdiv(B * (EMB + GOAL), 256)), dim3(256), 0, st, dppx, B, EMB, GOAL, demb, (long long)S * EMB, dgoal);
             if (bucket_ready(1)) return 1;
-            lin_wgrad(dprl_t, seqf_t, FCH, B, PLAN, FCH, pr_fs.dW, FCH, pr_fs.db);
+            if (wq_small(B)) wq_add(dprl_t, seqf_t, B, pr_fs);
+            else lin_wgrad(dprl_t, seqf_t, FCH, B, PLAN, FCH, pr_fs.dW, FCH, pr_fs.db);
             { EpiP ep = epi(dseqf, true);
               if (have_dseq) ep.accumulate = 1;
               else { ep.out2 = dseq_t; ep.out2_lo = 0; ep.out2_hi = (long long)B * FCH; dseq_cast_done = true; }
@@ -361,7 +356,8 @@
         }
         if (have_dseq) {
             if (!dseq_cast_done) hipLaunchKernelGGL((cast_kernel<float, T>), dim3(cdiv(B * FCH, 256)), dim3(256), 0, st, dseqf, dseq_t, (long long)B * FCH);
-            lin_wgrad(dseq_t, xm, EMB, B, FCH, EMB, pr_fc.dW, EMB, pr_fc.db);
+            if (wq_small(B)) wq_add(dseq_t, xm, B, pr_fc);
+            else lin_wgrad(dseq_t, xm, EMB, B, FCH, EMB, pr_fc.dW, EMB, pr_fc.db);
             { EpiP ep = epi(dxm, true); lin_dgrad(dseq_t, B, pr_fc, ep, dense_out(EMB)); }
             float* dx = dxa; float* dnext = dxb;
             if (!ln_bwd_can_bcast) hipLaunchKernelGGL(bcast_over_s_kernel, dim3(cdiv((long long)N * EMB, 256)), dim3(256), 0, st, dxm, B, S, EMB, dx);
@@ -390,7 +386,7 @@
                             if (B > 1) nd(ND_TR_LN_BWD);
                             launch_tr_ffn_bwd(st, q);
                         }
-                        tr_wgrad_add(b_c, hff[l], tr_l2[l]); tr_wgrad_add(b_a, x1t[l], tr_l1[l]);
+                        wq_add(b_c, hff[l], N, tr_l2[l]); wq_add(b_a, x1t[l], N, tr_l1[l]);
                     }
                 }
                 if (!ffn_fused) {
@@ -410,22 +406,21 @@
                         q.Wot = tr_out[l].Wtfr; q.Wint = tr_in[l].Wtfr; q.qkv = qkv[l]; q.Pat = Pat[l]; q.b_d = b_d; q.b_b = b_b; q.dy_f = dy_f; q.dx = dx;
                         q.B = B; q.S = S; q.dp = dp; q.seed_o = site_seed(2 + 4 * l); q.seed_att = site_seed(1 + 4 * l);
                         launch_tr_attn_bwd(st, q);
-                        tr_wgrad_add(b_d, ao[l], tr_out[l]);
-                        tr_wgrad_add(b_b, xt[l], tr_in[l]);
+                        wq_add(b_d, ao[l], N, tr_out[l]);
+                        wq_add(b_b, xt[l], N, tr_in[l]);
                         continue;
                     }
                 }
                 ln_bwd(ffn_fused ? dparts : dnext, EMB, y1[l], EMB, st1[l], tr_n1g[l], N, EMB, dy_f, EMB, 0, b_d, EMB, d_tr_n1g[l], d_tr_n1b[l], dp, site_seed(2 + 4 * l), 0, 1.f,
                        ffn_fused ? 4 : 1, (long long)N * EMB);
-                if (defer_w) tr_wgrad_add(b_d, ao[l], tr_out[l]);
+                if (defer_w) wq_add(b_d, ao[l], N, tr_out[l]);
                 else lin_wgrad(b_d, ao[l], EMB, N, EMB, EMB, tr_out[l].dW, EMB, tr_out[l].db);
                 { EpiP ep = epi(dt_a, false); lin_dgrad(b_d, N, tr_out[l], ep, dense_out(EMB)); }
                 launch_attention_bwd<T>(st, attention_s64(S), qkv[l], Pat[l], dt_a, B, S, EMB, NH, b_b, dp, site_seed(1 + 4 * l));
-                if (defer_w) tr_wgrad_add(b_b, xt[l], tr_in[l]);
+                if (defer_w) wq_add(b_b, xt[l], N, tr_in[l]);
                 else lin_wgrad(b_b, xt[l], EMB, N, 3 * EMB, EMB, tr_in[l].dW, EMB, tr_in[l].db);
                 { EpiP ep = epi(dx, true); ep.res = dy_f; ep.res_f32 = 1; ep.res_ld = EMB; lin_dgrad(b_b, N, tr_in[l], ep, dense_out(EMB)); }
             }
-            tr_wgrads_flush(N);
             {
                 const int bchunk = (std::is_same<T, float>::value || repro) ? B : 8;
                 if (cdiv(B, bchunk) > 1) nd(ND_POS_EMB);
@@ -455,6 +450,7 @@
             }
         }
         }
+        wq_flush();
         if (bucket_ready(3)) return 1;
         if (part == 0) {
             lazy_sweep(0, numel, st);
diff --git a/hulc_amd/csrc/engine_encoders.inc b/hulc_amd/csrc/engine_encoders.inc
--- a/hulc_amd/csrc/engine_encoders.inc
+++ b/hulc_amd/csrc/engine_encoders.inc
@@ -257,22 +257,19 @@
             const bool slab_pg = repro && nblk > 1;
             if (slab_pg) for (int k = 0; k < 2; ++k) q.cam[k].pg_slab = cspart + (long long)k * 2 * nblk * 64;
             if (!repro && Nf > 16) nd(ND_ENC_TAIL_LN);
-            if (!repro && Nf > 256) nd(ND_LIN_BWD_ROWS);
             launch_enc_tail_bwd(st, q);
             if (slab_pg)
                 for (int k = 0; k < 2; ++k) {
                     hipLaunchKernelGGL(colsum_final_kernel, dim3(1), dim3(256), 0, st, (const float*)q.cam[k].pg_slab, nblk, 64, encw(k).dlng, (float*)nullptr, 1.f);
                     hipLaunchKernelGGL(colsum_final_kernel, dim3(1), dim3(256), 0, st, (const float*)q.cam[k].pg_slab + (long long)nblk * 64, nblk, 64, encw(k).dlnb, (float*)nullptr, 1.f);
                 }
-            constexpr int chunk = 256;
-            LinBwdBatch bt{}; bt.M = Nf; bt.store = 0; bt.mchunk = chunk;
+            const int nz = enc_tail_nsplit(Nf);
+            if (!repro && nz > 1) nd(ND_LIN_BWD_ROWS);
+            LinStreamBatch bt{};
             int blk = 0;
-            const int nz = cdiv(Nf, chunk);
             const bool cs_bias = repro && nz > 1;
             auto add = [&](const T* dY, const T* X, const LinW& L, float* dW, float* slabs) {
-                LinBwdJob& J = bt.j[bt.n++];
-                J.dY = dY; J.X = X; J.dW = dW; J.db = cs_bias ? nullptr : L.db; J.ldx = L.K; J.lddw = L.K; J.N = L.N; J.K = L.K; J.nx = cdiv(L.N, 64); J.blk0 = blk; J.part = slabs;
-                blk += J.nx * cdiv(L.K, 128);
+                lin_stream_add(bt, blk, (const h16_t*)dY, (const h16_t*)X, L.K, Nf, L.N, L.K, dW, L.K, cs_bias ? nullptr : L.db, slabs, nz, 0);
             };
             for (int k = 0; k < 2; ++k) {
                 const EncW& e = encw(k); EncA& a = enca(k);
@@ -283,7 +280,7 @@
             float* const slabs7 = L.N == 128 && L.K == 3136 ? queue_unpack(L.dW, 128, 64, 7, 7, 1, nz, 1) : nullptr;
             tail_fc7_done = slabs7 != nullptr;
             if (slabs7) add(aG.d_g0, aG.a3, L, nullptr, slabs7);
-            hipLaunchKernelGGL(lin_bwd_smallm_batched_kernel, dim3(blk, nz), dim3(256), 0, st, bt);
+            launch_lin_stream(st, bt, blk);
             if (cs_bias) {
                 for (int k = 0; k < 2; ++k) {
                     const EncW& e = encw(k); EncA& a = enca(k);
@@ -294,8 +291,9 @@
             }
         }
     }
+    static int enc_tail_nsplit(int Nf) { return lin_stream_nsplit(2 * (1 * 4 + 8 * 1) + 2 * 25, Nf); }
     bool enc_tail_bwd_room(int Nf) const {
-        const int64_t nz = cdiv(Nf, 256);
+        const int64_t nz = enc_tail_nsplit(Nf);
         return unpack_room(5, nz * (2 * (64ll * 512 + 512ll * 128) + 128ll * 3136));
     }
     h16_t* zero_page = nullptr;
diff --git a/hulc_amd/csrc/engine_forward.inc b/hulc_amd/csrc/engine_forward.inc
--- a/hulc_amd/csrc/engine_forward.inc
+++ b/hulc_amd/csrc/engine_forward.inc
@@ -8,25 +8,21 @@
             }
         }
     }
-    T* mlp_dy[8] = {nullptr, nullptr, nullptr, nullptr, nullptr, nullptr, nullptr, nullptr};
+    static constexpr int MLP_DY_SETS = 4;
+    T* mlp_dy[MLP_DY_SETS][8] = {};
+    int mlp_dy_next = 0;
     void mlp_bwd(const T* dy, const T* x, long long ldx, int M, LinW* L, int n, T** acts, T* s0, T* s1, float* dxf, const DenseOut* om, int dx_acc) {
         const T* d = dy;
         if constexpr (std::is_same<T, h16_t>::value) {
-            if (M <= 64 && n <= 8) {
-                bool all_first = true;
-                for (int i = 0; i < n; ++i) { const int z = lazy_find(L[i].dW); all_first = all_first && (z >= 0 ? lazy[z].stale : grads_fresh); }
-                for (int i = 0; i < n; ++i) { if (all_first) grad_first(L[i].dW); else grad_ensure_zero(L[i].dW); }
-                LinBwdBatch bt{}; bt.M = M; bt.store = all_first ? 1 : 0;
-                int blk = 0;
+            if (M <= 64 && n <= 8 && mlp_dy_next < MLP_DY_SETS) {
+                T** const set = mlp_dy[mlp_dy_next++];
                 for (int i = n - 1; i >= 0; --i) {
                     const T* in = i > 0 ? acts[i - 1] : x;
                     const long long ld = i > 0 ? L[i - 1].N : ldx;
-                    LinBwdJob& J = bt.j[bt.n++];
-                    J.dY = d; J.X = in; J.dW = L[i].dW; J.db = L[i].db; J.ldx = ld; J.lddw = L[i].K; J.N = L[i].N; J.K = L[i].K; J.nx = cdiv(L[i].N, 64); J.blk0 = blk;
-                    blk += J.nx * cdiv(L[i].K, 128);
+                    wq_add(d, in, ld, M, L[i].N, L[i].K, L[i].dW, L[i].K, L[i].db);
                     if (i > 0) {
-                        if (!mlp_dy[i]) mlp_dy[i] = alloc<T>((int64_t)64 * 2048);
-                        T* o = L[i].K <= 2048 ? mlp_dy[i] : (T*)nullptr;
+                        if (!set[i]) set[i] = alloc<T>((int64_t)64 * 2048);
+                        T* o = L[i].K <= 2048 ? set[i] : (T*)nullptr;
                         if (!o) { hulc_set_error("mlp_bwd: hidden width %d exceeds the per-layer gradient buffers", L[i].K); return; }
                         EpiP ep = epi(o, false); ep.mask = acts[i - 1];
                         lin_dgrad(d, M, L[i], ep, dense_out(L[i].K));
@@ -36,7 +32,6 @@
                         lin_dgrad(d, M, L[i], ep, *om);
                     }
                 }
-                hipLaunchKernelGGL(lin_bwd_smallm_batched_kernel, dim3(blk), dim3(256), 0, st, bt);
                 return;
             }
         }
diff --git a/hulc_amd/csrc/iengine.h b/hulc_amd/csrc/iengine.h
--- a/hulc_amd/csrc/iengine.h
+++ b/hulc_amd/csrc/iengine.h
@@ -201,6 +201,8 @@
     int k_gemm_multi(int form, const hulc_gemm_epi_job* jobs, int n, int sh, int* ran, void* stream);                                           \
     int k_gemm_pick(int t16, int M, int N, int K, long long lda, long long ldb, int* pick, int* bk);                                            \
     int k_gemm_wgrad_nsplit(int t16, int M, int N, int K, int* nsplit, int* big);                                                               \
+    int k_lin_bwd_stream(const void* dY, const void* X, long long ldx, int M, int N, int K, int nsplit, int store, float* dW, long long lddw,    \
+                         float* db, float* slabs, void* stream);                                                                                \
     int k_conv_wgrad(const char* who, int typed, int which, const void* X, const void* dY, float* out, float* db_out, int Nf, int IH, int* slabs, \
                      void* stream);                                                                                                             \
     int k_conv1_wgrad_u8(const char* who, int typed, const void* X, const int* shifts, int pad, const void* dY, float* dw_out, float* db_out,   \
diff --git a/hulc_amd/csrc/k_entries.h b/hulc_amd/csrc/k_entries.h
--- a/hulc_amd/csrc/k_entries.h
+++ b/hulc_amd/csrc/k_entries.h
@@ -582,6 +582,26 @@
     *nsplit = t16 ? gemm_wgrad_nsplit<h16_t>(M, N, K, &b) : gemm_wgrad_nsplit<float>(M, N, K, &b);
     *big = b ? 1 : 0;
     return 0;
+}
+
+int k_lin_bwd_stream(const void* dY, const void* X, long long ldx, int M, int N, int K, int nsplit, int store, float* dW, long long lddw, float* db, float* slabs, void* stream) {
+    static const char* who = "hulc_k_lin_bwd_stream";
+    hipStream_t st = (hipStream_t)stream;
+    if (!dY || !X || !dW || M < 1 || N < 1 || K < 1 || ldx < K || lddw < K || nsplit < 1 || nsplit > 64) { hulc_set_error("%s: null argument or bad shape (M=%d N=%d K=%d nsplit=%d)", who, M, N, K, nsplit); return 1; }
+    if ((long long)M * std::max<long long>(N, ldx) >= (1ll << 31) || (long long)N * lddw >= (1ll << 31)) { hulc_set_error("%s: operand too large", who); return 1; }
+    if (!lin_stream_ok(dY, X, ldx, N)) { hulc_set_error("%s: rows must start 8-byte aligned (N, ldx multiples of 4; dY, X 8-byte aligned)", who); return 1; }
+    if (k_misaligned16(slabs)) { hulc_set_error("%s: the slab buffer [nsplit][N][K] must be 16-byte aligned", who); return 1; }
+    LinStreamBatch bt{};
+    int blocks = 0;
+    lin_stream_add(bt, blocks, (const h16_t*)dY, (const h16_t*)X, ldx, M, N, K, dW, lddw, db, slabs, nsplit, store ? 1 : 0);
+    const bool clear = store && (slabs || nsplit > 1);
+    if (clear && hipMemset2DAsync(dW, sizeof(float) * lddw, 0, sizeof(float) * K, N, st) != hipSuccess) { hulc_set_error("%s: clearing dW failed", who); return 1; }
+    launch_lin_stream(st, bt, blocks);
+    if (slabs) {
+        const int vec = (K & 3) == 0 && (lddw & 3) == 0 && !k_misaligned16(dW);
+        hipLaunchKernelGGL(slab_sum_kernel, dim3(cdiv((long long)N * K, vec ? 1024 : 256)), dim3(256), 0, st, (const float*)slabs, nsplit, (long long)N * K, N, K, dW, lddw, vec);
+    }
+    return k_launched(who);
 }
 
 static inline int k_conv_fwd_side(int in_side, int K, int S) { return in_side < K ? -1 : (in_side - K) / S + 1; }
diff --git a/hulc_amd/lib.py b/hulc_amd/lib.py
--- a/hulc_amd/lib.py
+++ b/hulc_amd/lib.py
@@ -117,7 +117,8 @@
            "hulc_k_det_head_loss", "hulc_k_det_head_bwd", "hulc_k_det_head_act",
            "hulc_k_conv_wgrad_t", "hulc_k_conv1_wgrad_u8_t", "hulc_k_conv_tile_t", "hulc_k_conv_pair_t", "hulc_k_conv_plan",
            "hulc_decoder_body_select", "hulc_trainable_set", "hulc_trainable_get", "hulc_trainable_steps_set",
-           "hulc_ema_enable", "hulc_ema_state_get", "hulc_ema_state_set", "hulc_ema_swap", "hulc_ema_swapped", "hulc_k_ema_update"]
+           "hulc_ema_enable", "hulc_ema_state_get", "hulc_ema_state_set", "hulc_ema_swap", "hulc_ema_swapped", "hulc_k_ema_update",
+           "hulc_k_lin_bwd_stream"]
 
 _lib = None
 
@@ -264,6 +265,9 @@
         lib.hulc_k_gemm_multi.argtypes = [I, I, C.POINTER(HulcGemmEpiJob), I, I, PI, C.c_void_p]
         lib.hulc_k_gemm_pick.argtypes = [I, I, I, I, Q, Q, PI, PI]
         lib.hulc_k_gemm_wgrad_nsplit.argtypes = [I, I, I, I, PI, PI]
+    if hasattr(lib, "hulc_k_lin_bwd_stream") or not os.environ.get("HULC_LIB_PATH"):
+        P, I, Q = C.c_void_p, C.c_int32, C.c_int64
+        lib.hulc_k_lin_bwd_stream.argtypes = [I, P, P, Q, I, I, I, I, I, P, Q, P, P, P]
     if hasattr(lib, "hulc_decoder_select") or not os.environ.get("HULC_LIB_PATH"):
         P, I, F = C.c_void_p, C.c_int32, C.c_float
         lib.hulc_decoder_select.argtypes = [P, I, I]
diff --git a/include/hulc_hip.h b/include/hulc_hip.h
--- a/include/hulc_hip.h
+++ b/include/hulc_hip.h
@@ -343,6 +343,8 @@
 int hulc_k_gemm_multi(int32_t dtype, int32_t form, const hulc_gemm_epi_job* jobs, int32_t n, int32_t sh, int32_t* ran, void* hip_stream);
 int hulc_k_gemm_pick(int32_t dtype, int32_t M, int32_t N, int32_t K, int64_t lda, int64_t ldb, int32_t* pick, int32_t* bk);
 int hulc_k_gemm_wgrad_nsplit(int32_t dtype, int32_t M, int32_t N, int32_t K, int32_t* nsplit, int32_t* big);
+int hulc_k_lin_bwd_stream(int32_t dtype, const void* dY, const void* X, int64_t ldx, int32_t M, int32_t N, int32_t K, int32_t nsplit, int32_t store, float* dW, int64_t lddw,
+                          float* db, float* slabs, void* hip_stream);
 
 #ifdef __cplusplus
 }
```

Measured after the change: 21670 windows/s (median of 6 runs). 1.01x the previous value.
